# nschloe/flow

Hardware: AMD Instinct MI355X
Metric: ipcs_time_steps_per_sec (higher is better)
Workload: dtype f64

## Files before the change

### flow_amd/_hip.py

```python
import ctypes
import os

import torch

from . import device

_HERE = os.path.dirname(os.path.abspath(__file__))
LIB_PATH = os.path.join(_HERE, 'csrc', 'libflow_hip.so')

REDUCE_WORK = 4096
GMRES_MAX_RESTART = 30
GMRES_PARTIALS = (GMRES_MAX_RESTART + 2) * 1024
GMRES_STATE = 1280
SPMV_ROWS_PER_BLOCK = 256
SPMV_NNZ_PER_BLOCK = 1022
PMG_NNZ_PER_BLOCK = 2044

c_double_p = ctypes.c_void_p
c_int_p = ctypes.c_void_p


class Operator(ctypes.Structure):
    _fields_ = [
        ('kind', ctypes.c_int),
        ('n', ctypes.c_int),
        ('nnz', ctypes.c_int),
        ('nblocks', ctypes.c_int),
        ('rowptr', ctypes.c_void_p),
        ('cols', ctypes.c_void_p),
        ('rowblocks', ctypes.c_void_p),
        ('vals', ctypes.c_void_p * 4),
        ('matfree', ctypes.c_void_p),
        ('rowmask', ctypes.c_void_p),
        ]


class CoarseS(ctypes.Structure):
    _fields_ = [
        ('n', ctypes.c_int),
        ('nc', ctypes.c_int),
        ('agg_ptr', ctypes.c_void_p),
        ('agg_dofs', ctypes.c_void_p),
        ('agg_of', ctypes.c_void_p),
        ('lda', ctypes.c_int),
        ('Ainv', ctypes.c_void_p),
        ]


MG_MAX_LEVELS = 8


class MgS(ctypes.Structure):
    _fields_ = [
        ('nlevels', ctypes.c_int),
        ('Ah', Operator * MG_MAX_LEVELS),
        ('dinv', ctypes.c_void_p * MG_MAX_LEVELS),
        ('Ps', Operator * MG_MAX_LEVELS),
        ('R', Operator * MG_MAX_LEVELS),
        ('r', ctypes.c_void_p * MG_MAX_LEVELS),
        ('x', ctypes.c_void_p * MG_MAX_LEVELS),
        ('t', ctypes.c_void_p * MG_MAX_LEVELS),
        ('nc', ctypes.c_int), ('lda', ctypes.c_int),
        ('Ainv', ctypes.c_void_p),
        ('omega', ctypes.c_double),
        ('C', Operator * MG_MAX_LEVELS),
        ('up_rowblocks', ctypes.c_void_p * MG_MAX_LEVELS),
        ('up_nblocks', ctypes.c_int * MG_MAX_LEVELS),
        ]


class IluPlanS(ctypes.Structure):
    _fields_ = [
        ('n', ctypes.c_int), ('nnz', ctypes.c_int), ('ncolors', ctypes.c_int),
        ('nnz_l', ctypes.c_int), ('nnz_u', ctypes.c_int),
        ('off_l', ctypes.c_int), ('off_u', ctypes.c_int),
        ('off_d', ctypes.c_int), ('lu_size', ctypes.c_int),
        ('max_row', ctypes.c_int), ('nslices', ctypes.c_int),
        ('color_ptr_host', ctypes.c_void_p),
        ('slice_ptr_host', ctypes.c_void_p),
        ('rowptr', ctypes.c_void_p), ('cols', ctypes.c_void_p),
        ('diag', ctypes.c_void_p), ('src_pos', ctypes.c_void_p),
        ('old_of_new', ctypes.c_void_p), ('new_of_old', ctypes.c_void_p),
        ('slice_row', ctypes.c_void_p),
        ('l_slice_off', ctypes.c_void_p), ('l_cols', ctypes.c_void_p),
        ('l_pos', ctypes.c_void_p),
        ('u_slice_off', ctypes.c_void_p), ('u_cols', ctypes.c_void_p),
        ('u_pos', ctypes.c_void_p),
        ]


class IluS(ctypes.Structure):
    _fields_ = [
        ('plan', ctypes.POINTER(IluPlanS)),
        ('nblocks', ctypes.c_int),
        ('lu', ctypes.c_void_p),
        ('packed', ctypes.c_void_p),
        ('single_vector', ctypes.c_int),
        ('cycle', ctypes.c_void_p),
        ]


class TlS(ctypes.Structure):
    _fields_ = [
        ('fine', ctypes.POINTER(IluS)), ('coarse', ctypes.POINTER(IluS)),
        ('fine_op', ctypes.c_void_p), ('coarse_op', ctypes.c_void_p),
        ('pre', ctypes.c_int), ('post', ctypes.c_int),
        ('coarse_sweeps', ctypes.c_int),
        ('ends', ctypes.c_void_p), ('rptr', ctypes.c_void_p),
        ('rsrc', ctypes.c_void_p),
        ('bc_fine', ctypes.c_void_p), ('bc_coarse', ctypes.c_void_p),
        ('rscale', ctypes.c_void_p), ('work', ctypes.c_void_p),
        ]


class PmgLevelS(ctypes.Structure):
    _fields_ = [
        ('n', ctypes.c_int), ('nnz', ctypes.c_int), ('nblocks', ctypes.c_int),
        ('rowptr', ctypes.c_void_p), ('cols', ctypes.c_void_p),
        ('rowblocks', ctypes.c_void_p),
        ('vals', ctypes.c_void_p), ('diag', ctypes.c_void_p),
        ('dinv', ctypes.c_void_p),
        ('lam_min', ctypes.c_double), ('lam_max', ctypes.c_double),
        ('cols16', ctypes.c_void_p), ('cbase', ctypes.c_void_p),
        ('packed', ctypes.c_void_p), ('idrows', ctypes.c_void_p),
        ]


class PmgS(ctypes.Structure):
    _fields_ = [
        ('fine', PmgLevelS), ('coarse', PmgLevelS),
        ('pre', ctypes.c_int), ('post', ctypes.c_int),
        ('coarse_steps', ctypes.c_int),
        ('ends', ctypes.c_void_p),
        ('rptr', ctypes.c_void_p), ('rsrc', ctypes.c_void_p),
        ('bc_fine', ctypes.c_void_p), ('bc_coarse', ctypes.c_void_p),
        ('work', ctypes.c_void_p),
        ('scalar', ctypes.c_int),
        ]


class MassS(ctypes.Structure):
    _fields_ = [
        ('A', ctypes.POINTER(Operator)),
        ('dinv', ctypes.c_void_p),
        ('nblocks16', ctypes.c_int),
        ('rowblocks16', ctypes.c_void_p),
        ('vals16', ctypes.c_void_p),
        ('lam_min', ctypes.c_double), ('lam_max', ctypes.c_double),
        ('steps', ctypes.c_int),
        ('contraction', ctypes.c_double),
        ('work16', ctypes.c_void_p),
        ('packed16', ctypes.c_void_p),
        ('cbase16', ctypes.c_void_p),
        ('work16_rows', ctypes.c_int),
        ]


class MassStripsS(ctypes.Structure):
    _fields_ = [
        ('nlevels', ctypes.c_int),
        ('rowblocks16', ctypes.c_void_p * 16),
        ('nblocks16', ctypes.c_int * 16),
        ('row_lo_last', ctypes.c_int), ('row_hi_last', ctypes.c_int),
        ]


class MeshS(ctypes.Structure):
    _fields_ = [('nc', ctypes.c_int), ('xy', ctypes.c_void_p),
                ('c0', ctypes.c_int), ('c1', ctypes.c_int)]


class SpaceS(ctypes.Structure):
    _fields_ = [
        ('deg', ctypes.c_int),
        ('n', ctypes.c_int),
        ('nnz', ctypes.c_int),
        ('cell_dofs', ctypes.c_void_p),
        ('cptr', ctypes.c_void_p),
        ('csrc', ctypes.c_void_p),
        ('vptr', ctypes.c_void_p),
        ('vsrc', ctypes.c_void_p),
        ('r0', ctypes.c_int), ('r1', ctypes.c_int),
        ('nnz0', ctypes.c_int), ('nnz1', ctypes.c_int),
        ]


class CoefS(ctypes.Structure):
    _fields_ = [
        ('nl', ctypes.c_int),
        ('cell_stride', ctypes.c_int),
        ('values', ctypes.c_void_p),
        ('G', ctypes.c_void_p),
        ]


FORM_MAX_PROGRAM = 64
FORM_REGISTERS = 8
FORM_MAX_CONSTANTS = 32
FORM_MAX_FIELDS = 6
FORM_MAX_EXPRESSIONS = 4
FORM_MAX_POINTS = 256


class FormS(ctypes.Structure):
    _fields_ = [
        ('nprog', ctypes.c_int),
        ('prog', ctypes.c_int * (4 * FORM_MAX_PROGRAM)),
        ('nconst', ctypes.c_int),
        ('consts', ctypes.c_double * FORM_MAX_CONSTANTS),
        ('nfield', ctypes.c_int),
        ('field', ctypes.c_void_p * FORM_MAX_FIELDS),
        ('field_deg', ctypes.c_int * FORM_MAX_FIELDS),
        ('cell_dofs', ctypes.c_void_p * 2),
        ('nexpr', ctypes.c_int),
        ('expr', ctypes.c_void_p * FORM_MAX_EXPRESSIONS),
        ('expr_nl', ctypes.c_int * FORM_MAX_EXPRESSIONS),
        ('expr_table', ctypes.c_int * FORM_MAX_EXPRESSIONS),
        ('nq', ctypes.c_int),
        ('rule', ctypes.c_void_p),
        ('tables', ctypes.c_void_p),
        ('ntables', ctypes.c_int),
        ('nout', ctypes.c_int),
        ]


class PointGridS(ctypes.Structure):
    _fields_ = [
        ('nx', ctypes.c_int), ('ny', ctypes.c_int),
        ('x0', ctypes.c_double), ('y0', ctypes.c_double),
        ('hx_inv', ctypes.c_double), ('hy_inv', ctypes.c_double),
        ('start', ctypes.c_void_p),
        ('cells', ctypes.c_void_p),
        ]


class NsParams(ctypes.Structure):
    _fields_ = [
        ('dt', ctypes.c_double), ('rho', ctypes.c_double),
        ('mu', ctypes.c_double), ('theta_i', ctypes.c_double),
        ('theta_e', ctypes.c_double),
        ]


ALLREDUCE_FN = ctypes.CFUNCTYPE(ctypes.c_int, ctypes.c_void_p, ctypes.c_int)


class PeerS(ctypes.Structure):
    _fields_ = [
        ('flags', ctypes.c_void_p), ('land', ctypes.c_void_p),
        ('land_cap', ctypes.c_int), ('spin_limit', ctypes.c_int),
        ('nb_flags', ctypes.c_void_p * 2), ('nb_land', ctypes.c_void_p * 2),
        ('seq_host', ctypes.POINTER(ctypes.c_ulonglong * 5)),
        ]


PEER_FLAGS = 16


class CommS(ctypes.Structure):
    _fields_ = [
        ('rank', ctypes.c_int), ('world', ctypes.c_int),
        ('buf', ctypes.c_void_p), ('capacity', ctypes.c_int),
        ('allreduce', ALLREDUCE_FN), ('user', ctypes.c_void_p),
        ('peer', ctypes.POINTER(PeerS)),
        ]


class RcclBinding(ctypes.Structure):
    _fields_ = [('comm', ctypes.c_void_p), ('buf', ctypes.c_void_p),
                ('stream', ctypes.c_void_p)]


class RowsS(ctypes.Structure):
    _fields_ = [
        ('n', ctypes.c_int), ('r0', ctypes.c_int), ('r1', ctypes.c_int),
        ('e0', ctypes.c_int), ('e1', ctypes.c_int), ('nhalo', ctypes.c_int),
        ('send_row', ctypes.c_int * 2), ('send_len', ctypes.c_int * 2),
        ('send_slot', ctypes.c_int * 2),
        ('recv_row', ctypes.c_int * 2), ('recv_len', ctypes.c_int * 2),
        ('recv_slot', ctypes.c_int * 2),
        ]


class MgShardS(ctypes.Structure):
    _fields_ = [
        ('mg', ctypes.POINTER(MgS)),
        ('Ah0', Operator), ('Ps0', Operator), ('Rg', Operator),
        ('Cg', Operator),
        ('up_rowblocks0', ctypes.c_void_p), ('up_nblocks0', ctypes.c_int),
        ('z_lo', ctypes.c_int), ('z_hi', ctypes.c_int),
        ]


class MomentumJvp(ctypes.Structure):
    _fields_ = [
        ('mesh', ctypes.POINTER(MeshS)),
        ('W', ctypes.POINTER(SpaceS)),
        ('bfmask', ctypes.c_void_p),
        ('ui', ctypes.c_void_p),
        ('prm', NsParams),
        ('scratch', ctypes.c_void_p),
        ('nbc', ctypes.c_int),
        ('bc_dofs', ctypes.c_void_p),
        ('bc_mask', ctypes.c_void_p),
        ]


_VP = ctypes.c_void_p
_I = ctypes.c_int
_D = ctypes.c_double
_P = ctypes.POINTER
SYMBOLS = {
    'flow_abi_version': [],
    'flow_launch_count': [_P(ctypes.c_ulonglong)],
    'flow_graph_mode': [_I, ctypes.c_longlong],
    'flow_graph_stats': [_P(ctypes.c_ulonglong)],
    'flow_xcd_tile_host': [_I, _I],
    'flow_spmv_tile_nnz': [_I],
    'flow_operator_apply': [_P(Operator), _VP, _VP, _VP],
    'flow_profile_spmv_begin': [_I, _I],
    'flow_profile_spmv_end': [_P(_D), _P(_I)],
    'flow_profile_event_overhead': [_P(_D), _VP],
    'flow_profile_marker': [_I, _VP],
    'flow_profile_stream_copy': [ctypes.c_size_t, _VP, _VP, _VP],
    'flow_profile_stream_read': [ctypes.c_size_t, _VP, _VP, _VP],
    'flow_operator_diag_inv': [_P(Operator), _VP, _VP, _VP],
    'flow_dot_host': [_I, _VP, _VP, _VP, _P(_D), _VP],
    'flow_norm_host': [_I, _VP, _I, _VP, _P(_D), _VP],
    'flow_axpby': [_I, _D, _VP, _D, _VP, _VP],
    'flow_vmul': [_I, _D, _VP, _VP, _VP, _VP],
    'flow_fill': [_I, _D, _VP, _VP],
    'flow_lincomb': [_I, _I, _P(_D), _P(_VP), _VP, _VP],
    'flow_fingerprint': [_I, _P(_VP), _P(_I), _VP, _VP, _VP],
    'flow_read_doubles': [_VP, _I, _P(_D), _VP],
    'flow_extrapolation_weights': [_I, _P(_D), _D, _I, _I, _P(_D)],
    'flow_scale_rows': [_I, _VP, _VP, _VP, _VP],
    'flow_cg_solve': [_P(Operator), _VP, _P(CoarseS), _P(MgS), _VP, _VP, _D, _D,
                      _I, _I, _I, _VP, ctypes.c_size_t, _P(_I), _P(_D), _VP],
    'flow_cg_solve_guarded': [_P(Operator), _VP, _P(CoarseS), _P(MgS), _VP, _VP,
                              _VP, _D, _D, _I, _I, _I, _VP, ctypes.c_size_t,
                              _P(_I), _P(_D), _P(_I), _VP],
    'flow_mg_apply': [_P(MgS), _I, _VP, _VP, _VP],
    'flow_two_level_apply': [_P(CoarseS), _VP, _VP, _VP, _VP, _VP],
    'flow_bicgstab_solve': [_P(Operator), _VP, _P(IluS), _VP, _VP, _D, _D, _I,
                            _I, _I, _VP, ctypes.c_size_t, _P(_I), _P(_D), _VP],
    'flow_gmres_solve': [_P(Operator), _VP, _P(IluS), _P(PmgS), _VP, _VP, _D,
                         _D, _I, _I, _I, _I, _I, _VP, ctypes.c_size_t, _P(_I),
                         _P(_D), _VP],
    'flow_pmg_pack': [_I, _I, _VP, _VP, _VP, _VP, _VP, _VP, _VP, _VP, _VP],
    'flow_pmg_pack1': [_I, _I, _I, _VP, _VP, _VP, _VP, _VP, _VP, _VP, _VP, _VP,
                       _VP, _VP, _VP, _VP],
    'flow_pmg_cols16': [_I, _VP, _VP, _VP, _VP, _VP, _VP, _VP],
    'flow_pmg_lambda_max': [_P(PmgLevelS), _I, _VP, _VP, _VP, _P(_D), _VP],
    'flow_pmg_apply': [_P(PmgS), _VP, _VP, _VP],
    'flow_tl_apply': [_P(TlS), _VP, _VP, _VP],
    'flow_aggregate_host': [_I, _VP, _VP, _VP, ctypes.c_double, _VP, _VP,
                            _P(ctypes.c_int)],
    'flow_peer_alloc': [ctypes.c_int, _P(ctypes.c_void_p), ctypes.c_char_p],
    'flow_peer_open': [ctypes.c_char_p, _P(ctypes.c_void_p)],
    'flow_peer_close': [_VP],
    'flow_peer_free': [_VP],
    'flow_peer_status': [_P(PeerS), _P(ctypes.c_ulonglong), _VP],
    'flow_mass_pack': [_I, _VP, _VP, _VP, _VP, _VP],
    'flow_mass_pack16': [_I, _I, _VP, _VP, _VP, _VP, _VP, _VP, _VP, _VP, _VP],
    'flow_mass_solve': [_P(MassS), _VP, _VP, _D, _D, _I, _I, _VP,
                        ctypes.c_size_t, _P(_I), _P(_D), _VP],
    'flow_mass_solve_increment': [_P(MassS), _VP, _VP, _VP, _VP, _D, _D, _I, _I, _VP,
                                  ctypes.c_size_t, _P(_I), _P(_D), _VP],
    'flow_gather_rows': [_I, _VP, _I, _VP, _I, _VP, _I, _VP],
    'flow_color_greedy_host': [_I, _VP, _VP, _VP, _P(_I)],
    'flow_color_iterate_host': [_I, _VP, _VP, _VP, _P(_I), _I],
    'flow_ilu0_factor': [_P(IluPlanS), _I, _VP, _VP, _VP, _VP],
    'flow_ilu0_pack': [_P(IluS), _VP, _VP],
    'flow_ilu0_solve': [_P(IluS), _VP, _VP, _VP, _VP],
    'flow_rccl_load': [ctypes.c_char_p],
    'flow_rccl_unique_id': [_VP],
    'flow_rccl_comm_create': [_VP, _I, _I, _P(_VP)],
    'flow_rccl_comm_destroy': [_VP],
    'flow_rccl_allreduce': [_VP, _I],
    'flow_shard_halo': [_P(CommS), _P(RowsS), _I, _VP, _I, _VP],
    'flow_shard_reduce_host': [_P(CommS), _P(RowsS), _I, _VP, _VP, _I, _I, _VP,
                               _P(_D), _VP],
    'flow_shard_cg_solve': [_P(CommS), _P(RowsS), _P(Operator), _VP, _VP, _VP,
                            _D, _D, _I, _I, _I, _VP, ctypes.c_size_t, _P(_I),
                            _P(_D), _P(_I), _VP],
    'flow_shard_mgcg_solve': [_P(CommS), _P(RowsS), _P(Operator), _VP,
                              _P(MgShardS), _VP, _VP, _D, _D, _I, _I, _I, _VP,
                              ctypes.c_size_t, _P(_I), _P(_D), _P(_I), _VP],
    'flow_shard_mass_solve': [_P(CommS), _P(RowsS), _P(MassS), _P(MassStripsS),
                              _VP, _VP, _VP, _VP, _D, _D, _I, _I, _VP,
                              ctypes.c_size_t, _P(_I), _P(_D), _VP],
    'flow_shard_gmres_solve': [_P(CommS), _P(RowsS), _P(Operator), _P(IluS),
                               _P(PmgS), _VP, _VP, _D, _D, _I, _I, _I, _I, _I,
                               _VP, ctypes.c_size_t, _P(_I), _P(_D), _VP],
    'flow_assemble_scalar_matrix': [_I, _P(MeshS), _P(SpaceS), _VP, _VP, _VP],
    'flow_assemble_pressure_rhs': [_P(MeshS), _P(SpaceS), _P(SpaceS), _VP, _VP,
                                   _D, _D, _I, _VP, _VP, _VP],
    'flow_assemble_correction_rhs': [_P(MeshS), _P(SpaceS), _P(SpaceS), _VP,
                                     _VP, _VP, _D, _D, _I, _VP, _VP, _VP],
    'flow_assemble_momentum': [_P(MeshS), _P(SpaceS), _P(SpaceS), _VP, _VP, _VP,
                               _VP, _P(CoefS), _P(CoefS), _P(NsParams), _VP,
                               _VP, _VP, ctypes.c_size_t, _VP],
    'flow_momentum_jvp_apply': [_P(MomentumJvp), _VP, _VP, _VP],
    'flow_assemble_source': [_P(MeshS), _P(SpaceS), _I, _P(CoefS), _VP, _VP,
                             _VP],
    'flow_assemble_magnitude': [_P(MeshS), _P(SpaceS), _I, _VP, _VP, _VP, _VP],
    'flow_assemble_div_adjoint': [_P(MeshS), _P(SpaceS), _P(SpaceS), _VP, _VP,
                                  _VP, _VP],
    'flow_bc_identity_rows': [_P(Operator), _VP, _VP, _I, _VP, _VP],
    'flow_bc_residual': [_I, _VP, _VP, _VP, _VP, _VP],
    'flow_bc_set_values': [_I, _VP, _VP, _VP, _VP],
    'flow_bc_symmetric_matrix': [_I, _VP, _VP, _VP, _VP, _VP, _VP],
    'flow_assemble_heat': [_P(MeshS), _P(SpaceS), _P(SpaceS), _VP, _D, _D, _I,
                           _VP, _VP, _VP, _VP, _VP, _VP],
    'flow_assemble_heat_supg_source': [_P(MeshS), _P(SpaceS), _P(SpaceS), _VP,
                                       _D, _D, _P(CoefS), _VP, _VP, _VP, _VP],
    'flow_form_functional': [_P(MeshS), _P(FormS), _VP, _VP, _P(_D), _VP],
    'flow_form_load_vector': [_P(MeshS), _P(SpaceS), _P(FormS), _VP, _VP, _VP],
    'flow_form_facet_functional': [_P(MeshS), _P(FormS), _I, _VP, _VP, _VP, _VP,
                                   _P(_D), _VP],
    'flow_locate_points': [_P(MeshS), _P(PointGridS), _I, _VP, _VP, _VP, _VP],
    'flow_form_points': [_P(MeshS), _P(FormS), _I, _VP, _VP, _VP, _VP],
    }

_LIB = None


class HipError(RuntimeError):
    pass


class NotConverged(RuntimeError):
    '''Krylov / Newton non-convergence.  A RuntimeError, because callers of the
    reference catch exactly that (tests/test_boussinesq.py:254).'''


ABI_VERSION = 30


def load_library():
    global _LIB
    if _LIB is None:
        if not os.path.isfile(LIB_PATH):
            raise HipError(
                'libflow_hip.so not found at %s -- build it with '
                '`python -c "import __graft_entry__ as g; g.build()"` or '
                '`make -C flow_amd/csrc`' % LIB_PATH
                )
        lib = ctypes.CDLL(LIB_PATH)
        lib.flow_last_error.restype = ctypes.c_char_p
        lib.flow_last_error.argtypes = []
        for name, argtypes in SYMBOLS.items():
            fn = getattr(lib, name)
            fn.restype = ctypes.c_int
            fn.argtypes = argtypes
        got = lib.flow_abi_version()
        if got != ABI_VERSION:
            raise HipError(
                '%s is ABI version %d, these bindings are version %d: '
                'rebuild it (`make -C flow_amd/csrc`)'
                % (LIB_PATH, got, ABI_VERSION))
        _LIB = lib
    return _LIB


def launch_count():
    n = ctypes.c_ulonglong(0)
    check(load_library().flow_launch_count(ctypes.byref(n)))
    return int(n.value)


_GRAPHS = {'mode': None}


def graph_mode(mode, auto_rows=-1, sites=0):
    check(load_library().flow_graph_mode(int(mode) | (int(sites) << 4),
                                         int(auto_rows)))
    _GRAPHS['mode'] = int(mode)


def graphs_possible():
    if _GRAPHS['mode'] is not None:
        return _GRAPHS['mode'] != 0
    return os.environ.get('FLOW_AMD_GRAPHS', '0') not in ('', '0')


def graph_stats():
    v = (ctypes.c_ulonglong * 8)()
    check(load_library().flow_graph_stats(v))
    return {'graphs': int(v[0]), 'captures': int(v[1]), 'replays': int(v[2]),
            'nodes': int(v[3]), 'captures_cg': int(v[4]),
            'captures_gmres': int(v[5]), 'captures_mass': int(v[6])}


def spmv_tile_nnz(kind=0):
    return int(load_library().flow_spmv_tile_nnz(int(kind)))


def lib():
    handle = load_library()
    if not device.on_gpu():
        raise HipError(
            'flow_amd needs an AMD GPU (MI355X): the hot path has no CPU '
            'fallback'
            )
    return handle


def check(rc):
    if rc == 0:
        return
    msg = load_library().flow_last_error().decode('utf-8', 'replace')
    if rc == 1:
        raise NotConverged(msg)
    if rc == 2:
        raise ValueError(msg)
    raise HipError(msg)


def _ptr(t, dtype, numel=None, name='operand'):
    if t is None:
        return None
    if not isinstance(t, torch.Tensor):
        raise TypeError('%s: expected a torch tensor' % name)
    if t.dtype != dtype:
        raise TypeError('%s: dtype %s, expected %s' % (name, t.dtype, dtype))
    if not t.is_cuda:
        raise HipError('%s is not in device memory' % name)
    if not t.is_contiguous():
        raise ValueError('%s is not contiguous' % name)
    if numel is not None and t.numel() < numel:
        raise ValueError(
            '%s has %d elements, needs %d' % (name, t.numel(), numel)
            )
    return ctypes.c_void_p(t.data_ptr())


def f64(t, numel=None, name='fp64 operand'):
    return _ptr(t, torch.float64, numel, name)


def f32(t, numel=None, name='fp32 operand'):
    return _ptr(t, torch.float32, numel, name)


def f16(t, numel=None, name='fp16 operand'):
    return _ptr(t, torch.float16, numel, name)


def i32(t, numel=None, name='int32 operand'):
    return _ptr(t, torch.int32, numel, name)


def u8(t, numel=None, name='uint8 operand'):
    return _ptr(t, torch.uint8, numel, name)


def stream():
    return ctypes.c_void_p(device.stream_handle())


def copy(dst, src):
    assert dst.numel() == src.numel()
    if not dst.is_cuda:
        dst.copy_(src)
    elif dst.data_ptr() != src.data_ptr():
        check(lib().flow_axpby(dst.numel(), 1.0, f64(src, name='src'), 0.0,
                               f64(dst, name='dst'), stream()))
    return dst


def fill(t, value=0.0):
    if not t.is_cuda:
        t.fill_(float(value))
    elif t.numel() > 0:
        check(lib().flow_fill(t.numel(), float(value), f64(t), stream()))
    return t


def clone(t):
    out = torch.empty_like(t)
    return copy(out, t)
```

### flow_amd/csrc/assembly_kernels.hip

```cpp
#include <cstdlib>

#include "fem_device.h"

namespace flow {

template <int NP>
__global__ __launch_bounds__(kBlock) void gather_kernel(
    int nout, const int* __restrict__ ptr, const int* __restrict__ src,
    const double* __restrict__ scratch, size_t plane_stride, size_t out_stride,
    double* __restrict__ out, const double* __restrict__ stop,
    const unsigned char* __restrict__ idrow = nullptr, size_t id_stride = 0,
    const double* __restrict__ v = nullptr, size_t v_stride = 0) {
  if (stopped(stop)) return;
  for (int k = blockIdx.x * blockDim.x + threadIdx.x; k < nout;
       k += gridDim.x * blockDim.x) {
    const int a = ptr[k];
    const int b = ptr[k + 1];
    double s[NP];
#pragma unroll
    for (int p = 0; p < NP; ++p) s[p] = 0.0;
    for (int t = a; t < b; t += 4) {
      int idx[4];
#pragma unroll
      for (int j = 0; j < 4; ++j) idx[j] = t + j < b ? src[t + j] : -1;
      double w[NP][4];
#pragma unroll
      for (int p = 0; p < NP; ++p)
#pragma unroll
        for (int j = 0; j < 4; ++j)
          w[p][j] = idx[j] >= 0 ? scratch[p * plane_stride + idx[j]] : 0.0;
#pragma unroll
      for (int p = 0; p < NP; ++p)
#pragma unroll
        for (int j = 0; j < 4; ++j) s[p] += w[p][j];
    }
    if (idrow) {
#pragma unroll
      for (int p = 0; p < NP; ++p)
        if (idrow[p * id_stride + k]) s[p] = v[p * v_stride + k];
    }
#pragma unroll
    for (int p = 0; p < NP; ++p) out[static_cast<size_t>(p) * out_stride + k] = s[p];
  }
}

int gather(int nout, int nplanes, const int* ptr, const int* src,
           const double* scratch, size_t plane_stride, double* out,
           hipStream_t st, size_t out_stride, int r0, int r1, const double* stop,
           const unsigned char* idrow, const double* v, size_t v_stride) {
  const size_t os = out_stride ? out_stride : static_cast<size_t>(nout);
  const size_t ids = static_cast<size_t>(nout);
  if (r1 > 0) {
    ptr += r0;
    out += r0;
    if (idrow) idrow += r0;
    if (v) v += r0;
    nout = r1 - r0;
  }
  const dim3 grid(grid_for(nout, kBlock, 1 << 20));
  FLOW_REQUIRE(nplanes == 1 || nplanes == 2, "gather: 1 or 2 planes");
  if (nplanes == 1)
    hipLaunchKernelGGL(gather_kernel<1>, grid, dim3(kBlock), 0, st, nout, ptr,
                       src, scratch, plane_stride, os, out, stop, idrow, ids, v,
                       v_stride);
  else
    hipLaunchKernelGGL(gather_kernel<2>, grid, dim3(kBlock), 0, st, nout, ptr,
                       src, scratch, plane_stride, os, out, stop, idrow, ids, v,
                       v_stride);
  FLOW_CHECK_LAUNCH();
  return FLOW_OK;
}

template <int NL>
__device__ __forceinline__ void load_local(const double* __restrict__ u, int n,
                                           const int* __restrict__ cd, int nc,
                                           int c, int ,
                                           double U[2][NL]) {
#pragma unroll
  for (int i = 0; i < NL; ++i) {
    const int d = cd[i * nc + c];
    U[0][i] = u[d];
    U[1][i] = u[static_cast<size_t>(n) + d];
  }
}

template <int DEG>
__global__ __launch_bounds__(kBlock) void scalar_matrix_kernel(
    int kind, int nc, const double* __restrict__ xy,
    double* __restrict__ scratch) {
  constexpr int NL = Elem<DEG>::NL;
  constexpr int NQ = Elem<2>::NQ;
  const int c = blockIdx.x * blockDim.x + threadIdx.x;
  if (c >= nc) return;
  const Geom g = load_geom(xy, nc, c);
  double Ke[NL][NL];
#pragma unroll
  for (int i = 0; i < NL; ++i)
#pragma unroll
    for (int j = 0; j < NL; ++j) Ke[i][j] = 0.0;
  if (kind == 2) {
#pragma unroll
    for (int i = 0; i < 3; ++i) Ke[i][i] = g.adet / 6.0;
  } else {
#pragma unroll
    for (int q = 0; q < NQ; ++q) {
      const double L[3] = {kQ7L[q][0], kQ7L[q][1], kQ7L[q][2]};
      const double w = 0.5 * kQ7W[q] * g.adet;
      double phi[NL], dphi[NL][3], gphi[NL][2];
      basis<DEG>(L, phi, dphi);
      phys_grad<NL>(g, dphi, gphi);
#pragma unroll
      for (int i = 0; i < NL; ++i)
#pragma unroll
        for (int j = 0; j < NL; ++j)
          Ke[i][j] += (kind == 0)
                          ? w * (gphi[i][0] * gphi[j][0] + gphi[i][1] * gphi[j][1])
                          : w * phi[i] * phi[j];
    }
  }
#pragma unroll
  for (int i = 0; i < NL; ++i)
#pragma unroll
    for (int j = 0; j < NL; ++j)
      scratch[static_cast<size_t>(i * NL + j) * nc + c] = Ke[i][j];
}

template <int DEG>
__global__ __launch_bounds__(kBlock) void pressure_rhs_kernel(
    int nc, int cb, int ce, const double* __restrict__ xy, const int* __restrict__ cdu, int nu,
    const int* __restrict__ cdp, const double* __restrict__ u,
    const double* __restrict__ p0, double alpha_rho_dt, double mu,
    int rotational, double* __restrict__ scratch) {
  constexpr int NL = Elem<DEG>::NL;
  const int c = cb + xcd_tile(blockIdx.x, gridDim.x) * blockDim.x + threadIdx.x;
  if (c >= ce) return;
  const Geom g = load_geom(xy, nc, c);
  double U[2][NL];
  load_local<NL>(u, nu, cdu, nc, c, 2, U);
  double d[3];
  div_at_vertices<DEG>(g, U, d);
  const double area = 0.5 * g.adet;
  const double dsum = d[0] + d[1] + d[2];
  double gp[2] = {0.0, 0.0};
#pragma unroll
  for (int k = 0; k < 3; ++k) {
    double coef = p0[cdp[k * nc + c]];
    if (rotational) coef -= mu * d[k];
    gp[0] += coef * g.gl[k][0];
    gp[1] += coef * g.gl[k][1];
  }
#pragma unroll
  for (int i = 0; i < 3; ++i) {
    const double b = -alpha_rho_dt * (area / 12.0) * (dsum + d[i]) +
                     area * (gp[0] * g.gl[i][0] + gp[1] * g.gl[i][1]);
    scratch[static_cast<size_t>(i) * nc + c] = b;
  }
}

template <int DEG>
__global__ __launch_bounds__(kBlock) void correction_rhs_kernel(
    int nc, int cb, int ce, const double* __restrict__ xy, const int* __restrict__ cdu, int nu,
    const int* __restrict__ cdp, const double* __restrict__ u,
    const double* __restrict__ p1, const double* __restrict__ p0, double dt_rho,
    double mu, int rotational, double* __restrict__ scratch) {
  constexpr int NL = Elem<DEG>::NL;
  constexpr int NQ = Elem<2>::NQ;
  const int c = cb + xcd_tile(blockIdx.x, gridDim.x) * blockDim.x + threadIdx.x;
  if (c >= ce) return;
  const Geom g = load_geom(xy, nc, c);
  double U[2][NL];
  load_local<NL>(u, nu, cdu, nc, c, 2, U);
  double d[3] = {0.0, 0.0, 0.0};
  if (rotational & 1) div_at_vertices<DEG>(g, U, d);
  const double mass = (rotational & 2) ? 0.0 : 1.0;
  double gphi_f[2] = {0.0, 0.0};
#pragma unroll
  for (int k = 0; k < 3; ++k) {
    const int dof = cdp[k * nc + c];
    const double coef = p1[dof] - p0[dof] + mu * d[k];
    gphi_f[0] += coef * g.gl[k][0];
    gphi_f[1] += coef * g.gl[k][1];
  }
  double acc[2][NL];
#pragma unroll
  for (int a = 0; a < 2; ++a)
#pragma unroll
    for (int i = 0; i < NL; ++i) acc[a][i] = 0.0;
#pragma unroll
  for (int q = 0; q < NQ; ++q) {
    const double L[3] = {kQ7L[q][0], kQ7L[q][1], kQ7L[q][2]};
    const double w = 0.5 * kQ7W[q] * g.adet;
    double phi[NL], dphi[NL][3];
    basis<DEG>(L, phi, dphi);
#pragma unroll
    for (int a = 0; a < 2; ++a) {
      double uq = 0.0;
#pragma unroll
      for (int j = 0; j < NL; ++j) uq += U[a][j] * phi[j];
      const double val = w * (mass * uq - dt_rho * gphi_f[a]);
#pragma unroll
      for (int i = 0; i < NL; ++i) acc[a][i] += val * phi[i];
    }
  }
#pragma unroll
  for (int a = 0; a < 2; ++a)
#pragma unroll
    for (int i = 0; i < NL; ++i)
      scratch[static_cast<size_t>(a * NL + i) * nc + c] = acc[a][i];
}

template <int NL>
__device__ __forceinline__ void add_source(const flow_coef& f, int nc, int c,
                                           int dim, double scale,
                                           double acc[][NL]) {
  const size_t nce = f.cell_stride ? static_cast<size_t>(nc) : 1;
  const size_t cc = f.cell_stride ? static_cast<size_t>(c) : 0;
  for (int a = 0; a < dim; ++a) {
    for (int l = 0; l < f.nl; ++l) {
      const double F = scale * f.values[(static_cast<size_t>(a) * f.nl + l) * nce + cc];
#pragma unroll
      for (int i = 0; i < NL; ++i) acc[a][i] += F * f.G[l * NL + i];
    }
  }
}

template <int DEG>
__global__ __launch_bounds__(kBlock) void source_kernel(
    int nc, const double* __restrict__ xy, int dim, flow_coef f,
    double* __restrict__ scratch) {
  constexpr int NL = Elem<DEG>::NL;
  const int c = blockIdx.x * blockDim.x + threadIdx.x;
  if (c >= nc) return;
  const Geom g = load_geom(xy, nc, c);
  double acc[2][NL];
#pragma unroll
  for (int a = 0; a < 2; ++a)
#pragma unroll
    for (int i = 0; i < NL; ++i) acc[a][i] = 0.0;
  add_source<NL>(f, nc, c, dim, g.adet, acc);
  for (int a = 0; a < dim; ++a)
#pragma unroll
    for (int i = 0; i < NL; ++i)
      scratch[static_cast<size_t>(a * NL + i) * nc + c] = acc[a][i];
}

template <int NL>
__device__ __forceinline__ void add_rhs_weak_point(
    double w, double rho, double mu, const double U[2][NL], const double P[3],
    const double L[3], const double phi[NL], const double gphi[NL][2],
    double acc[2][NL]) {
  double uq[2] = {0.0, 0.0};
  double gu[2][2] = {{0.0, 0.0}, {0.0, 0.0}};
#pragma unroll
  for (int j = 0; j < NL; ++j) {
#pragma unroll
    for (int a = 0; a < 2; ++a) {
      uq[a] += U[a][j] * phi[j];
      gu[a][0] += U[a][j] * gphi[j][0];
      gu[a][1] += U[a][j] * gphi[j][1];
    }
  }
  const double pq = P[0] * L[0] + P[1] * L[1] + P[2] * L[2];
  const double conv[2] = {gu[0][0] * uq[0] + gu[0][1] * uq[1],
                          gu[1][0] * uq[0] + gu[1][1] * uq[1]};
#pragma unroll
  for (int i = 0; i < NL; ++i) {
    const double ugp = uq[0] * gphi[i][0] + uq[1] * gphi[i][1];
#pragma unroll
    for (int a = 0; a < 2; ++a) {
      double r = -0.5 * rho * (conv[a] * phi[i] - ugp * uq[a]);
      r -= mu * ((gu[a][0] + gu[0][a]) * gphi[i][0] +
                 (gu[a][1] + gu[1][a]) * gphi[i][1]);
      r += pq * gphi[i][a];
      acc[a][i] += w * r;
    }
  }
}

template <int DEG>
__device__ __forceinline__ void add_rhs_weak_facets(
    int mask, double scale, double mu, const Geom& g,
    const double U[2][Elem<DEG>::NL], const double P[3],
    double acc[2][Elem<DEG>::NL]) {
  constexpr int NL = Elem<DEG>::NL;
  for (int lf = 0; lf < 3; ++lf) {
    if (!((mask >> lf) & 1)) continue;
    const int v0 = facet_v0(lf), v1 = facet_v1(lf);
    const double nL[2] = {-g.gl[lf][0] * g.adet, -g.gl[lf][1] * g.adet};
    for (int gq = 0; gq < 2; ++gq) {
      const double s = gq == 0 ? FLOW_G2A : FLOW_G2B;
      double L[3] = {0.0, 0.0, 0.0};
      L[v0] = 1.0 - s;
      L[v1] = s;
      double phi[NL], dphi[NL][3], gphi[NL][2];
      basis<DEG>(L, phi, dphi);
      phys_grad<NL>(g, dphi, gphi);
      double gu[2][2] = {{0.0, 0.0}, {0.0, 0.0}};
#pragma unroll
      for (int j = 0; j < NL; ++j)
#pragma unroll
        for (int a = 0; a < 2; ++a) {
          gu[a][0] += U[a][j] * gphi[j][0];
          gu[a][1] += U[a][j] * gphi[j][1];
        }
      const double pq = P[0] * L[0] + P[1] * L[1] + P[2] * L[2];
      const double w = 0.5 * scale;
#pragma unroll
      for (int a = 0; a < 2; ++a) {
        const double t = -pq * nL[a] + mu * (gu[0][a] * nL[0] + gu[1][a] * nL[1]);
#pragma unroll
        for (int i = 0; i < NL; ++i) acc[a][i] += w * t * phi[i];
      }
    }
  }
}

template <int DEG>
__global__ __launch_bounds__(kBlock) void momentum_residual_kernel(
    int nc, int cb, int ce, const double* __restrict__ xy, const int* __restrict__ cdu, int nu,
    const int* __restrict__ cdp, const int* __restrict__ bfmask,
    const double* __restrict__ ui, const double* __restrict__ u0,
    const double* __restrict__ p0, flow_coef f0, flow_coef f1,
    flow_ns_params prm, double* __restrict__ scratch) {
  constexpr int NL = Elem<DEG>::NL;
  constexpr int NQ = Elem<DEG>::NQ;
  const int c = cb + xcd_tile(blockIdx.x, gridDim.x) * blockDim.x + threadIdx.x;
  if (c >= ce) return;
  const Geom g = load_geom(xy, nc, c);
  double Ui[2][NL], U0[2][NL], P[3];
  load_local<NL>(ui, nu, cdu, nc, c, 2, Ui);
  load_local<NL>(u0, nu, cdu, nc, c, 2, U0);
#pragma unroll
  for (int k = 0; k < 3; ++k) P[k] = p0[cdp[k * nc + c]];
  const int mask = bfmask[c];
  const double ci = -prm.dt / prm.rho * prm.theta_i;
  const double cexp = -prm.dt / prm.rho * prm.theta_e;
  double acc[2][NL];
#pragma unroll
  for (int a = 0; a < 2; ++a)
#pragma unroll
    for (int i = 0; i < NL; ++i) acc[a][i] = 0.0;

#pragma unroll
  for (int q = 0; q < NQ; ++q) {
    const double L[3] = {qpoint<DEG>(q, 0), qpoint<DEG>(q, 1), qpoint<DEG>(q, 2)};
    const double w = 0.5 * qweight<DEG>(q) * g.adet;
    double phi[NL], dphi[NL][3], gphi[NL][2];
    basis<DEG>(L, phi, dphi);
    phys_grad<NL>(g, dphi, gphi);
#pragma unroll
    for (int a = 0; a < 2; ++a) {
      double du = 0.0;
#pragma unroll
      for (int j = 0; j < NL; ++j) du += (Ui[a][j] - U0[a][j]) * phi[j];
#pragma unroll
      for (int i = 0; i < NL; ++i) acc[a][i] += w * du * phi[i];
    }
    if (ci != 0.0)
      add_rhs_weak_point<NL>(w * ci, prm.rho, prm.mu, Ui, P, L, phi, gphi, acc);
    if (cexp != 0.0)
      add_rhs_weak_point<NL>(w * cexp, prm.rho, prm.mu, U0, P, L, phi, gphi, acc);
  }
  if (mask) {
    if (ci != 0.0) add_rhs_weak_facets<DEG>(mask, ci, prm.mu, g, Ui, P, acc);
    if (cexp != 0.0) add_rhs_weak_facets<DEG>(mask, cexp, prm.mu, g, U0, P, acc);
  }
  if (ci != 0.0) add_source<NL>(f1, nc, c, 2, ci * g.adet, acc);
  if (cexp != 0.0) add_source<NL>(f0, nc, c, 2, cexp * g.adet, acc);
#pragma unroll
  for (int a = 0; a < 2; ++a)
#pragma unroll
    for (int i = 0; i < NL; ++i)
      scratch[static_cast<size_t>(a * NL + i) * nc + c] = acc[a][i];
}

template <int DEG>
__global__ __launch_bounds__(kBlock) void momentum_jvp_kernel(
    int nc, int cb, int ce, const double* __restrict__ xy,
    const int* __restrict__ cdu, int nu, int nv,
    const int* __restrict__ bfmask, const double* __restrict__ ui,
    const double* __restrict__ v, flow_ns_params prm,
    const double* __restrict__ prm_dev,
    double* __restrict__ scratch, const double* __restrict__ stop) {
  constexpr int NL = Elem<DEG>::NL;
  constexpr int NQ = Elem<DEG>::NQ;
  if (stopped(stop)) return;
  const int c = cb + xcd_tile(blockIdx.x, gridDim.x) * blockDim.x + threadIdx.x;
  if (c >= ce) return;
  const Geom g = load_geom(xy, nc, c);
  double U[2][NL], V[2][NL];
  load_local<NL>(ui, nu, cdu, nc, c, 2, U);
  load_local<NL>(v, nv, cdu, nc, c, 2, V);
  const int mask = bfmask[c];
  const double ci = prm_dev ? load_scalar(prm_dev)
                            : -prm.dt / prm.rho * prm.theta_i;
  const double hr = prm_dev ? load_scalar(prm_dev + 1) : 0.5 * prm.rho;
  const double mu = prm_dev ? load_scalar(prm_dev + 2) : prm.mu;
  double acc[2][NL];
#pragma unroll
  for (int a = 0; a < 2; ++a)
#pragma unroll
    for (int i = 0; i < NL; ++i) acc[a][i] = 0.0;

#pragma unroll
  for (int q = 0; q < NQ; ++q) {
    const double L[3] = {qpoint<DEG>(q, 0), qpoint<DEG>(q, 1), qpoint<DEG>(q, 2)};
    const double w = 0.5 * qweight<DEG>(q) * g.adet;
    double uq[2], vq[2], gu[2][2], gv[2][2];
#pragma unroll
    for (int a = 0; a < 2; ++a) {
      uq[a] = eval_at<DEG>(U[a], L);
      vq[a] = eval_at<DEG>(V[a], L);
      double gur[3], gvr[3];
      ref_gradient<DEG>(U[a], L, gur);
      ref_gradient<DEG>(V[a], L, gvr);
#pragma unroll
      for (int d = 0; d < 2; ++d) {
        gu[a][d] = gur[0] * g.gl[0][d] + gur[1] * g.gl[1][d] + gur[2] * g.gl[2][d];
        gv[a][d] = gvr[0] * g.gl[0][d] + gvr[1] * g.gl[1][d] + gvr[2] * g.gl[2][d];
      }
    }
#pragma unroll
    for (int a = 0; a < 2; ++a) {
      const double dconv = gv[a][0] * uq[0] + gv[a][1] * uq[1] +
                           gu[a][0] * vq[0] + gu[a][1] * vq[1];
      const double s0 = w * (vq[a] - ci * hr * dconv);
      double S1[2];
#pragma unroll
      for (int d = 0; d < 2; ++d)
        S1[d] = w * ci * (hr * (vq[d] * uq[a] + uq[d] * vq[a]) -
                          mu * (gv[a][d] + gv[d][a]));
      double T[3];
#pragma unroll
      for (int k = 0; k < 3; ++k) T[k] = g.gl[k][0] * S1[0] + g.gl[k][1] * S1[1];
      test_accumulate<DEG>(L, s0, T, acc[a]);
    }
  }
  if (mask && ci != 0.0) {
    const double P0[3] = {0.0, 0.0, 0.0};
    add_rhs_weak_facets<DEG>(mask, ci, mu, g, V, P0, acc);
  }
#pragma unroll
  for (int a = 0; a < 2; ++a)
#pragma unroll
    for (int i = 0; i < NL; ++i)
      scratch[static_cast<size_t>(a * NL + i) * nc + c] = acc[a][i];
}

template <int DEG>
__global__ __launch_bounds__(kBlock) void momentum_jvp_pair_kernel(
    int nc, int cb, int ce, const double* __restrict__ xy,
    const int* __restrict__ cdu, int nu, int nv,
    const int* __restrict__ bfmask, const double* __restrict__ ui,
    const double* __restrict__ v, flow_ns_params prm,
    const double* __restrict__ prm_dev,
    double* __restrict__ scratch, const double* __restrict__ stop) {
  constexpr int NL = Elem<DEG>::NL;
  constexpr int NQ = Elem<DEG>::NQ;
  if (stopped(stop)) return;
  const int t = xcd_tile(blockIdx.x, gridDim.x) * blockDim.x + threadIdx.x;
  const int c = cb + (t >> 1);
  const int a = t & 1;
  if (c >= ce) return;
  const Geom g = load_geom(xy, nc, c);
  double U[NL], V[NL];
#pragma unroll
  for (int i = 0; i < NL; ++i) {
    const int d = cdu[i * nc + c];
    U[i] = ui[static_cast<size_t>(a) * nu + d];
    V[i] = v[static_cast<size_t>(a) * nv + d];
  }
  const int mask = bfmask[c];
  const double ci = prm_dev ? load_scalar(prm_dev)
                            : -prm.dt / prm.rho * prm.theta_i;
  const double hr = prm_dev ? load_scalar(prm_dev + 1) : 0.5 * prm.rho;
  const double mu = prm_dev ? load_scalar(prm_dev + 2) : prm.mu;
  double acc[NL];
#pragma unroll
  for (int i = 0; i < NL; ++i) acc[i] = 0.0;

#pragma unroll
  for (int q = 0; q < NQ; ++q) {
    const double L[3] = {qpoint<DEG>(q, 0), qpoint<DEG>(q, 1), qpoint<DEG>(q, 2)};
    const double w = 0.5 * qweight<DEG>(q) * g.adet;
    const double uq = eval_at<DEG>(U, L);
    const double vq = eval_at<DEG>(V, L);
    double gur[3], gvr[3], gu[2], gv[2];
    ref_gradient<DEG>(U, L, gur);
    ref_gradient<DEG>(V, L, gvr);
#pragma unroll
    for (int d = 0; d < 2; ++d) {
      gu[d] = gur[0] * g.gl[0][d] + gur[1] * g.gl[1][d] + gur[2] * g.gl[2][d];
      gv[d] = gvr[0] * g.gl[0][d] + gvr[1] * g.gl[1][d] + gvr[2] * g.gl[2][d];
    }
    const double uo = __shfl_xor(uq, 1, 64);
    const double vo = __shfl_xor(vq, 1, 64);
    const double cross = __shfl_xor(a == 0 ? gv[1] : gv[0], 1, 64);
    const double u0 = a == 0 ? uq : uo, u1 = a == 0 ? uo : uq;
    const double v0 = a == 0 ? vq : vo, v1 = a == 0 ? vo : vq;
    const double dconv = gv[0] * u0 + gv[1] * u1 + gu[0] * v0 + gu[1] * v1;
    const double s0 = w * (vq - ci * hr * dconv);
    const double t0 = a == 0 ? gv[0] : cross;
    const double t1 = a == 0 ? cross : gv[1];
    double S1[2];
    S1[0] = w * ci * (hr * (v0 * uq + u0 * vq) - mu * (gv[0] + t0));
    S1[1] = w * ci * (hr * (v1 * uq + u1 * vq) - mu * (gv[1] + t1));
    double T[3];
#pragma unroll
    for (int k = 0; k < 3; ++k) T[k] = g.gl[k][0] * S1[0] + g.gl[k][1] * S1[1];
    test_accumulate<DEG>(L, s0, T, acc);
  }
  if (mask && ci != 0.0) {
    for (int lf = 0; lf < 3; ++lf) {
      if (!((mask >> lf) & 1)) continue;
      const int f0 = facet_v0(lf), f1 = facet_v1(lf);
      const double nL[2] = {-g.gl[lf][0] * g.adet, -g.gl[lf][1] * g.adet};
      for (int gq = 0; gq < 2; ++gq) {
        const double sg = gq == 0 ? FLOW_G2A : FLOW_G2B;
        double L[3] = {0.0, 0.0, 0.0};
        L[f0] = 1.0 - sg;
        L[f1] = sg;
        double gvr[3], gv[2];
        ref_gradient<DEG>(V, L, gvr);
#pragma unroll
        for (int d = 0; d < 2; ++d)
          gv[d] = gvr[0] * g.gl[0][d] + gvr[1] * g.gl[1][d] + gvr[2] * g.gl[2][d];
        const double cross = __shfl_xor(a == 0 ? gv[1] : gv[0], 1, 64);
        const double tn = a == 0 ? gv[0] * nL[0] + cross * nL[1]
                                 : cross * nL[0] + gv[1] * nL[1];
        const double wt = 0.5 * ci * mu * tn;
        double phi[NL], dphi[NL][3];
        basis<DEG>(L, phi, dphi);
#pragma unroll
        for (int i = 0; i < NL; ++i) acc[i] += wt * phi[i];
      }
    }
  }
#pragma unroll
  for (int i = 0; i < NL; ++i)
    scratch[static_cast<size_t>(a * NL + i) * nc + c] = acc[i];
}

__global__ void bc_copy_kernel(int nbc, const int* __restrict__ dofs, int n,
                               int r0, int r1, const double* __restrict__ v,
                               int vs, double* __restrict__ out, int os,
                               const double* __restrict__ stop) {
  if (stopped(stop)) return;
  const int k = blockIdx.x * blockDim.x + threadIdx.x;
  if (k >= nbc) return;
  const int d = dofs[k];
  const int a = d / n;
  const int row = d - a * n;
  if (row >= r0 && row < r1)
    out[static_cast<size_t>(a) * os + row] = v[static_cast<size_t>(a) * vs + row];
}

template <int DEG>
struct BasisTab {
  double phi[Elem<DEG>::NQ][Elem<DEG>::NL];
  double dphi[Elem<DEG>::NQ][Elem<DEG>::NL][3];
};

template <int DEG>
__global__ __launch_bounds__(kBlock) void momentum_jacobian_kernel(
    int nc, int cb, int ce, const double* __restrict__ xy, const int* __restrict__ cdu, int nu,
    const int* __restrict__ bfmask, const double* __restrict__ ui,
    flow_ns_params prm, double* __restrict__ scratch) {
  constexpr int NL = Elem<DEG>::NL;
  constexpr int NQ = Elem<DEG>::NQ;
  constexpr int NP = NL * NL;
  __shared__ double s_uq[NQ][2][64];
  __shared__ double s_gu[NQ][4][64];
  __shared__ BasisTab<DEG> tab;

  const int lane = threadIdx.x & 63;
  const int grp = threadIdx.x >> 6;
  const int c = cb + blockIdx.x * 64 + lane;
  const bool active = c < ce;
  const int cc = active ? c : ce - 1;

  for (int t = threadIdx.x; t < NQ * NL; t += kBlock) {
    const int q = t / NL, i = t % NL;
    const double L[3] = {qpoint<DEG>(q, 0), qpoint<DEG>(q, 1), qpoint<DEG>(q, 2)};
    double phi[NL], dphi[NL][3];
    basis<DEG>(L, phi, dphi);
    tab.phi[q][i] = phi[i];
    tab.dphi[q][i][0] = dphi[i][0];
    tab.dphi[q][i][1] = dphi[i][1];
    tab.dphi[q][i][2] = dphi[i][2];
  }

  const Geom g = load_geom(xy, nc, cc);
  const int mask = bfmask[cc];
  {
    double U[2][NL];
    load_local<NL>(ui, nu, cdu, nc, cc, 2, U);
    for (int q = grp; q < NQ; q += 4) {
      const double L[3] = {qpoint<DEG>(q, 0), qpoint<DEG>(q, 1),
                           qpoint<DEG>(q, 2)};
      double phi[NL], dphi[NL][3], gphi[NL][2];
      basis<DEG>(L, phi, dphi);
      phys_grad<NL>(g, dphi, gphi);
      double uq[2] = {0.0, 0.0}, gu[4] = {0.0, 0.0, 0.0, 0.0};
#pragma unroll
      for (int j = 0; j < NL; ++j) {
        uq[0] += U[0][j] * phi[j];
        uq[1] += U[1][j] * phi[j];
        gu[0] += U[0][j] * gphi[j][0];
        gu[1] += U[0][j] * gphi[j][1];
        gu[2] += U[1][j] * gphi[j][0];
        gu[3] += U[1][j] * gphi[j][1];
      }
      s_uq[q][0][lane] = uq[0];
      s_uq[q][1][lane] = uq[1];
#pragma unroll
      for (int k = 0; k < 4; ++k) s_gu[q][k][lane] = gu[k];
    }
  }
  __syncthreads();

  const double c1 = -prm.dt / prm.rho * prm.theta_i;
  const double hr = 0.5 * prm.rho;
  const double mu = prm.mu;

  for (int pr = grp; pr < NP; pr += 4) {
    const int i = pr / NL, j = pr % NL;
    double B[2][2] = {{0.0, 0.0}, {0.0, 0.0}};
#pragma unroll
    for (int q = 0; q < NQ; ++q) {
      const double w = 0.5 * qweight<DEG>(q) * g.adet;
      const double pi = tab.phi[q][i], pj = tab.phi[q][j];
      double gi[2], gj[2];
#pragma unroll
      for (int d = 0; d < 2; ++d) {
        gi[d] = tab.dphi[q][i][0] * g.gl[0][d] + tab.dphi[q][i][1] * g.gl[1][d] +
                tab.dphi[q][i][2] * g.gl[2][d];
        gj[d] = tab.dphi[q][j][0] * g.gl[0][d] + tab.dphi[q][j][1] * g.gl[1][d] +
                tab.dphi[q][j][2] * g.gl[2][d];
      }
      const double u0 = s_uq[q][0][lane], u1 = s_uq[q][1][lane];
      const double gu[2][2] = {{s_gu[q][0][lane], s_gu[q][1][lane]},
                               {s_gu[q][2][lane], s_gu[q][3][lane]}};
      const double uq[2] = {u0, u1};
      const double ugj = u0 * gj[0] + u1 * gj[1];
      const double ugi = u0 * gi[0] + u1 * gi[1];
      const double kij = gi[0] * gj[0] + gi[1] * gj[1];
      const double diag =
          pi * pj + c1 * (-hr * (ugj * pi - ugi * pj) - mu * kij);
#pragma unroll
      for (int a = 0; a < 2; ++a)
#pragma unroll
        for (int cb = 0; cb < 2; ++cb) {
          double v = c1 * (-hr * (pj * pi * gu[a][cb] - pj * gi[cb] * uq[a]) -
                           mu * gj[a] * gi[cb]);
          if (a == cb) v += diag;
          B[a][cb] += w * v;
        }
    }
    if (mask) {
      for (int lf = 0; lf < 3; ++lf) {
        if (!((mask >> lf) & 1)) continue;
        const int v0 = facet_v0(lf), v1 = facet_v1(lf);
        const double nL[2] = {-g.gl[lf][0] * g.adet, -g.gl[lf][1] * g.adet};
        for (int gq = 0; gq < 2; ++gq) {
          const double s = gq == 0 ? FLOW_G2A : FLOW_G2B;
          double L[3] = {0.0, 0.0, 0.0};
          L[v0] = 1.0 - s;
          L[v1] = s;
          double phi[NL], dphi[NL][3], gphi[NL][2];
          basis<DEG>(L, phi, dphi);
          phys_grad<NL>(g, dphi, gphi);
          double pi = 0.0, gj0 = 0.0, gj1 = 0.0;
#pragma unroll
          for (int t = 0; t < NL; ++t) {
            if (t == i) pi = phi[t];
            if (t == j) {
              gj0 = gphi[t][0];
              gj1 = gphi[t][1];
            }
          }
          const double w = 0.5 * c1 * mu * pi;
          B[0][0] += w * gj0 * nL[0];
          B[0][1] += w * gj0 * nL[1];
          B[1][0] += w * gj1 * nL[0];
          B[1][1] += w * gj1 * nL[1];
        }
      }
    }
    if (active) {
      double2* out = reinterpret_cast<double2*>(
          scratch + (static_cast<size_t>(c) * NP + pr) * 4);
      out[0] = make_double2(B[0][0], B[0][1]);
      out[1] = make_double2(B[1][0], B[1][1]);
    }
  }
}

__global__ void gather_blocks_kernel(int k0, int nnz, int nc, int np,
                                     const int* __restrict__ ptr,
                                     const int* __restrict__ src,
                                     const double* __restrict__ scratch,
                                     size_t out_stride,
                                     double* __restrict__ out) {
  for (int k = k0 + blockIdx.x * blockDim.x + threadIdx.x; k < nnz;
       k += gridDim.x * blockDim.x) {
    const int a = ptr[k];
    const int b = ptr[k + 1];
    double s0 = 0.0, s1 = 0.0, s2 = 0.0, s3 = 0.0;
    for (int t = a; t < b; ++t) {
      const int s = src[t];
      const int ij = s / nc;
      const int cell = s - ij * nc;
      const double2* blk = reinterpret_cast<const double2*>(
          scratch + (static_cast<size_t>(cell) * np + ij) * 4);
      const double2 v0 = blk[0], v1 = blk[1];
      s0 += v0.x;
      s1 += v0.y;
      s2 += v1.x;
      s3 += v1.y;
    }
    out[k] = s0;
    out[out_stride + k] = s1;
    out[2 * out_stride + k] = s2;
    out[3 * out_stride + k] = s3;
  }
}

__global__ void bc_identity_rows_kernel(int kind, int n, size_t nnz,
                                        const int* __restrict__ rowptr,
                                        const int* __restrict__ diag_idx,
                                        int nbc, const int* __restrict__ dofs,
                                        double* __restrict__ vals) {
  for (int t = blockIdx.x * blockDim.x + threadIdx.x; t < nbc;
       t += gridDim.x * blockDim.x) {
    const int d = dofs[t];
    const int a = d / n;
    const int i = d - a * n;
    const int k0 = rowptr[i], k1 = rowptr[i + 1];
    if (kind == 2) {
      double* p0 = vals + static_cast<size_t>(2 * a) * nnz;
      double* p1 = vals + static_cast<size_t>(2 * a + 1) * nnz;
      for (int k = k0; k < k1; ++k) {
        p0[k] = 0.0;
        p1[k] = 0.0;
      }
      vals[static_cast<size_t>(3 * a) * nnz + diag_idx[i]] = 1.0;
    } else {
      double* p = vals + static_cast<size_t>(a) * nnz;
      for (int k = k0; k < k1; ++k) p[k] = 0.0;
      p[diag_idx[i]] = 1.0;
    }
  }
}

__global__ void bc_residual_kernel(int nbc, const int* __restrict__ dofs,
                                   const double* __restrict__ g,
                                   const double* __restrict__ u,
                                   double* __restrict__ F) {
  for (int t = blockIdx.x * blockDim.x + threadIdx.x; t < nbc;
       t += gridDim.x * blockDim.x) {
    const int d = dofs[t];
    F[d] = u ? u[d] - g[t] : g[t];
  }
}

__global__ void bc_symmetric_kernel(int n, const int* __restrict__ rowptr,
                                    const int* __restrict__ cols,
                                    const double* __restrict__ vin,
                                    const unsigned char* __restrict__ isbc,
                                    double* __restrict__ vout) {
  for (int r = blockIdx.x * blockDim.x + threadIdx.x; r < n;
       r += gridDim.x * blockDim.x) {
    const bool rb = isbc[r] != 0;
    for (int k = rowptr[r]; k < rowptr[r + 1]; ++k) {
      const int c = cols[k];
      vout[k] = (rb || isbc[c]) ? (r == c ? 1.0 : 0.0) : vin[k];
    }
  }
}

__device__ __forceinline__ double supg_tau(const double px[3], const double py[3],
                                           double area, double bx, double by,
                                           double eps, int p, int* status) {
  const double nb = sqrt(bx * bx + by * by);
  if (nb < 1.0e-10) return 0.0;
  double sum = 0.0;
#pragma unroll
  for (int i = 0; i < 3; ++i)
#pragma unroll
    for (int j = i + 1; j < 3; ++j) {
      const double e0 = px[i] - px[j];
      const double e1 = py[i] - py[j];
      sum += fabs(e1 * bx - e0 * by);
    }
  const double h = 4.0 * nb * area / sum;
  const double Pe = 0.5 * nb * h / (p * eps);
  const double xi = Pe > 1.0e-5
                        ? (1.0 / tanh(Pe) - 1.0 / Pe) / Pe
                        : 1.0 / 3.0 - Pe * Pe / 45.0 +
                              2.0 / 945.0 * Pe * Pe * Pe * Pe;
  const double tau = h * h / 4.0 / eps / p * xi;
  if (tau > 1.0e3) *status = 1;
  return tau;
}

template <int DEGQ, int DEGW, bool SUPG>
__global__ __launch_bounds__(kBlock) void heat_kernel(
    int nc, int cb, int ce, const double* __restrict__ xy,
    const int* __restrict__ cdw, int nw,
    const double* __restrict__ conv, double kappa, double rho_cp,
    double* __restrict__ scratch, double* __restrict__ tau_out,
    int* __restrict__ status) {
  constexpr int NL = Elem<DEGQ>::NL;
  constexpr int NW = Elem<DEGW>::NL;
  constexpr int NQ = SUPG ? 16 : 7;
  const int c = cb + blockIdx.x * blockDim.x + threadIdx.x;
  if (c >= ce) return;
  const Geom g = load_geom(xy, nc, c);
  double Cv[2][NW];
  load_local<NW>(conv, nw, cdw, nc, c, 2, Cv);
  double tau_v[3] = {0.0, 0.0, 0.0};
  double lap[NL];
#pragma unroll
  for (int i = 0; i < NL; ++i) lap[i] = 0.0;
  if constexpr (SUPG) {
    const double px[3] = {xy[0 * nc + c], xy[1 * nc + c], xy[2 * nc + c]};
    const double py[3] = {xy[3 * nc + c], xy[4 * nc + c], xy[5 * nc + c]};
#pragma unroll
    for (int m = 0; m < 3; ++m)
      tau_v[m] = supg_tau(px, py, 0.5 * g.adet, Cv[0][m], Cv[1][m], kappa, DEGQ,
                          status);
    if (tau_out) {
#pragma unroll
      for (int m = 0; m < 3; ++m) tau_out[static_cast<size_t>(m) * nc + c] = tau_v[m];
    }
    if constexpr (DEGQ == 2) {
#pragma unroll
      for (int i = 0; i < 3; ++i)
        lap[i] = 4.0 * (g.gl[i][0] * g.gl[i][0] + g.gl[i][1] * g.gl[i][1]);
#pragma unroll
      for (int e = 0; e < 3; ++e) {
        const int j = facet_v0(e), k = facet_v1(e);
        lap[3 + e] = 8.0 * (g.gl[j][0] * g.gl[k][0] + g.gl[j][1] * g.gl[k][1]);
      }
    }
  }
  const size_t plane = static_cast<size_t>(NL * NL) * nc;
  for (int i = 0; i < NL; ++i) {
    double Ka[NL], Ma[NL];
#pragma unroll
    for (int j = 0; j < NL; ++j) Ka[j] = Ma[j] = 0.0;
    for (int q = 0; q < NQ; ++q) {
      const double L[3] = {SUPG ? kQ16L[q][0] : kQ7L[q][0],
                           SUPG ? kQ16L[q][1] : kQ7L[q][1],
                           SUPG ? kQ16L[q][2] : kQ7L[q][2]};
      const double w = 0.5 * (SUPG ? kQ16W[q] : kQ7W[q]) * g.adet;
      double phi[NL], dphi[NL][3], gphi[NL][2];
      basis<DEGQ>(L, phi, dphi);
      phys_grad<NL>(g, dphi, gphi);
      double wphi[NW], wd[NW][3];
      basis<DEGW>(L, wphi, wd);
      double b[2] = {0.0, 0.0};
#pragma unroll
      for (int t = 0; t < NW; ++t) {
        b[0] += Cv[0][t] * wphi[t];
        b[1] += Cv[1][t] * wphi[t];
      }
      double pi = 0.0, gi0 = 0.0, gi1 = 0.0;
#pragma unroll
      for (int t = 0; t < NL; ++t)
        if (t == i) {
          pi = phi[t];
          gi0 = gphi[t][0];
          gi1 = gphi[t][1];
        }
      const double tq = tau_v[0] * L[0] + tau_v[1] * L[1] + tau_v[2] * L[2];
      const double cgi = b[0] * gi0 + b[1] * gi1;
#pragma unroll
      for (int j = 0; j < NL; ++j) {
        const double cgj = b[0] * gphi[j][0] + b[1] * gphi[j][1];
        double k = -kappa / rho_cp * (gphi[j][0] * gi0 + gphi[j][1] * gi1) -
                   cgj * pi;
        if constexpr (SUPG) {
          k += (kappa / rho_cp * lap[j] - cgj) * tq * cgi;
          Ma[j] += w * phi[j] * tq * cgi;
        }
        Ka[j] += w * k;
      }
    }
#pragma unroll
    for (int j = 0; j < NL; ++j) {
      const size_t idx = static_cast<size_t>(i * NL + j) * nc + c;
      scratch[idx] = Ka[j];
      if constexpr (SUPG) scratch[plane + idx] = Ma[j];
    }
  }
}

template <int DEGQ, int DEGW>
__global__ __launch_bounds__(kBlock) void heat_supg_source_kernel(
    int nc, int cb, int ce, const double* __restrict__ xy,
    const int* __restrict__ cdw, int nw,
    const double* __restrict__ conv, double kappa, double rho_cp, flow_coef f,
    double* __restrict__ scratch, int* __restrict__ status) {
  constexpr int NL = Elem<DEGQ>::NL;
  constexpr int NW = Elem<DEGW>::NL;
  const int c = cb + blockIdx.x * blockDim.x + threadIdx.x;
  if (c >= ce) return;
  const Geom g = load_geom(xy, nc, c);
  double Cv[2][NW];
  load_local<NW>(conv, nw, cdw, nc, c, 2, Cv);
  const double px[3] = {xy[0 * nc + c], xy[1 * nc + c], xy[2 * nc + c]};
  const double py[3] = {xy[3 * nc + c], xy[4 * nc + c], xy[5 * nc + c]};
  double tau_v[3];
#pragma unroll
  for (int m = 0; m < 3; ++m)
    tau_v[m] = supg_tau(px, py, 0.5 * g.adet, Cv[0][m], Cv[1][m], kappa, DEGQ,
                        status);
  const size_t nce = f.cell_stride ? static_cast<size_t>(nc) : 1;
  const size_t cc = f.cell_stride ? static_cast<size_t>(c) : 0;
  double Sv[6] = {0.0, 0.0, 0.0, 0.0, 0.0, 0.0};
  for (int l = 0; l < f.nl; ++l) Sv[l] = f.values[static_cast<size_t>(l) * nce + cc];
  double acc[NL];
#pragma unroll
  for (int i = 0; i < NL; ++i) acc[i] = 0.0;
  for (int q = 0; q < 16; ++q) {
    const double L[3] = {kQ16L[q][0], kQ16L[q][1], kQ16L[q][2]};
    const double w = 0.5 * kQ16W[q] * g.adet;
    double phi[NL], dphi[NL][3], gphi[NL][2];
    basis<DEGQ>(L, phi, dphi);
    phys_grad<NL>(g, dphi, gphi);
    double wphi[NW], wd[NW][3];
    basis<DEGW>(L, wphi, wd);
    double b[2] = {0.0, 0.0};
#pragma unroll
    for (int t = 0; t < NW; ++t) {
      b[0] += Cv[0][t] * wphi[t];
      b[1] += Cv[1][t] * wphi[t];
    }
    double sq;
    if (f.nl == 1) {
      sq = Sv[0];
    } else if (f.nl == 3) {
      sq = Sv[0] * L[0] + Sv[1] * L[1] + Sv[2] * L[2];
    } else {
      double p2[6], d2[6][3];
      basis<2>(L, p2, d2);
      sq = 0.0;
#pragma unroll
      for (int l = 0; l < 6; ++l) sq += Sv[l] * p2[l];
    }
    const double tq = tau_v[0] * L[0] + tau_v[1] * L[1] + tau_v[2] * L[2];
    const double fac = w * sq / rho_cp * tq;
#pragma unroll
    for (int i = 0; i < NL; ++i)
      acc[i] += fac * (b[0] * gphi[i][0] + b[1] * gphi[i][1]);
  }
#pragma unroll
  for (int i = 0; i < NL; ++i) scratch[static_cast<size_t>(i) * nc + c] = acc[i];
}

template <int DEG>
__global__ __launch_bounds__(kBlock) void div_adjoint_kernel(
    int nc, const double* __restrict__ xy, const int* __restrict__ cdp,
    const double* __restrict__ p, double* __restrict__ scratch) {
  constexpr int NL = Elem<DEG>::NL;
  constexpr int NQ = 7;
  const int c = blockIdx.x * blockDim.x + threadIdx.x;
  if (c >= nc) return;
  const Geom g = load_geom(xy, nc, c);
  double P[3];
#pragma unroll
  for (int k = 0; k < 3; ++k) P[k] = p[cdp[k * nc + c]];
  double acc[2][NL];
#pragma unroll
  for (int a = 0; a < 2; ++a)
#pragma unroll
    for (int i = 0; i < NL; ++i) acc[a][i] = 0.0;
#pragma unroll
  for (int q = 0; q < NQ; ++q) {
    const double L[3] = {kQ7L[q][0], kQ7L[q][1], kQ7L[q][2]};
    const double w = 0.5 * kQ7W[q] * g.adet;
    double phi[NL], dphi[NL][3], gphi[NL][2];
    basis<DEG>(L, phi, dphi);
    phys_grad<NL>(g, dphi, gphi);
    const double pq = P[0] * L[0] + P[1] * L[1] + P[2] * L[2];
#pragma unroll
    for (int i = 0; i < NL; ++i) {
      acc[0][i] -= w * pq * gphi[i][0];
      acc[1][i] -= w * pq * gphi[i][1];
    }
  }
#pragma unroll
  for (int a = 0; a < 2; ++a)
#pragma unroll
    for (int i = 0; i < NL; ++i)
      scratch[static_cast<size_t>(a * NL + i) * nc + c] = acc[a][i];
}

template <int DEG>
__global__ __launch_bounds__(kBlock) void magnitude_kernel(
    int nc, int cb, int ce, const double* __restrict__ xy, const int* __restrict__ cdu, int nu,
    const double* __restrict__ u, int mode, double* __restrict__ scratch) {
  constexpr int NL = Elem<DEG>::NL;
  constexpr int NQ = 7;
  const int c = cb + xcd_tile(blockIdx.x, gridDim.x) * blockDim.x + threadIdx.x;
  if (c >= ce) return;
  const Geom g = load_geom(xy, nc, c);
  double U[2][NL];
  load_local<NL>(u, nu, cdu, nc, c, 2, U);
  double acc[NL];
#pragma unroll
  for (int i = 0; i < NL; ++i) acc[i] = 0.0;
#pragma unroll
  for (int q = 0; q < NQ; ++q) {
    const double L[3] = {kQ7L[q][0], kQ7L[q][1], kQ7L[q][2]};
    const double w = 0.5 * kQ7W[q] * g.adet;
    double phi[NL], dphi[NL][3];
    basis<DEG>(L, phi, dphi);
    double ux = 0.0, uy = 0.0;
#pragma unroll
    for (int j = 0; j < NL; ++j) {
      ux += U[0][j] * phi[j];
      uy += U[1][j] * phi[j];
    }
    const double m = mode == 0 ? sqrt(ux * ux + uy * uy) : fabs(ux) + fabs(uy);
#pragma unroll
    for (int i = 0; i < NL; ++i) acc[i] += w * m * phi[i];
  }
#pragma unroll
  for (int i = 0; i < NL; ++i) scratch[static_cast<size_t>(i) * nc + c] = acc[i];
}

static int check_mesh_space(const flow_mesh* mesh, const flow_space* V) {
  FLOW_REQUIRE(mesh && mesh->nc > 0 && mesh->xy, "mesh");
  FLOW_REQUIRE(mesh->c1 == 0 ||
                   (0 <= mesh->c0 && mesh->c0 < mesh->c1 && mesh->c1 <= mesh->nc),
               "mesh cell range");
  FLOW_REQUIRE(V && (V->deg == 1 || V->deg == 2) && V->n > 0 && V->cell_dofs,
               "space");
  FLOW_REQUIRE(V->r1 == 0 || (0 <= V->r0 && V->r0 < V->r1 && V->r1 <= V->n),
               "space row range");
  return FLOW_OK;
}

struct CellRange {
  int cb, ce;
  explicit CellRange(const flow_mesh* m)
      : cb(m->c1 > 0 ? m->c0 : 0), ce(m->c1 > 0 ? m->c1 : m->nc) {}
  int count() const { return ce - cb; }
};

}

using namespace flow;

#define FLOW_DISPATCH_DEG(deg, KERNEL, grid, st, ...)                          \
  do {                                                                         \
    if ((deg) == 1)                                                            \
      hipLaunchKernelGGL(KERNEL<1>, grid, dim3(kBlock), 0, st, __VA_ARGS__);   \
    else                                                                       \
      hipLaunchKernelGGL(KERNEL<2>, grid, dim3(kBlock), 0, st, __VA_ARGS__);   \
    FLOW_CHECK_LAUNCH();                                                       \
  } while (0)

static inline dim3 cell_grid(int nc) { return dim3((nc + kBlock - 1) / kBlock); }


extern "C" int flow_assemble_scalar_matrix(int kind, const flow_mesh* mesh,
                                           const flow_space* V, double* scratch,
                                           double* vals, void* stream) {
  int rc = check_mesh_space(mesh, V);
  if (rc) return rc;
  FLOW_REQUIRE(kind >= 0 && kind <= 2, "matrix kind");
  FLOW_REQUIRE(scratch && vals && V->cptr && V->csrc && V->nnz > 0, "matrix maps");
  hipStream_t st = as_stream(stream);
  FLOW_DISPATCH_DEG(V->deg, scalar_matrix_kernel, cell_grid(mesh->nc), st, kind,
                    mesh->nc, mesh->xy, scratch);
  return gather(V->nnz, 1, V->cptr, V->csrc, scratch, 0, vals, st);
}

extern "C" int flow_assemble_pressure_rhs(const flow_mesh* mesh,
                                          const flow_space* W,
                                          const flow_space* P, const double* u,
                                          const double* p0, double alpha_rho_dt,
                                          double mu, int rotational,
                                          double* scratch, double* b,
                                          void* stream) {
  int rc = check_mesh_space(mesh, W);
  if (rc) return rc;
  if ((rc = check_mesh_space(mesh, P))) return rc;
  FLOW_REQUIRE(P->deg == 1 && P->vptr && P->vsrc, "pressure space must be P1");
  FLOW_REQUIRE(u && p0 && scratch && b, "pointers");
  hipStream_t st = as_stream(stream);
  const CellRange cr(mesh);
  FLOW_DISPATCH_DEG(W->deg, pressure_rhs_kernel, cell_grid(cr.count()), st,
                    mesh->nc, cr.cb, cr.ce, mesh->xy, W->cell_dofs, W->n,
                    P->cell_dofs, u, p0, alpha_rho_dt, mu, rotational, scratch);
  return gather(P->n, 1, P->vptr, P->vsrc, scratch, 0, b, st, 0, P->r0, P->r1);
}

extern "C" int flow_assemble_correction_rhs(
    const flow_mesh* mesh, const flow_space* W, const flow_space* P,
    const double* u, const double* p1, const double* p0, double dt_rho,
    double mu, int rotational, double* scratch, double* b, void* stream) {
  int rc = check_mesh_space(mesh, W);
  if (rc) return rc;
  if ((rc = check_mesh_space(mesh, P))) return rc;
  FLOW_REQUIRE(P->deg == 1 && W->vptr && W->vsrc, "spaces");
  FLOW_REQUIRE(u && p1 && p0 && scratch && b, "pointers");
  hipStream_t st = as_stream(stream);
  const CellRange cr(mesh);
  FLOW_DISPATCH_DEG(W->deg, correction_rhs_kernel, cell_grid(cr.count()), st,
                    mesh->nc, cr.cb, cr.ce, mesh->xy, W->cell_dofs, W->n,
                    P->cell_dofs, u, p1, p0, dt_rho, mu, rotational, scratch);
  const int nl = W->deg == 1 ? 3 : 6;
  return gather(W->n, 2, W->vptr, W->vsrc, scratch,
                static_cast<size_t>(nl) * mesh->nc, b, st, 0, W->r0, W->r1);
}

static int check_coef(const flow_coef* f) {
  FLOW_REQUIRE(f && f->nl >= 1 && f->nl <= 21 && f->values && f->G, "coefficient");
  FLOW_REQUIRE(f->cell_stride == 0 || f->cell_stride == 1, "coefficient stride");
  return FLOW_OK;
}

extern "C" int flow_assemble_source(const flow_mesh* mesh, const flow_space* V,
                                    int dim, const flow_coef* f, double* scratch,
                                    double* b, void* stream) {
  int rc = check_mesh_space(mesh, V);
  if (rc) return rc;
  if ((rc = check_coef(f))) return rc;
  FLOW_REQUIRE(dim == 1 || dim == 2, "dim");
  FLOW_REQUIRE(scratch && b && V->vptr && V->vsrc, "pointers");
  hipStream_t st = as_stream(stream);
  FLOW_DISPATCH_DEG(V->deg, source_kernel, cell_grid(mesh->nc), st, mesh->nc,
                    mesh->xy, dim, *f, scratch);
  const int nl = V->deg == 1 ? 3 : 6;
  return gather(V->n, dim, V->vptr, V->vsrc, scratch,
                static_cast<size_t>(nl) * mesh->nc, b, st);
}

extern "C" int flow_assemble_momentum(
    const flow_mesh* mesh, const flow_space* W, const flow_space* P,
    const int* bfmask, const double* ui, const double* u0, const double* p0,
    const flow_coef* f0, const flow_coef* f1, const flow_ns_params* prm,
    double* scratch, double* F, double* Jvals, size_t j_plane_stride,
    void* stream) {
  int rc = check_mesh_space(mesh, W);
  if (rc) return rc;
  if ((rc = check_mesh_space(mesh, P))) return rc;
  if ((rc = check_coef(f0))) return rc;
  if ((rc = check_coef(f1))) return rc;
  FLOW_REQUIRE(P->deg == 1, "pressure space must be P1");
  FLOW_REQUIRE(bfmask && ui && u0 && p0 && prm && scratch, "pointers");
  FLOW_REQUIRE(prm->dt > 0.0 && prm->rho > 0.0 && prm->mu > 0.0, "parameters");
  hipStream_t st = as_stream(stream);
  const int nl = W->deg == 1 ? 3 : 6;
  const CellRange cr(mesh);
  if (F) {
    FLOW_REQUIRE(W->vptr && W->vsrc, "vector map");
    FLOW_DISPATCH_DEG(W->deg, momentum_residual_kernel, cell_grid(cr.count()),
                      st, mesh->nc, cr.cb, cr.ce, mesh->xy, W->cell_dofs, W->n,
                      P->cell_dofs, bfmask, ui, u0, p0, *f0, *f1, *prm, scratch);
    if ((rc = gather(W->n, 2, W->vptr, W->vsrc, scratch,
                     static_cast<size_t>(nl) * mesh->nc, F, st, 0, W->r0,
                     W->r1)))
      return rc;
  }
  if (Jvals) {
    FLOW_REQUIRE(W->cptr && W->csrc && W->nnz > 0, "matrix map");
    FLOW_REQUIRE(j_plane_stride >= (size_t)W->nnz, "Jacobian plane stride");
    FLOW_DISPATCH_DEG(W->deg, momentum_jacobian_kernel,
                      dim3((cr.count() + 63) / 64), st, mesh->nc, cr.cb, cr.ce,
                      mesh->xy, W->cell_dofs, W->n, bfmask, ui, *prm, scratch);
    int k0 = 0, k1 = W->nnz;
    if (W->r1 > 0) {
      FLOW_REQUIRE(W->nnz0 >= 0 && W->nnz0 < W->nnz1 && W->nnz1 <= W->nnz,
                   "space nonzero range");
      k0 = W->nnz0;
      k1 = W->nnz1;
    }
    hipLaunchKernelGGL(gather_blocks_kernel,
                       dim3(grid_for(k1 - k0, kBlock, 1 << 20)), dim3(kBlock), 0,
                       st, k0, k1, mesh->nc, nl * nl, W->cptr, W->csrc, scratch,
                       j_plane_stride, Jvals);
    FLOW_CHECK_LAUNCH();
  }
  return FLOW_OK;
}

int flow::momentum_jvp_check(const flow_momentum_jvp* J) {
  FLOW_REQUIRE(J != nullptr, "matrix-free Jacobian is NULL");
  int rc = check_mesh_space(J->mesh, J->W);
  if (rc) return rc;
  FLOW_REQUIRE(J->W->vptr && J->W->vsrc, "vector map");
  FLOW_REQUIRE(J->bfmask && J->ui && J->scratch, "matrix-free Jacobian pointers");
  FLOW_REQUIRE(J->prm.dt > 0.0 && J->prm.rho > 0.0 && J->prm.mu > 0.0,
               "parameters");
  FLOW_REQUIRE(J->nbc >= 0 && (J->nbc == 0 || J->bc_dofs), "Dirichlet dofs");
  return FLOW_OK;
}

__global__ void jvp_params_kernel(flow_ns_params prm, double* __restrict__ dst) {
  if (threadIdx.x == 0) {
    store_scalar(dst, -prm.dt / prm.rho * prm.theta_i);
    store_scalar(dst + 1, 0.5 * prm.rho);
    store_scalar(dst + 2, prm.mu);
  }
}

int flow::momentum_jvp_params(const flow_momentum_jvp* J, double* dst,
                              hipStream_t st) {
  hipLaunchKernelGGL(jvp_params_kernel, dim3(1), dim3(64), 0, st, J->prm, dst);
  FLOW_CHECK_LAUNCH();
  return FLOW_OK;
}

int flow::momentum_jvp_apply(const flow_momentum_jvp* J, const double* v,
                             double* out, hipStream_t st, int v_stride,
                             int out_stride, const double* stop,
                             const double* prm_dev) {
  const flow_mesh* mesh = J->mesh;
  const flow_space* W = J->W;
  const int nl = W->deg == 1 ? 3 : 6;
  const int vs = v_stride ? v_stride : W->n;
  const int os = out_stride ? out_stride : W->n;
  const CellRange cr(mesh);
  int rc;
  static const bool pair = [] {
    const char* e = getenv("FLOW_AMD_JVP_PAIR");
    return e && e[0] == '1';
  }();
  if (W->deg == 2 && pair) {
    hipLaunchKernelGGL(momentum_jvp_pair_kernel<2>, cell_grid(2 * cr.count()),
                       dim3(kBlock), 0, st, mesh->nc, cr.cb, cr.ce, mesh->xy,
                       W->cell_dofs, W->n, vs, J->bfmask, J->ui, v, J->prm,
                       prm_dev, J->scratch, stop);
    FLOW_CHECK_LAUNCH();
  } else {
    FLOW_DISPATCH_DEG(W->deg, momentum_jvp_kernel, cell_grid(cr.count()), st,
                      mesh->nc, cr.cb, cr.ce, mesh->xy, W->cell_dofs, W->n, vs,
                      J->bfmask, J->ui, v, J->prm, prm_dev, J->scratch, stop);
  }
  if ((rc = gather(W->n, 2, W->vptr, W->vsrc, J->scratch,
                   static_cast<size_t>(nl) * mesh->nc, out, st, os, W->r0,
                   W->r1, stop, J->nbc > 0 ? J->bc_mask : nullptr, v, vs)))
    return rc;
  if (J->nbc > 0 && !J->bc_mask) {
    const int r0 = W->r1 > 0 ? W->r0 : 0, r1 = W->r1 > 0 ? W->r1 : W->n;
    hipLaunchKernelGGL(bc_copy_kernel, dim3(grid_for(J->nbc)), dim3(kBlock), 0,
                       st, J->nbc, J->bc_dofs, W->n, r0, r1, v, vs, out, os, stop);
    FLOW_CHECK_LAUNCH();
  }
  return FLOW_OK;
}

extern "C" int flow_momentum_jvp_apply(const flow_momentum_jvp* J,
                                       const double* v, double* out,
                                       void* stream) {
  int rc = momentum_jvp_check(J);
  if (rc) return rc;
  FLOW_REQUIRE(v && out && v != out, "jvp vectors");
  return momentum_jvp_apply(J, v, out, as_stream(stream), 0, 0, nullptr);
}

extern "C" int flow_assemble_magnitude(const flow_mesh* mesh, const flow_space* W,
                                       int mode, const double* u,
                                       double* scratch, double* b,
                                       void* stream) {
  int rc = check_mesh_space(mesh, W);
  if (rc) return rc;
  FLOW_REQUIRE(mode == 0 || mode == 1, "mode");
  FLOW_REQUIRE(u && scratch && b && W->vptr && W->vsrc, "pointers");
  hipStream_t st = as_stream(stream);
  const CellRange cr(mesh);
  FLOW_DISPATCH_DEG(W->deg, magnitude_kernel, cell_grid(cr.count()), st, mesh->nc,
                    cr.cb, cr.ce, mesh->xy, W->cell_dofs, W->n, u, mode, scratch);
  return gather(W->n, 1, W->vptr, W->vsrc, scratch, 0, b, st, 0, W->r0, W->r1);
}

extern "C" int flow_assemble_div_adjoint(const flow_mesh* mesh,
                                         const flow_space* W, const flow_space* P,
                                         const double* p, double* scratch,
                                         double* out, void* stream) {
  int rc = check_mesh_space(mesh, W);
  if (rc) return rc;
  if ((rc = check_mesh_space(mesh, P))) return rc;
  FLOW_REQUIRE(P->deg == 1, "pressure space must be P1");
  FLOW_REQUIRE(p && scratch && out && W->vptr && W->vsrc, "pointers");
  hipStream_t st = as_stream(stream);
  FLOW_DISPATCH_DEG(W->deg, div_adjoint_kernel, cell_grid(mesh->nc), st, mesh->nc,
                    mesh->xy, P->cell_dofs, p, scratch);
  const int nl = W->deg == 1 ? 3 : 6;
  return gather(W->n, 2, W->vptr, W->vsrc, scratch,
                static_cast<size_t>(nl) * mesh->nc, out, st);
}

extern "C" int flow_bc_identity_rows(const flow_operator* A, double* vals_planes,
                                     const int* diag_idx, int nbc,
                                     const int* dofs, void* stream) {
  FLOW_REQUIRE(A && A->n > 0 && A->nnz > 0 && A->rowptr, "operator");
  FLOW_REQUIRE(A->kind >= 0 && A->kind <= 2, "operator kind");
  FLOW_REQUIRE(vals_planes && diag_idx && nbc >= 0, "pointers");
  if (nbc == 0) return FLOW_OK;
  FLOW_REQUIRE(dofs != nullptr, "dofs");
  FLOW_REQUIRE(vals_planes == A->vals[0], "vals_planes must be A->vals[0]");
  const long long stride =
      A->kind == 0 ? A->nnz : static_cast<long long>(A->vals[1] - A->vals[0]);
  FLOW_REQUIRE(stride >= A->nnz, "plane stride");
  if (A->kind == 2)
    FLOW_REQUIRE(A->vals[2] - A->vals[0] == 2 * stride &&
                     A->vals[3] - A->vals[0] == 3 * stride,
                 "equally spaced planes");
  hipLaunchKernelGGL(bc_identity_rows_kernel, dim3(grid_for(nbc)), dim3(kBlock),
                     0, as_stream(stream), A->kind, A->n,
                     static_cast<size_t>(stride), A->rowptr, diag_idx, nbc, dofs,
                     vals_planes);
  FLOW_CHECK_LAUNCH();
  return FLOW_OK;
}

extern "C" int flow_bc_residual(int nbc, const int* dofs, const double* g,
                                const double* u, double* F, void* stream) {
  FLOW_REQUIRE(nbc >= 0, "nbc");
  if (nbc == 0) return FLOW_OK;
  FLOW_REQUIRE(dofs && g && u && F, "pointers");
  hipLaunchKernelGGL(bc_residual_kernel, dim3(grid_for(nbc)), dim3(kBlock), 0,
                     as_stream(stream), nbc, dofs, g, u, F);
  FLOW_CHECK_LAUNCH();
  return FLOW_OK;
}

extern "C" int flow_bc_set_values(int nbc, const int* dofs, const double* g,
                                  double* x, void* stream) {
  FLOW_REQUIRE(nbc >= 0, "nbc");
  if (nbc == 0) return FLOW_OK;
  FLOW_REQUIRE(dofs && g && x, "pointers");
  hipLaunchKernelGGL(bc_residual_kernel, dim3(grid_for(nbc)), dim3(kBlock), 0,
                     as_stream(stream), nbc, dofs, g,
                     static_cast<const double*>(nullptr), x);
  FLOW_CHECK_LAUNCH();
  return FLOW_OK;
}

extern "C" int flow_bc_symmetric_matrix(int n, const int* rowptr,
                                        const int* cols, const double* vals_in,
                                        const unsigned char* isbc,
                                        double* vals_out, void* stream) {
  FLOW_REQUIRE(n > 0 && rowptr && cols && vals_in && isbc && vals_out, "pointers");
  hipLaunchKernelGGL(bc_symmetric_kernel, dim3(grid_for(n)), dim3(kBlock), 0,
                     as_stream(stream), n, rowptr, cols, vals_in, isbc, vals_out);
  FLOW_CHECK_LAUNCH();
  return FLOW_OK;
}

extern "C" int flow_assemble_heat(const flow_mesh* mesh, const flow_space* Q,
                                  const flow_space* W, const double* conv,
                                  double kappa, double rho_cp, int supg,
                                  double* scratch, double* Avals,
                                  double* Msupg_vals, double* tau_out,
                                  int* status_dev, void* stream) {
  int rc = check_mesh_space(mesh, Q);
  if (rc) return rc;
  if ((rc = check_mesh_space(mesh, W))) return rc;
  FLOW_REQUIRE(conv && scratch && Avals && status_dev, "pointers");
  FLOW_REQUIRE(Q->cptr && Q->csrc && Q->nnz > 0, "matrix map");
  FLOW_REQUIRE(!supg || Msupg_vals, "Msupg_vals required with supg");
  FLOW_REQUIRE(kappa > 0.0 && rho_cp > 0.0, "coefficients");
  hipStream_t st = as_stream(stream);
  const CellRange cr(mesh);
  const dim3 grid = cell_grid(cr.count());
#define FLOW_HEAT(DQ, DW)                                                      \
  do {                                                                         \
    if (supg)                                                                  \
      hipLaunchKernelGGL((heat_kernel<DQ, DW, true>), grid, dim3(kBlock), 0, st, \
                         mesh->nc, cr.cb, cr.ce, mesh->xy, W->cell_dofs, W->n, \
                         conv, kappa, rho_cp, scratch, tau_out, status_dev);   \
    else                                                                       \
      hipLaunchKernelGGL((heat_kernel<DQ, DW, false>), grid, dim3(kBlock), 0,  \
                         st, mesh->nc, cr.cb, cr.ce, mesh->xy, W->cell_dofs,   \
                         W->n, conv, kappa, rho_cp, scratch, tau_out,          \
                         status_dev);                                          \
  } while (0)
  if (Q->deg == 1 && W->deg == 1) FLOW_HEAT(1, 1);
  else if (Q->deg == 1 && W->deg == 2) FLOW_HEAT(1, 2);
  else if (Q->deg == 2 && W->deg == 1) FLOW_HEAT(2, 1);
  else FLOW_HEAT(2, 2);
#undef FLOW_HEAT
  FLOW_CHECK_LAUNCH();
  const int nl = Q->deg == 1 ? 3 : 6;
  const size_t plane = static_cast<size_t>(nl) * nl * mesh->nc;
  int k0 = 0, k1 = 0;
  if (Q->r1 > 0) {
    FLOW_REQUIRE(Q->nnz0 >= 0 && Q->nnz0 < Q->nnz1 && Q->nnz1 <= Q->nnz,
                 "space nonzero range");
    k0 = Q->nnz0;
    k1 = Q->nnz1;
  }
  if ((rc = gather(Q->nnz, 1, Q->cptr, Q->csrc, scratch, 0, Avals, st, 0, k0, k1)))
    return rc;
  if (supg)
    return gather(Q->nnz, 1, Q->cptr, Q->csrc, scratch + plane, 0, Msupg_vals, st,
                  0, k0, k1);
  return FLOW_OK;
}

extern "C" int flow_assemble_heat_supg_source(
    const flow_mesh* mesh, const flow_space* Q, const flow_space* W,
    const double* conv, double kappa, double rho_cp, const flow_coef* source,
    double* scratch, double* b, int* status_dev, void* stream) {
  int rc = check_mesh_space(mesh, Q);
  if (rc) return rc;
  if ((rc = check_mesh_space(mesh, W))) return rc;
  FLOW_REQUIRE(source && source->values &&
                   (source->nl == 1 || source->nl == 3 || source->nl == 6),
               "SUPG source: a P0, P1 or P2 interpolant per cell");
  FLOW_REQUIRE(source->cell_stride == 0 || source->cell_stride == 1,
               "coefficient stride");
  FLOW_REQUIRE(conv && scratch && b && status_dev && Q->vptr && Q->vsrc,
               "pointers");
  FLOW_REQUIRE(kappa > 0.0 && rho_cp > 0.0, "coefficients");
  hipStream_t st = as_stream(stream);
  const CellRange cr(mesh);
  const dim3 grid = cell_grid(cr.count());
#define FLOW_HEAT(DQ, DW)                                                        \
  hipLaunchKernelGGL((heat_supg_source_kernel<DQ, DW>), grid, dim3(kBlock), 0,   \
                     st, mesh->nc, cr.cb, cr.ce, mesh->xy, W->cell_dofs, W->n,   \
                     conv, kappa, rho_cp, *source, scratch, status_dev)
  if (Q->deg == 1 && W->deg == 1) FLOW_HEAT(1, 1);
  else if (Q->deg == 1 && W->deg == 2) FLOW_HEAT(1, 2);
  else if (Q->deg == 2 && W->deg == 1) FLOW_HEAT(2, 1);
  else FLOW_HEAT(2, 2);
#undef FLOW_HEAT
  FLOW_CHECK_LAUNCH();
  return gather(Q->n, 1, Q->vptr, Q->vsrc, scratch, 0, b, st, 0, Q->r0, Q->r1);
}
```

### flow_amd/csrc/common.h

```cpp
#pragma once
#include <hip/hip_runtime.h>

#include <algorithm>
#include <cstdarg>
#include <cstdio>
#include <functional>
#include <vector>

#include "../../include/flow_hip.h"

namespace flow {
extern unsigned long long g_launches;
}
#undef hipLaunchKernelGGL
#define hipLaunchKernelGGL(kernelName, numBlocks, numThreads, memPerBlock,        \
                           streamId, ...)                                       \
  do {                                                                          \
    ++flow::g_launches;                                                         \
    (kernelName)<<<(numBlocks), (numThreads), (memPerBlock), (streamId)>>>(     \
        __VA_ARGS__);                                                           \
  } while (0)

namespace flow {

void set_error(const char* fmt, ...);

inline hipStream_t as_stream(void* s) { return static_cast<hipStream_t>(s); }

int ilu_apply(const flow_ilu* ilu, const double* in, double* out, double* work,
              hipStream_t st, const double* stop = nullptr);
int ilu_check(const flow_ilu* ilu, int op_size);

int pmg_apply(const flow_pmg* M, const double* r, double* z, hipStream_t st,
              const double* stop = nullptr);
int pmg_check(const flow_pmg* M, int op_size);
int tl_apply(const flow_tl* T, const double* r, double* z, hipStream_t st,
             const double* stop = nullptr);
int tl_check(const flow_tl* T, int op_size);
int operator_apply(const flow_operator* A, const double* x, double* y,
                   hipStream_t st, const double* stop = nullptr);
int operator_size(const flow_operator* A);
int sum_partials_host(double* work, int nparts, double* host, hipStream_t st);
int check_operator(const flow_operator* A);
int fill(int n, double value, double* y, hipStream_t st);
struct NoEarly {
  __device__ __forceinline__ void operator()(int, bool) const {}
};

enum Slot {
  kGamma = 0, kAlpha, kBeta, kRes2, kB2, kRho, kOmega, kRhoNew, kTmp,
  kBreak, kTarget2, kDone, kConvIt, kIter, kNumSlots = 16
};
int read_state(const double* S, double* host, hipStream_t st);
int check_comm(const flow_comm* c, long long need);
int check_rows(const flow_rows* R);
int exchange(const flow_comm* c, int count);
int exchange_halo(const flow_comm* C, const flow_rows* R, int ncomp, int sum_count,
                  int hoff, hipStream_t st);

int gather(int nout, int nplanes, const int* ptr, const int* src,
           const double* scratch, size_t plane_stride, double* out,
           hipStream_t st, size_t out_stride = 0, int r0 = 0, int r1 = 0,
           const double* stop = nullptr, const unsigned char* idrow = nullptr,
           const double* v = nullptr, size_t v_stride = 0);
int momentum_jvp_check(const flow_momentum_jvp* J);
int momentum_jvp_apply(const flow_momentum_jvp* J, const double* v, double* out,
                       hipStream_t st, int v_stride = 0, int out_stride = 0,
                       const double* stop = nullptr,
                       const double* prm_dev = nullptr);
int momentum_jvp_params(const flow_momentum_jvp* J, double* dst, hipStream_t st);

constexpr long long kReplayAutoRows = 1500000;
struct KeyHash {
  unsigned long long h = 1469598103934665603ull;
  void bytes(const void* p, size_t n) {
    const unsigned char* c = static_cast<const unsigned char*>(p);
    for (size_t i = 0; i < n; ++i) h = (h ^ c[i]) * 1099511628211ull;
  }
  template <class T> KeyHash& pod(const T& v) {
    bytes(&v, sizeof(T));
    return *this;
  }
  template <class T> KeyHash& obj(const T* p) {
    const unsigned char tag = p ? 1 : 0;
    bytes(&tag, 1);
    if (p) bytes(p, sizeof(T));
    return *this;
  }
};
enum ReplaySite { kReplayCg = 1, kReplayGmres = 2, kReplayMass = 4 };
bool replay_wanted(long long rows, int site);
int replay_prepare(unsigned long long key, int site, hipStream_t st,
                   const std::function<int()>& body, hipGraphExec_t* exec,
                   int* nodes);
int replay_launch(hipGraphExec_t exec, int nodes, hipStream_t st);
void key_operator(KeyHash& k, const flow_operator* A, bool skip_prm = false);

#define FLOW_CHECK_HIP(expr)                                                 \
  do {                                                                       \
    hipError_t err_ = (expr);                                                \
    if (err_ != hipSuccess) {                                                \
      flow::set_error("%s failed: %s (%s:%d)", #expr, hipGetErrorString(err_), \
                      __FILE__, __LINE__);                                   \
      return FLOW_HIP_ERROR;                                                 \
    }                                                                        \
  } while (0)

#define FLOW_REQUIRE(cond, msg)                                  \
  do {                                                           \
    if (!(cond)) {                                               \
      flow::set_error("invalid argument: %s (%s)", msg, #cond);  \
      return FLOW_INVALID;                                       \
    }                                                            \
  } while (0)

#define FLOW_CHECK_LAUNCH() FLOW_CHECK_HIP(hipGetLastError())

constexpr int kBlock = 256;
constexpr int kRedBlocks = 1024;
constexpr int kMaxGrid = 2048;

inline int grid_for(long long n, int per_block = kBlock, int cap = kMaxGrid) {
  long long g = (n + per_block - 1) / per_block;
  if (g < 1) g = 1;
  if (g > cap) g = cap;
  return static_cast<int>(g);
}

__device__ __forceinline__ double load_scalar(const double* p) {
  return __hip_atomic_load(const_cast<double*>(p), __ATOMIC_RELAXED,
                           __HIP_MEMORY_SCOPE_SYSTEM);
}
__device__ __forceinline__ void store_scalar(double* p, double v) {
  __hip_atomic_store(p, v, __ATOMIC_RELAXED, __HIP_MEMORY_SCOPE_SYSTEM);
}

__device__ __forceinline__ bool stopped(const double* stop) {
  return stop != nullptr && load_scalar(stop) != 0.0;
}

constexpr int kXcdRun = 64;
__host__ __device__ __forceinline__ int xcd_tile(int b, int nwg) {
  constexpr int kGroup = 8 * kXcdRun;
  const int full = (nwg / kGroup) * kGroup;
  if (b < full) {
    const int g = b / kGroup, i = b - g * kGroup;
    return g * kGroup + (i & 7) * kXcdRun + (i >> 3);
  }
  const int nt = nwg - full, i = b - full;
  const int q = nt >> 3, r = nt & 7, xcd = i & 7;
  return full + (xcd < r ? xcd * (q + 1) : r * (q + 1) + (xcd - r) * q) +
         (i >> 3);
}

__device__ inline double block_sum(double v) {
  __shared__ double wave_part[4];
#pragma unroll
  for (int off = 32; off > 0; off >>= 1) v += __shfl_down(v, off, 64);
  const int lane = threadIdx.x & 63;
  const int wave = threadIdx.x >> 6;
  __syncthreads();
  if (lane == 0) wave_part[wave] = v;
  __syncthreads();
  if (threadIdx.x == 0) v = wave_part[0] + wave_part[1] + wave_part[2] + wave_part[3];
  return v;
}

__device__ inline double block_sum_once(double v) {
  __shared__ double wave_part_once[4];
#pragma unroll
  for (int off = 32; off > 0; off >>= 1) v += __shfl_down(v, off, 64);
  if ((threadIdx.x & 63) == 0) wave_part_once[threadIdx.x >> 6] = v;
  __syncthreads();
  if (threadIdx.x == 0)
    v = wave_part_once[0] + wave_part_once[1] + wave_part_once[2] +
        wave_part_once[3];
  return v;
}

__device__ inline double block_max(double v) {
  __shared__ double wave_part_m[4];
#pragma unroll
  for (int off = 32; off > 0; off >>= 1) v = fmax(v, __shfl_down(v, off, 64));
  const int lane = threadIdx.x & 63;
  const int wave = threadIdx.x >> 6;
  __syncthreads();
  if (lane == 0) wave_part_m[wave] = v;
  __syncthreads();
  if (threadIdx.x == 0)
    v = fmax(fmax(wave_part_m[0], wave_part_m[1]), fmax(wave_part_m[2], wave_part_m[3]));
  return v;
}

}
```

### flow_amd/csrc/la_kernels.hip

```cpp
#include <cstring>

#include "common.h"
#include "csr_stream.h"

namespace flow {

thread_local char g_error[512] = "";

void set_error(const char* fmt, ...) {
  va_list ap;
  va_start(ap, fmt);
  vsnprintf(g_error, sizeof(g_error), fmt, ap);
  va_end(ap);
}

static_assert(3 * kRedBlocks + kNumSlots <= FLOW_REDUCE_WORK, "work size");


template <bool DOT>
__global__ __launch_bounds__(kBlock) void spmv_stream_kernel(
    int n, const int* __restrict__ rowptr, const int* __restrict__ cols,
    const double* __restrict__ vals0, const double* __restrict__ vals1,
    const int* __restrict__ rowblocks, const double* __restrict__ x,
    double* __restrict__ y, double* __restrict__ dpart,
    const double* __restrict__ stop) {
  __shared__ double prod[kTile];
  if (stopped(stop)) return;
  const double* __restrict__ vals = blockIdx.y == 0 ? vals0 : vals1;
  x += static_cast<size_t>(blockIdx.y) * n;
  y += static_cast<size_t>(blockIdx.y) * n;
  int r, r1;
  double xi = 0.0;
  auto early = [&](int row, bool has) {
    if (DOT && has) xi = x[row];
  };
  const double s =
      stream_tile_row_sum(rowptr, cols, vals, rowblocks, x, prod, r, r1, early);
  double t = 0.0;
  if (r < r1) {
    y[r] = s;
    if (DOT) t = s * xi;
  }
  if (DOT) {
    t = block_sum_once(t);
    if (threadIdx.x == 0) dpart[blockIdx.y * gridDim.x + blockIdx.x] = t;
  }
}

template <int UP, bool DOTS>
__global__ __launch_bounds__(kBlock) void mg_level_kernel(
    const int* __restrict__ rowptr, const int* __restrict__ cols,
    const double* __restrict__ vals, const int* __restrict__ rowblocks,
    const double* __restrict__ x, const double* __restrict__ c,
    const double* __restrict__ t, const double* __restrict__ dinv, double omega,
    double* __restrict__ y, double* __restrict__ gpart,
    double* __restrict__ rpart, const double* __restrict__ stop) {
  __shared__ double prod[kTile];
  if (stopped(stop)) return;
  int r, r1;
  const double s =
      stream_tile_row_sum(rowptr, cols, vals, rowblocks, x, prod, r, r1);
  double g = 0.0, rr = 0.0;
  if (r < r1) {
    const double ci = c[r];
    if (UP) {
      const double yi = s + omega * dinv[r] * (ci + t[r]);
      y[r] = yi;
      if (DOTS) {
        g = ci * yi;
        rr = yi * yi;
      }
    } else {
      y[r] = ci - s;
    }
  }
  if (DOTS) {
    g = block_sum(g);
    rr = block_sum(rr);
    if (threadIdx.x == 0) {
      gpart[blockIdx.x] = g;
      rpart[blockIdx.x] = rr;
    }
  }
}

template <bool DOTS>
__global__ __launch_bounds__(kBlock) void mg_up2_kernel(
    const int* __restrict__ rowblocks, const int* __restrict__ p_rowptr,
    const int* __restrict__ p_cols, const double* __restrict__ p_vals,
    const int* __restrict__ a_rowptr, const int* __restrict__ a_cols,
    const double* __restrict__ a_vals, const double* __restrict__ xc,
    const double* __restrict__ c, const double* __restrict__ dinv, double omega,
    double* __restrict__ y, double* __restrict__ gpart,
    double* __restrict__ rpart, const double* __restrict__ stop,
    int own_lo = 0, int own_hi = 0x7fffffff) {
  __shared__ double prod_p[kTile];
  __shared__ double prod_a[kTile];
  if (stopped(stop)) return;
  const int tile = xcd_tile(blockIdx.x, gridDim.x);
  const int r0 = rowblocks[tile];
  const int r1 = rowblocks[tile + 1];
  const int r = r0 + threadIdx.x;
  double ci = 0.0, di = 0.0;
  if (r < r1) {
    ci = c[r];
    di = dinv[r];
  }
  const double sp = stream_rows_sum(r0, r1, p_rowptr, p_cols, p_vals, xc, prod_p);
  const double sa = stream_rows_sum(r0, r1, a_rowptr, a_cols, a_vals, c, prod_a);
  double g = 0.0, rr = 0.0;
  if (r < r1) {
    const double yi = sp + omega * di * (2.0 * ci - sa);
    y[r] = yi;
    if (DOTS && r >= own_lo && r < own_hi) {
      g = ci * yi;
      rr = yi * yi;
    }
  }
  if (DOTS) {
    g = block_sum(g);
    rr = block_sum(rr);
    if (threadIdx.x == 0) {
      gpart[blockIdx.x] = g;
      rpart[blockIdx.x] = rr;
    }
  }
}

template <bool DOT>
__global__ __launch_bounds__(kBlock) void spmv_stream_block2_kernel(
    int n, const int* __restrict__ rowptr, const int* __restrict__ cols,
    const double* __restrict__ vxx, const double* __restrict__ vxy,
    const double* __restrict__ vyx, const double* __restrict__ vyy,
    const int* __restrict__ rowblocks, const double* __restrict__ x,
    double* __restrict__ y, double* __restrict__ dpart,
    const double* __restrict__ stop) {
  __shared__ double prod0[kTile2];
  __shared__ double prod1[kTile2];
  if (stopped(stop)) return;
  const int tile = xcd_tile(blockIdx.x, gridDim.x);
  const int r0 = rowblocks[tile];
  const int r1 = rowblocks[tile + 1];
  const int k0 = rowptr[r0];
  const int k1 = rowptr[r1];
  const int ka = k0 & ~1;
  const int r = r0 + threadIdx.x;
  int a = 0, b = 0;
  if (r < r1) {
    a = rowptr[r] - ka;
    b = rowptr[r + 1] - ka;
  }
  const int npair = (k1 - ka + 1) >> 1;
  const int2* __restrict__ c2p = reinterpret_cast<const int2*>(cols + ka);
  const double2* __restrict__ pxx = reinterpret_cast<const double2*>(vxx + ka);
  const double2* __restrict__ pxy = reinterpret_cast<const double2*>(vxy + ka);
  const double2* __restrict__ pyx = reinterpret_cast<const double2*>(vyx + ka);
  const double2* __restrict__ pyy = reinterpret_cast<const double2*>(vyy + ka);
#pragma unroll
  for (int j = 0; j < kPairs2; ++j) {
    const int p = threadIdx.x + j * kBlock;
    if (p < npair) {
      const int2 c = c2p[p];
      const double2 axx = pxx[p], axy = pxy[p], ayx = pyx[p], ayy = pyy[p];
      const int cx = 2 * p >= k0 - ka ? c.x : cols[k0];
      const int cy = 2 * p + 1 < k1 - ka ? c.y : cols[k0];
      const double u0 = x[cx], u1 = x[n + cx];
      const double w0 = x[cy], w1 = x[n + cy];
      prod0[2 * p] = axx.x * u0 + axy.x * u1;
      prod1[2 * p] = ayx.x * u0 + ayy.x * u1;
      prod0[2 * p + 1] = axx.y * w0 + axy.y * w1;
      prod1[2 * p + 1] = ayx.y * w0 + ayy.y * w1;
    }
  }
  __syncthreads();
  double t = 0.0;
  if (r < r1) {
    double s0 = 0.0, s1 = 0.0;
    for (int k = a; k < b; ++k) {
      s0 += prod0[k];
      s1 += prod1[k];
    }
    y[r] = s0;
    y[n + r] = s1;
    if (DOT) t = s0 * x[r] + s1 * x[n + r];
  }
  if (DOT) {
    t = block_sum_once(t);
    if (threadIdx.x == 0) dpart[blockIdx.x] = t;
  }
}

template <bool DOT>
__global__ __launch_bounds__(kBlock) void spmv_stream_pair_kernel(
    int n, const int* __restrict__ rowptr, const int* __restrict__ cols,
    const double* __restrict__ vals, const int* __restrict__ rowblocks,
    const unsigned char* __restrict__ mask, const double* __restrict__ x,
    double* __restrict__ y, int xs, double* __restrict__ dpart,
    const double* __restrict__ stop) {
  __shared__ double2 prod[kTile2];
  if (stopped(stop)) return;
  int r, r1;
  const double2 s =
      stream_tile_pair_row_sum(rowptr, cols, vals, rowblocks, x, xs, prod, r, r1);
  double s0 = s.x, s1 = s.y;
  double t = 0.0;
  if (r < r1) {
    const double x0 = x[r], x1 = x[xs + r];
    if (!mask[r]) s0 = x0;
    if (!mask[n + r]) s1 = x1;
    y[r] = s0;
    y[xs + r] = s1;
    if (DOT) t = s0 * x0 + s1 * x1;
  }
  if (DOT) {
    t = block_sum_once(t);
    if (threadIdx.x == 0) dpart[blockIdx.x] = t;
  }
}

int check_operator(const flow_operator* A) {
  FLOW_REQUIRE(A != nullptr, "operator is NULL");
  FLOW_REQUIRE(A->kind >= 0 && A->kind <= 4, "operator kind");
  if (A->kind == 3) {
    const flow_momentum_jvp* J =
        static_cast<const flow_momentum_jvp*>(A->matfree);
    int rc = momentum_jvp_check(J);
    if (rc) return rc;
    FLOW_REQUIRE(A->n == J->W->n, "matrix-free operator size");
    return FLOW_OK;
  }
  FLOW_REQUIRE(A->n > 0 && A->nnz > 0 && A->nblocks > 0, "operator sizes");
  FLOW_REQUIRE(A->rowptr && A->cols && A->rowblocks, "operator pattern");
  const int planes = (A->kind == 0 || A->kind == 4) ? 1 : (A->kind == 1 ? 2 : 4);
  FLOW_REQUIRE(A->kind != 4 || A->rowmask != nullptr, "operator row mask");
  for (int p = 0; p < planes; ++p) {
    FLOW_REQUIRE(A->vals[p] != nullptr, "operator value plane");
    FLOW_REQUIRE((reinterpret_cast<size_t>(A->vals[p]) & 15) == 0,
                 "value planes must be 16-byte aligned");
  }
  FLOW_REQUIRE((reinterpret_cast<size_t>(A->cols) & 7) == 0,
               "cols must be 8-byte aligned");
  return FLOW_OK;
}

static inline int op_size(const flow_operator* A) {
  return A->kind == 0 ? A->n : 2 * A->n;
}

static inline int dot_parts(const flow_operator* A) {
  return A->kind == 1 ? 2 * A->nblocks : A->nblocks;
}

struct SpmvProfile {
  int rows = 0, cap = 0, used = 0;
  hipEvent_t* ev = nullptr;
};
static SpmvProfile g_spmv_profile;

void key_operator(KeyHash& k, const flow_operator* A, bool skip_prm) {
  k.obj(A);
  if (A && A->kind == 3 && A->matfree) {
    flow_momentum_jvp J = *static_cast<const flow_momentum_jvp*>(A->matfree);
    if (skip_prm) J.prm = flow_ns_params{0.0, 0.0, 0.0, 0.0, 0.0};
    k.obj(&J).obj(J.mesh).obj(J.W);
  }
}

static int apply(const flow_operator* A, const double* x, double* y,
                 hipStream_t st, double* dpart = nullptr,
                 const double* stop = nullptr, int vec_stride = 0,
                 int out_stride = 0, const double* jvp_prm = nullptr) {
  if (A->kind == 3) {
    FLOW_REQUIRE(dpart == nullptr, "matrix-free operators carry no fused dot");
    return momentum_jvp_apply(static_cast<const flow_momentum_jvp*>(A->matfree),
                              x, y, st, vec_stride, out_stride, stop, jvp_prm);
  }
  const int xs = vec_stride ? vec_stride : A->n;
  const dim3 grid(A->nblocks, A->kind == 1 ? 2 : 1);
  const double* v1 = A->kind == 1 ? A->vals[1] : A->vals[0];
  if (A->kind == 4) {
    if (dpart)
      hipLaunchKernelGGL(spmv_stream_pair_kernel<true>, grid, dim3(kBlock), 0, st,
                         A->n, A->rowptr, A->cols, A->vals[0], A->rowblocks,
                         A->rowmask, x, y, xs, dpart, stop);
    else
      hipLaunchKernelGGL(spmv_stream_pair_kernel<false>, grid, dim3(kBlock), 0,
                         st, A->n, A->rowptr, A->cols, A->vals[0], A->rowblocks,
                         A->rowmask, x, y, xs, dpart, stop);
  } else if (A->kind == 2) {
    if (dpart)
      hipLaunchKernelGGL(spmv_stream_block2_kernel<true>, grid, dim3(kBlock), 0,
                         st, A->n, A->rowptr, A->cols, A->vals[0], A->vals[1],
                         A->vals[2], A->vals[3], A->rowblocks, x, y, dpart,
                         stop);
    else
      hipLaunchKernelGGL(spmv_stream_block2_kernel<false>, grid, dim3(kBlock), 0,
                         st, A->n, A->rowptr, A->cols, A->vals[0], A->vals[1],
                         A->vals[2], A->vals[3], A->rowblocks, x, y, dpart,
                         stop);
  } else if (dpart) {
    SpmvProfile& pf = g_spmv_profile;
    const bool timed = pf.used < pf.cap && A->kind == 0 && A->n == pf.rows;
    if (timed) FLOW_CHECK_HIP(hipEventRecord(pf.ev[2 * pf.used], st));
    hipLaunchKernelGGL(spmv_stream_kernel<true>, grid, dim3(kBlock), 0, st, A->n,
                       A->rowptr, A->cols, A->vals[0], v1, A->rowblocks, x, y,
                       dpart, stop);
    if (timed) FLOW_CHECK_HIP(hipEventRecord(pf.ev[2 * pf.used++ + 1], st));
  } else {
    hipLaunchKernelGGL(spmv_stream_kernel<false>, grid, dim3(kBlock), 0, st,
                       A->n, A->rowptr, A->cols, A->vals[0], v1, A->rowblocks, x,
                       y, dpart, stop);
  }
  FLOW_CHECK_LAUNCH();
  return FLOW_OK;
}

int operator_apply(const flow_operator* A, const double* x, double* y,
                   hipStream_t st, const double* stop) {
  return apply(A, x, y, st, nullptr, stop);
}
int operator_size(const flow_operator* A) { return op_size(A); }

__global__ void diag_inv_kernel(int n, int planes_kind,
                                const int* __restrict__ diag_idx,
                                const double* __restrict__ v0,
                                const double* __restrict__ v1,
                                const unsigned char* __restrict__ mask,
                                double* __restrict__ dinv) {
  for (int i = blockIdx.x * blockDim.x + threadIdx.x; i < n;
       i += gridDim.x * blockDim.x) {
    const int k = diag_idx[i];
    dinv[i] = (mask && !mask[i]) ? 1.0 : 1.0 / v0[k];
    if (planes_kind > 0)
      dinv[n + i] = (mask && !mask[n + i]) ? 1.0 : 1.0 / v1[k];
  }
}

__global__ __launch_bounds__(kBlock) void dot3_kernel(
    int n, int nd, const double* __restrict__ a0, const double* __restrict__ b0,
    const double* __restrict__ a1, const double* __restrict__ b1,
    const double* __restrict__ a2, const double* __restrict__ b2,
    double* __restrict__ partial) {
  double s0 = 0.0, s1 = 0.0, s2 = 0.0;
  for (int i = blockIdx.x * blockDim.x + threadIdx.x; i < n;
       i += gridDim.x * blockDim.x) {
    s0 += a0[i] * b0[i];
    if (nd > 1) s1 += a1[i] * b1[i];
    if (nd > 2) s2 += a2[i] * b2[i];
  }
  s0 = block_sum(s0);
  if (nd > 1) s1 = block_sum(s1);
  if (nd > 2) s2 = block_sum(s2);
  if (threadIdx.x == 0) {
    partial[blockIdx.x] = s0;
    if (nd > 1) partial[kRedBlocks + blockIdx.x] = s1;
    if (nd > 2) partial[2 * kRedBlocks + blockIdx.x] = s2;
  }
}

__global__ __launch_bounds__(kBlock) void absmax_kernel(
    int n, const double* __restrict__ x, double* __restrict__ partial) {
  double m = 0.0;
  for (int i = blockIdx.x * blockDim.x + threadIdx.x; i < n;
       i += gridDim.x * blockDim.x)
    m = fmax(m, fabs(x[i]));
  m = block_max(m);
  if (threadIdx.x == 0) partial[blockIdx.x] = m;
}

__global__ __launch_bounds__(kBlock) void finish_kernel(
    int nparts, int nd, int is_max, const double* __restrict__ partial,
    double* __restrict__ out) {
  for (int j = 0; j < nd; ++j) {
    double v = 0.0;
    for (int i = threadIdx.x; i < nparts; i += kBlock) {
      const double p = load_scalar(partial + j * kRedBlocks + i);
      v = is_max ? fmax(v, p) : v + p;
    }
    v = is_max ? block_max(v) : block_sum(v);
    if (threadIdx.x == 0) store_scalar(out + j, v);
  }
}

__global__ void axpby_kernel(int n, double a, const double* __restrict__ x,
                             double b, double* __restrict__ y) {
  for (int i = blockIdx.x * blockDim.x + threadIdx.x; i < n;
       i += gridDim.x * blockDim.x)
    y[i] = (b == 0.0) ? a * x[i] : a * x[i] + b * y[i];
}

__global__ void fill_kernel(int n, double value, double* __restrict__ y) {
  for (int i = blockIdx.x * blockDim.x + threadIdx.x; i < n;
       i += gridDim.x * blockDim.x)
    y[i] = value;
}

int fill(int n, double value, double* y, hipStream_t st) {
  hipLaunchKernelGGL(fill_kernel, dim3(grid_for(n)), dim3(kBlock), 0, st, n,
                     value, y);
  FLOW_CHECK_LAUNCH();
  return FLOW_OK;
}

__global__ void vmul_kernel(int n, double a, const double* x, const double* y,
                            double* out, const double* stop = nullptr) {
  if (stopped(stop)) return;
  for (int i = blockIdx.x * blockDim.x + threadIdx.x; i < n;
       i += gridDim.x * blockDim.x)
    out[i] = a * x[i] * y[i];
}

__global__ void residual_kernel(int n, const double* __restrict__ b,
                                const double* __restrict__ q,
                                const double* __restrict__ dinv,
                                double* __restrict__ r, double* __restrict__ z) {
  for (int i = blockIdx.x * blockDim.x + threadIdx.x; i < n;
       i += gridDim.x * blockDim.x) {
    const double ri = b[i] - q[i];
    r[i] = ri;
    if (z) z[i] = dinv ? dinv[i] * ri : ri;
  }
}

constexpr int kScalarBlock = 1024;
__global__ __launch_bounds__(kScalarBlock) void cg_scalar_kernel(
    int nparts, int ndelta, int first, const double* __restrict__ gpart,
    const double* __restrict__ rpart, const double* __restrict__ dpart,
    double rtol2, double atol2, double* __restrict__ S) {
  __shared__ double wsum[3][kScalarBlock / 64];
  if (stopped(S + kDone)) return;
  double g = 0.0, rr = 0.0;
  for (int i = threadIdx.x; i < nparts; i += kScalarBlock) {
    g += load_scalar(gpart + i);
    rr += load_scalar(rpart + i);
  }
  double d0 = 0.0, d1 = 0.0, d2 = 0.0, d3 = 0.0;
  int i = threadIdx.x;
  for (; i + 3 * kScalarBlock < ndelta; i += 4 * kScalarBlock) {
    d0 += load_scalar(dpart + i);
    d1 += load_scalar(dpart + i + kScalarBlock);
    d2 += load_scalar(dpart + i + 2 * kScalarBlock);
    d3 += load_scalar(dpart + i + 3 * kScalarBlock);
  }
  for (; i < ndelta; i += kScalarBlock) d0 += load_scalar(dpart + i);
  double d = (d0 + d1) + (d2 + d3);
#pragma unroll
  for (int off = 32; off > 0; off >>= 1) {
    g += __shfl_down(g, off, 64);
    d += __shfl_down(d, off, 64);
    rr += __shfl_down(rr, off, 64);
  }
  if ((threadIdx.x & 63) == 0) {
    wsum[0][threadIdx.x >> 6] = g;
    wsum[1][threadIdx.x >> 6] = d;
    wsum[2][threadIdx.x >> 6] = rr;
  }
  __syncthreads();
  if (threadIdx.x == 0) {
    g = d = rr = 0.0;
    for (int w = 0; w < kScalarBlock / 64; ++w) {
      g += wsum[0][w];
      d += wsum[1][w];
      rr += wsum[2][w];
    }
  }
  if (threadIdx.x == 0) {
    double alpha, beta;
    if (first) {
      beta = 0.0;
      alpha = (d != 0.0) ? g / d : 0.0;
      const double b2 = load_scalar(S + kB2);
      store_scalar(S + kTarget2, fmax(rtol2 * b2, atol2));
      store_scalar(S + kIter, 0.0);
      if (first == 2 && rr > b2) {
        store_scalar(S + kConvIt, 0.0);
        store_scalar(S + kRes2, rr);
        store_scalar(S + kDone, 5.0);
        return;
      }
    } else {
      const double g_old = load_scalar(S + kGamma);
      const double a_old = load_scalar(S + kAlpha);
      beta = (g_old != 0.0) ? g / g_old : 0.0;
      const double den = (a_old != 0.0) ? d - beta * g / a_old : 0.0;
      alpha = (den != 0.0) ? g / den : 0.0;
    }
    const double k = load_scalar(S + kIter);
    const bool nan = !(rr == rr);
    if (nan || rr <= load_scalar(S + kTarget2)) {
      store_scalar(S + kConvIt, k);
      store_scalar(S + kDone, nan ? 2.0 : 1.0);
      alpha = beta = 0.0;
    }
    store_scalar(S + kIter, k + 1.0);
    store_scalar(S + kGamma, g);
    store_scalar(S + kAlpha, alpha);
    store_scalar(S + kBeta, beta);
    store_scalar(S + kRes2, rr);
  }
}

template <bool DOTS>
__global__ __launch_bounds__(kBlock) void cg_update_kernel(
    int n, const double* __restrict__ S, const double* __restrict__ dinv,
    const double* __restrict__ w, double* __restrict__ z, double* __restrict__ p,
    double* __restrict__ s, double* __restrict__ x, double* __restrict__ r,
    int want_z, double* __restrict__ partial,
    const double* __restrict__ own) {
  if (stopped(S + kDone)) return;
  const double alpha = load_scalar(S + kAlpha);
  const double beta = load_scalar(S + kBeta);
  double g = 0.0, rr = 0.0;
  for (int i = blockIdx.x * blockDim.x + threadIdx.x; i < n;
       i += gridDim.x * blockDim.x) {
    const double pi = z[i] + beta * p[i];
    const double si = w[i] + beta * s[i];
    p[i] = pi;
    s[i] = si;
    x[i] += alpha * pi;
    const double ri = r[i] - alpha * si;
    r[i] = ri;
    if (want_z) {
      const double zi = dinv ? dinv[i] * ri : ri;
      z[i] = zi;
      if (DOTS && (!own || own[i] != 0.0)) {
        g += ri * zi;
        rr += zi * zi;
      }
    }
  }
  if (DOTS) {
    g = block_sum(g);
    rr = block_sum(rr);
    if (threadIdx.x == 0) {
      partial[blockIdx.x] = g;
      partial[2 * kRedBlocks + blockIdx.x] = rr;
    }
  }
}

__global__ __launch_bounds__(kBlock) void coarse_restrict_kernel(
    int nc, const int* __restrict__ agg_ptr, const int* __restrict__ agg_dofs,
    const double* __restrict__ r, int r0, int r1, double* __restrict__ rc,
    const double* __restrict__ stop) {
  if (stopped(stop)) return;
  const int lane = threadIdx.x & 63;
  for (int a = blockIdx.x * 4 + (threadIdx.x >> 6); a < nc; a += gridDim.x * 4) {
    double sum = 0.0;
    for (int k = agg_ptr[a] + lane; k < agg_ptr[a + 1]; k += 64) {
      const int d = agg_dofs[k];
      if (d >= r0 && d < r1) sum += r[d];
    }
#pragma unroll
    for (int off = 32; off > 0; off >>= 1) sum += __shfl_down(sum, off, 64);
    if (lane == 0) rc[a] = sum;
  }
}

__global__ __launch_bounds__(kBlock) void coarse_gemv_kernel(
    int nc, int lda, const float* __restrict__ Ainv,
    const double* __restrict__ rc, double* __restrict__ zc,
    const double* __restrict__ stop) {
  if (stopped(stop)) return;
  const int lane = threadIdx.x & 63;
  const int nq = lda >> 2;
  for (int row = blockIdx.x * 4 + (threadIdx.x >> 6); row < nc;
       row += gridDim.x * 4) {
// ... 2987 lines not shown
```

### flow_amd/fem/ops.py

```python
import ctypes

import numpy
import torch

from . import reference
from .function import (
    Function, Expression, Constant, as_cell_coefficient, cell_lattice_points,
    )
from .space import mesh_geometry_dev
from .. import _hip
from .. import device


def mesh_struct(mesh):
    if 'mesh_struct' not in mesh._cache:
        xy = mesh_geometry_dev(mesh)
        s = _hip.MeshS(mesh.num_cells(), _hip.f64(xy, 6 * mesh.num_cells(), 'xy'))
        mesh._cache['mesh_struct'] = (s, xy)
    return mesh._cache['mesh_struct'][0]


def space_struct(layout):
    if 'struct' not in layout._dev:
        nc = layout.mesh.num_cells()
        cd = layout.dev('cell_dofs')
        s = _hip.SpaceS(
            layout.degree, layout.N, layout.nnz,
            _hip.i32(cd, layout.nloc * nc, 'cell_dofs'),
            _hip.i32(layout.dev('cptr'), layout.nnz + 1, 'cptr'),
            _hip.i32(layout.dev('csrc'), layout.nloc**2 * nc, 'csrc'),
            _hip.i32(layout.dev('vptr'), layout.N + 1, 'vptr'),
            _hip.i32(layout.dev('vsrc'), layout.nloc * nc, 'vsrc'),
            )
        layout._dev['struct'] = s
    return layout._dev['struct']


_G_CACHE = {}


def coef_struct(coef, mesh, test_degree):
    key = (coef.k, test_degree, str(device.get()))
    if key not in _G_CACHE:
        _G_CACHE[key] = device.to_device(
            reference.source_matrix(coef.k, test_degree)
            )
    G = _G_CACHE[key]
    nce = mesh.num_cells() if coef.cell_stride else 1
    s = _hip.CoefS(
        coef.nl, coef.cell_stride,
        _hip.f64(coef.values, coef.dim * coef.nl * nce, 'coefficient values'),
        _hip.f64(G, coef.nl * reference.nloc(test_degree), 'G'),
        )
    return s, (coef.values, G)


def scratch(mesh, ndoubles):
    buf = mesh._cache.get('scratch')
    if buf is None or buf.numel() < ndoubles:
        mesh._cache['scratch'] = None
        buf = device.empty(ndoubles)
        mesh._cache['scratch'] = buf
    if device._POISON:
        _hip.fill(buf, float('nan'))
    return buf


_WORK = {}


def work(ndoubles):
    key = str(device.get())
    buf = _WORK.get(key)
    if buf is None or buf.numel() < ndoubles:
        _WORK[key] = None
        buf = device.empty(ndoubles)
        _WORK[key] = buf
    return buf


def plane_stride(layout):
    return layout.nnz + (layout.nnz & 1)


def value_plane(layout):
    return device.zeros(plane_stride(layout))


class Matrix(object):
    NPLANES = {0: 1, 1: 2, 2: 4, 4: 1}

    def __init__(self, layout, kind, vals=None, rowmask=None):
        self.layout = layout
        self.kind = kind
        assert (rowmask is not None) == (kind == 4)
        if rowmask is not None:
            assert rowmask.dtype == torch.uint8 and \
                rowmask.numel() == 2 * layout.N
        self.rowmask = rowmask
        self.nplanes = self.NPLANES[kind]
        nnz = layout.nnz
        self.stride = plane_stride(layout)
        if vals is None:
            vals = device.zeros(self.nplanes * self.stride)
        elif vals.numel() == self.nplanes * nnz and self.stride != nnz:
            packed = device.zeros(self.nplanes * self.stride)
            for p in range(self.nplanes):
                packed[p * self.stride:p * self.stride + nnz] = \
                    vals[p * nnz:(p + 1) * nnz]
            vals = packed
        assert vals.numel() == self.nplanes * self.stride
        assert vals.data_ptr() % 16 == 0
        self.vals = vals
        self._op = None
        return

    @property
    def size(self):
        return self.layout.N * (1 if self.kind == 0 else 2)

    def plane(self, p):
        return self.vals[p * self.stride:p * self.stride + self.layout.nnz]

    def operator(self):
        if self._op is None:
            lay = self.layout
            op = _hip.Operator()
            op.kind = self.kind
            op.n = lay.N
            op.nnz = lay.nnz
            rb = lay.dev('rowblocks2' if self.kind in (2, 4) else 'rowblocks')
            op.nblocks = rb.numel() - 1
            op.rowptr = _hip.i32(lay.dev('rowptr'), lay.N + 1, 'rowptr')
            op.cols = _hip.i32(lay.dev('cols'), lay.nnz, 'cols')
            op.rowblocks = _hip.i32(rb, None, 'rowblocks')
            base = _hip.f64(self.vals, self.nplanes * self.stride, 'vals').value
            for p in range(self.nplanes):
                op.vals[p] = base + 8 * p * self.stride
            if self.rowmask is not None:
                op.rowmask = _hip.u8(self.rowmask, 2 * lay.N, 'rowmask').value
            self._op = op
        return self._op

    def apply(self, x, y):
        lib = _hip.lib()
        assert x.data_ptr() != y.data_ptr()
        _hip.check(lib.flow_operator_apply(
            ctypes.byref(self.operator()), _hip.f64(x, self.size, 'x'),
            _hip.f64(y, self.size, 'y'), _hip.stream()
            ))
        return y

    def diag_inv(self):
        lib = _hip.lib()
        out = device.empty(self.size)
        _hip.check(lib.flow_operator_diag_inv(
            ctypes.byref(self.operator()),
            _hip.i32(self.layout.dev('diag_idx'), self.layout.N, 'diag_idx'),
            _hip.f64(out), _hip.stream()
            ))
        return out

    def to_scipy(self):
        import scipy.sparse as sp
        lay = self.layout
        rp = lay.pattern('rowptr')
        cols = lay.pattern('cols')
        v = device.to_host(self.vals).numpy()
        nnz = lay.nnz
        st = self.stride
        P = [sp.csr_matrix((v[p * st:p * st + nnz], cols, rp),
                           shape=(lay.N, lay.N)) for p in range(self.nplanes)]
        if self.kind == 0:
            return P[0]
        if self.kind == 4:
            m = device.to_host(self.rowmask).numpy().astype(float)
            blocks = [
                sp.diags(m[c * lay.N:(c + 1) * lay.N]).dot(P[0])
                + sp.diags(1.0 - m[c * lay.N:(c + 1) * lay.N])
                for c in range(2)
                ]
            return sp.block_diag(blocks, format='csr')
        if self.kind == 1:
            return sp.block_diag(P, format='csr')
        return sp.bmat([[P[0], P[1]], [P[2], P[3]]], format='csr')


class MomentumJacobian(object):
    kind = 3

    def __init__(self, W, bfmask, ui, prm, bc_dofs, mesh_s=None, space_s=None):
        mesh = W.mesh()
        self.layout = W.layout
        self.size = W.size()
        n2 = self.size
        nc = mesh.num_cells()
        if mesh_s is None:
            mesh_s = mesh_struct(mesh)
        if space_s is None:
            space_s = space_struct(W.layout)
        self._keep = (bfmask, ui, bc_dofs,
                      device.empty(2 * W.layout.nloc * nc), mesh_s, space_s)
        self.struct = _hip.MomentumJvp(
            ctypes.pointer(mesh_s),
            ctypes.pointer(space_s),
            _hip.i32(bfmask, nc, 'bfmask'), _hip.f64(ui, n2, 'ui'), prm,
            _hip.f64(self._keep[3]), int(bc_dofs.numel()),
            _hip.i32(bc_dofs) if bc_dofs.numel() else None,
            self._bc_mask(bc_dofs),
            )
        op = _hip.Operator()
        op.kind = 3
        op.n = W.layout.N
        op.matfree = ctypes.cast(ctypes.pointer(self.struct), ctypes.c_void_p)
        self._op = op

    def operator(self):
        return self._op

    def _bc_mask(self, bc_dofs):
        if not bc_dofs.numel():
            return None
        held = getattr(self, '_mask', None)
        stamp = (bc_dofs.data_ptr(), bc_dofs.numel(), bc_dofs._version)
        if held is None or held[0] is not bc_dofs or held[2] != stamp:
            mask = torch.zeros(self.size, dtype=torch.uint8,
                               device=bc_dofs.device)
            mask[bc_dofs.long()] = 1
            device.synchronize()
            self._mask = held = (bc_dofs, mask, stamp)
        return _hip.u8(held[1], self.size, 'bc_mask')

    def rebind(self, bfmask, ui, prm, bc_dofs):
        nc = self.layout.mesh.num_cells()
        self._keep = (bfmask, ui, bc_dofs) + self._keep[3:]
        s = self.struct
        s.bfmask = _hip.i32(bfmask, nc, 'bfmask')
        s.ui = _hip.f64(ui, self.size, 'ui')
        s.prm = prm
        s.nbc = int(bc_dofs.numel())
        s.bc_dofs = _hip.i32(bc_dofs) if bc_dofs.numel() else None
        s.bc_mask = self._bc_mask(bc_dofs)
        return self

    @classmethod
    def cached(cls, W, bfmask, ui, prm, bc_dofs, mesh_s=None, space_s=None):
        key = ('jvp_operator', id(mesh_s), id(space_s))
        held = W.layout._dev.get(key)
        if held is None:
            held = cls(W, bfmask, ui, prm, bc_dofs, mesh_s, space_s)
            W.layout._dev[key] = held
            return held
        return held.rebind(bfmask, ui, prm, bc_dofs)

    def apply(self, x, y):
        lib = _hip.lib()
        assert x.data_ptr() != y.data_ptr()
        _hip.check(lib.flow_momentum_jvp_apply(
            ctypes.byref(self.struct), _hip.f64(x, self.size, 'x'),
            _hip.f64(y, self.size, 'y'), _hip.stream()
            ))
        return y


STIFFNESS, MASS, LUMPED_MASS = 0, 1, 2


def assemble_scalar_matrix(layout, kind):
    key = ('matrix', kind)
    if key not in layout._dev:
        lib = _hip.lib()
        mesh = layout.mesh
        A = Matrix(layout, 0)
        buf = scratch(mesh, layout.nloc**2 * mesh.num_cells())
        _hip.check(lib.flow_assemble_scalar_matrix(
            kind, ctypes.byref(mesh_struct(mesh)),
            ctypes.byref(space_struct(layout)), _hip.f64(buf),
            _hip.f64(A.vals), _hip.stream()
            ))
        layout._dev[key] = A
    return layout._dev[key]


def assemble_mass(V):
    return assemble_scalar_matrix(V.layout, MASS)


def assemble_stiffness(V):
    return assemble_scalar_matrix(V.layout, STIFFNESS)


def symmetric_bc_matrix(A, isbc):
    lib = _hip.lib()
    lay = A.layout
    out = Matrix(lay, 0)
    _hip.check(lib.flow_bc_symmetric_matrix(
        lay.N, _hip.i32(lay.dev('rowptr')), _hip.i32(lay.dev('cols')),
        _hip.f64(A.vals, lay.nnz), _hip.u8(isbc, lay.N, 'isbc'),
        _hip.f64(out.vals, lay.nnz), _hip.stream()
        ))
    return out


class CoarseSpace(object):

    def __init__(self, A, isbc=None, singular=False, target_nc=4096):
        import scipy.sparse as sp
        lay = A.layout
        n = lay.N
        assert A.kind == 0
        isbc = numpy.zeros(n, dtype=bool) if isbc is None else \
            numpy.asarray(isbc, dtype=bool)
        x = lay.dof_coords
        h = numpy.sqrt(2.0 * lay.mesh.cell_areas().mean())
        nfree = int(n - isbc.sum())
        s = max(2.0, numpy.sqrt(max(nfree, 1) / float(target_nc)))
        while True:
            ix = numpy.floor((x[:, 0] - x[:, 0].min()) / (s * h) + 1e-9)
            iy = numpy.floor((x[:, 1] - x[:, 1].min()) / (s * h) + 1e-9)
            key = (ix * 2000003 + iy).astype(numpy.int64)
            key[isbc] = -1
            ukey, agg = numpy.unique(key, return_inverse=True)
            if len(ukey) and ukey[0] == -1:
                agg = agg - 1
                nc = len(ukey) - 1
            else:
                nc = len(ukey)
            if nc <= 1.25 * target_nc or s > 1.0e6:
                break
            s *= 1.1
        assert nc >= 1
        self.s = s
        self.nc = nc
        self.n = n
        free = numpy.nonzero(agg >= 0)[0]
        Pm = sp.csr_matrix(
            (numpy.ones(len(free)), (free, agg[free])), shape=(n, nc)
            )
# ... 529 lines not shown
```

### include/flow_hip.h

```cpp
#ifndef FLOW_HIP_H
#define FLOW_HIP_H

#include <stddef.h>

#ifdef __cplusplus
extern "C" {
#endif

#define FLOW_OK 0
#define FLOW_NOT_CONVERGED 1
#define FLOW_INVALID 2
#define FLOW_HIP_ERROR 3

#define FLOW_SPMV_ROWS_PER_BLOCK 256
#define FLOW_SPMV_NNZ_PER_BLOCK 1022
int flow_spmv_tile_nnz(int kind);

const char* flow_last_error(void);
int flow_abi_version(void);
int flow_launch_count(unsigned long long* count_host);
int flow_graph_mode(int mode, long long auto_rows);
int flow_graph_stats(unsigned long long* stats_host);
int flow_xcd_tile_host(int block, int nblocks);

// ... 120 lines not shown
int flow_ilu0_factor(const flow_ilu_plan* plan, int nblocks,
                     const double* avals0, const double* avals1, double* lu,
                     void* stream);
int flow_ilu0_pack(const flow_ilu* ilu, float* packed, void* stream);
int flow_ilu0_solve(const flow_ilu* ilu, const double* r, double* z,
                    double* work, void* stream);

#define FLOW_PMG_NNZ_PER_BLOCK 2044
typedef struct {
  int n, nnz, nblocks;
  const int* rowptr;
  const int* cols;
  const int* rowblocks;
  const void* vals;
  const float* diag;
  const float* dinv;
  double lam_min, lam_max;
  const void* cols16;
  const int* cbase;
  const void* packed;
  const unsigned char* idrows;
} flow_pmg_level;
typedef struct {
  flow_pmg_level fine, coarse;
  int pre, post, coarse_steps;
  const int* ends;
  const int* rptr;
  const int* rsrc;
  const unsigned char* bc_fine;
  const unsigned char* bc_coarse;
  float* work;
  int scalar;
} flow_pmg;
int flow_pmg_pack(int n, int nnz, const int* rowptr, const int* diag_idx,
                  const double* a00, const double* a11,
                  const unsigned char* keep, void* vals, float* diag,
                  float* dinv, void* stream);
int flow_pmg_pack1(int n, int nnz, int nblocks, const int* rowblocks,
                   const int* rowptr, const int* cols, const int* diag_idx,
                   const double* a00, const double* a11,
                   const unsigned char* keep, const int* cbase,
                   unsigned char* idrows, void* packed, float* diag,
                   float* dinv, void* stream);
int flow_pmg_cols16(int nblocks, const int* rowblocks, const int* rowptr,
                    const int* cols, int* cbase, void* cols16,
                    int* overflow_dev, void* stream);
int flow_pmg_lambda_max(const flow_pmg_level* level, int iterations, float* work,
                        double* dwork, float* start, double* result_host,
                        void* stream);
int flow_pmg_apply(const flow_pmg* pmg, const double* r, double* z, void* stream);

int flow_aggregate_host(int n, const int* rowptr, const int* cols,
                        const double* vals, double theta,
                        const unsigned char* free_rows, int* agg,
                        int* naggregates);

typedef struct {
  const flow_ilu* fine;
  const flow_ilu* coarse;
  const flow_operator* fine_op;
  const flow_operator* coarse_op;
  int pre, post;
  int coarse_sweeps;
  const int* ends;
  const int* rptr;
  const int* rsrc;
  const unsigned char* bc_fine;
  const unsigned char* bc_coarse;
  const double* rscale;
  double* work;
} flow_tl;
int flow_tl_apply(const flow_tl* tl, const double* r, double* z, void* stream);

typedef struct {
  const flow_operator* A;
  const double* dinv;
  int nblocks16;
  const int* rowblocks16;
  const void* vals16;
  double lam_min, lam_max;
  int steps;
  double contraction;
  float* work16;
  const void* packed16;
  const int* cbase16;
  int work16_rows;
} flow_mass;
int flow_mass_pack(int n, const int* rowptr, const int* diag_idx,
                   const double* vals, void* vals16, void* stream);
int flow_mass_pack16(int n, int nblocks16, const int* rowblocks16,
                     const int* rowptr, const int* cols, const int* diag_idx,
                     const double* vals, int* cbase16, void* packed16,
                     int* overflow_dev, void* stream);
int flow_mass_solve(const flow_mass* M, const double* b, double* x, double rtol,
                    double atol, int maxit, int first_check, double* work,
                    size_t work_len, int* iters_host, double* resid_host,
                    void* stream);

int flow_mass_solve_increment(const flow_mass* M, const double* g,
                              const double* xbase, const double* delta0,
                              double* x, double rtol,
                              double atol, int maxit, int first_check,
                              double* work, size_t work_len, int* iters_host,
                              double* resid_host, void* stream);

int flow_cg_solve(const flow_operator* A, const double* dinv,
                  const flow_coarse* coarse, const flow_mg* mg,
                  const double* b, double* x,
                  double rtol, double atol, int maxit, int check_every,
                  int first_check, double* work, size_t work_len,
                  int* iters_host, double* resid_host, void* stream);
int flow_cg_solve_guarded(const flow_operator* A, const double* dinv,
                          const flow_coarse* coarse, const flow_mg* mg,
                          const double* b, double* x, const double* x_fallback,
                          double rtol, double atol, int maxit, int check_every,
                          int first_check, double* work, size_t work_len,
                          int* iters_host, double* resid_host,
                          int* starts_dropped_host, void* stream);
int flow_bicgstab_solve(const flow_operator* A, const double* dinv,
                        const flow_ilu* ilu, const double* b, double* x,
                        double rtol, double atol, int maxit, int check_every,
                        int first_check, double* work, size_t work_len,
                        int* iters_host, double* resid_host, void* stream);
#define FLOW_GMRES_MAX_RESTART 30
#define FLOW_GMRES_PARTIALS ((FLOW_GMRES_MAX_RESTART + 2) * 1024)
#define FLOW_GMRES_STATE 1280
int flow_gmres_solve(const flow_operator* A, const double* dinv,
                     const flow_ilu* ilu, const flow_pmg* pmg, const double* b,
                     double* x,
                     double rtol, double atol, int maxit, int restart,
                     int x_is_zero, int expected_its, int verify, double* work,
                     size_t work_len, int* iters_host, double* resid_host,
                     void* stream);

typedef int (*flow_allreduce_fn)(void* user, int count);
#define FLOW_PEER_FLAGS 16
typedef struct {
  unsigned long long* flags;
  double* land;
  int land_cap;
  int spin_limit;
  unsigned long long* nb_flags[2];
  double* nb_land[2];
  unsigned long long* seq_host;
} flow_peer;
typedef struct {
  int rank, world;
  double* buf;
  int capacity;
  flow_allreduce_fn allreduce;
  void* user;
  const flow_peer* peer;
} flow_comm;
int flow_peer_alloc(int land_cap, void** base_out, char* handle_out);
int flow_peer_open(const char* handle, void** base_out);
int flow_peer_close(void* mapped_base);
int flow_peer_free(void* base);
int flow_peer_status(const flow_peer* peer, unsigned long long* error_host,
                     void* stream);

#define FLOW_RCCL_ID_BYTES 128
typedef struct {
  void* comm;
  double* buf;
  void* stream;
} flow_rccl_binding;
int flow_rccl_load(const char* librccl_path);
int flow_rccl_unique_id(char* id_host);
int flow_rccl_comm_create(const char* id_host, int rank, int world,
                          void** comm_out);
int flow_rccl_comm_destroy(void* comm);
int flow_rccl_allreduce(void* user, int count);

typedef struct {
  int n;
  int r0, r1;
  int e0, e1;
  int nhalo;
  int send_row[2], send_len[2], send_slot[2];
  int recv_row[2], recv_len[2], recv_slot[2];
} flow_rows;

int flow_shard_halo(const flow_comm* comm, const flow_rows* rows, int ncomp,
                    double* x, int stride, void* stream);
int flow_shard_reduce_host(const flow_comm* comm, const flow_rows* rows,
                           int ncomp, const double* x, const double* y,
                           int stride, int kind, double* work,
                           double* result_host, void* stream);

int flow_shard_cg_solve(const flow_comm* comm, const flow_rows* rows,
                        const flow_operator* A, const double* dinv,
                        const double* b, double* x, double rtol, double atol,
                        int maxit, int check_every, int first_check,
                        double* work, size_t work_len, int* iters_host,
                        double* resid_host, int* start_rejected_host,
                        void* stream);

typedef struct {
  const flow_mg* mg;
  flow_operator Ah0, Ps0, Rg;
  flow_operator Cg;
  const int* up_rowblocks0;
  int up_nblocks0;
  int z_lo, z_hi;
} flow_mg_shard;
int flow_shard_mgcg_solve(const flow_comm* comm, const flow_rows* rows,
                          const flow_operator* A, const double* dinv,
                          const flow_mg_shard* mgs, const double* b, double* x,
                          double rtol, double atol, int maxit, int check_every,
                          int first_check, double* work, size_t work_len,
                          int* iters_host, double* resid_host,
                          int* start_rejected_host, void* stream);

typedef struct {
  int nlevels;
  const int* rowblocks16[16];
  int nblocks16[16];
  int row_lo_last, row_hi_last;
} flow_mass_strips;
int flow_shard_mass_solve(const flow_comm* comm, const flow_rows* rows,
                          const flow_mass* M, const flow_mass_strips* levels,
                          const double* b, const double* xbase,
                          const double* delta0, double* x, double rtol,
                          double atol, int maxit, int first_check, double* work,
                          size_t work_len, int* iters_host, double* resid_host,
                          void* stream);

int flow_shard_gmres_solve(const flow_comm* comm, const flow_rows* rows,
                           const flow_operator* A, const flow_ilu* ilu,
                           const flow_pmg* pmg, const double* b, double* x,
                           double rtol, double atol,
                           int maxit, int restart, int x_is_zero,
                           int expected_its, int verify, double* work,
                           size_t work_len, int* iters_host, double* resid_host,
                           void* stream);

typedef struct {
  int nc;
  const double* xy;
  int c0, c1;
} flow_mesh;

typedef struct {
  int deg;
  int n;
  int nnz;
  const int* cell_dofs;
  const int* cptr;
  const int* csrc;
  const int* vptr;
  const int* vsrc;
  int r0, r1;
  int nnz0, nnz1;
} flow_space;

typedef struct {
  int nl;
  int cell_stride;
  const double* values;
  const double* G;
} flow_coef;

int flow_assemble_scalar_matrix(int kind, const flow_mesh* mesh,
                                const flow_space* V, double* scratch,
                                double* vals, void* stream);

int flow_assemble_pressure_rhs(const flow_mesh* mesh, const flow_space* W,
                               const flow_space* P, const double* u,
                               const double* p0, double alpha_rho_dt, double mu,
                               int rotational, double* scratch, double* b,
                               void* stream);

int flow_assemble_correction_rhs(const flow_mesh* mesh, const flow_space* W,
                                 const flow_space* P, const double* u,
                                 const double* p1, const double* p0,
                                 double dt_rho, double mu, int rotational,
                                 double* scratch, double* b, void* stream);

typedef struct {
  double dt, rho, mu, theta_i, theta_e;
} flow_ns_params;
int flow_assemble_momentum(const flow_mesh* mesh, const flow_space* W,
                           const flow_space* P, const int* bfmask,
                           const double* ui, const double* u0,
                           const double* p0, const flow_coef* f0,
                           const flow_coef* f1, const flow_ns_params* prm,
                           double* scratch, double* F, double* Jvals,
                           size_t j_plane_stride, void* stream);

typedef struct {
  const flow_mesh* mesh;
  const flow_space* W;
  const int* bfmask;
  const double* ui;
  flow_ns_params prm;
  double* scratch;
  int nbc;
  const int* bc_dofs;
  const unsigned char* bc_mask;
} flow_momentum_jvp;
int flow_momentum_jvp_apply(const flow_momentum_jvp* J, const double* v,
                            double* out, void* stream);

int flow_assemble_source(const flow_mesh* mesh, const flow_space* V, int dim,
                         const flow_coef* f, double* scratch, double* b,
                         void* stream);

int flow_assemble_div_adjoint(const flow_mesh* mesh, const flow_space* W,
                              const flow_space* P, const double* p,
                              double* scratch, double* out, void* stream);

int flow_assemble_magnitude(const flow_mesh* mesh, const flow_space* W, int mode,
                            const double* u, double* scratch, double* b,
                            void* stream);

#define FLOW_FORM_MAX_PROGRAM 64
#define FLOW_FORM_REGISTERS 8
#define FLOW_FORM_MAX_CONSTANTS 32
#define FLOW_FORM_MAX_FIELDS 6
#define FLOW_FORM_MAX_EXPRESSIONS 4
#define FLOW_FORM_MAX_POINTS 256
#define FLOW_FORM_OP_CONST 0
#define FLOW_FORM_OP_COORD 1
#define FLOW_FORM_OP_FIELD 2
#define FLOW_FORM_OP_EXPR 3
#define FLOW_FORM_OP_MOV 4
#define FLOW_FORM_OP_ADD 5
#define FLOW_FORM_OP_SUB 6
#define FLOW_FORM_OP_MUL 7
#define FLOW_FORM_OP_DIV 8
#define FLOW_FORM_OP_POW 9
#define FLOW_FORM_OP_NEG 10
#define FLOW_FORM_OP_ABS 11
#define FLOW_FORM_OP_SQRT 12
#define FLOW_FORM_OP_EXP 13
#define FLOW_FORM_OP_LN 14
#define FLOW_FORM_OP_SIN 15
#define FLOW_FORM_OP_COS 16
#define FLOW_FORM_OP_OUT 17
#define FLOW_FORM_OP_NORMAL 18
typedef struct {
  int nprog;
  int prog[4 * FLOW_FORM_MAX_PROGRAM];
  int nconst;
  double consts[FLOW_FORM_MAX_CONSTANTS];
  int nfield;
  const double* field[FLOW_FORM_MAX_FIELDS];
  int field_deg[FLOW_FORM_MAX_FIELDS];
  const int* cell_dofs[2];
  int nexpr;
  const double* expr[FLOW_FORM_MAX_EXPRESSIONS];
  int expr_nl[FLOW_FORM_MAX_EXPRESSIONS];
  int expr_table[FLOW_FORM_MAX_EXPRESSIONS];
  int nq;
  const double* rule;
  const double* tables;
  int ntables;
  int nout;
} flow_form;

int flow_form_functional(const flow_mesh* mesh, const flow_form* form,
                         double* scratch, double* work, double* result_host,
                         void* stream);

int flow_form_facet_functional(const flow_mesh* mesh, const flow_form* form,
                               int nfacets, const int* facet_cell,
                               const int* facet_local, double* scratch,
                               double* work, double* result_host, void* stream);

int flow_form_load_vector(const flow_mesh* mesh, const flow_space* V,
                          const flow_form* form, double* scratch, double* b,
                          void* stream);

typedef struct {
  int nx, ny;
  double x0, y0;
  double hx_inv, hy_inv;
  const int* start;
  const int* cells;
} flow_point_grid;

int flow_locate_points(const flow_mesh* mesh, const flow_point_grid* grid, int n,
                       const double* xy, int* cell, double* bary, void* stream);

int flow_form_points(const flow_mesh* mesh, const flow_form* form, int n,
                     const int* cell, const double* bary, double* out,
                     void* stream);

int flow_bc_identity_rows(const flow_operator* A, double* vals_planes,
                          const int* diag_idx, int nbc, const int* dofs,
                          void* stream);
int flow_bc_residual(int nbc, const int* dofs, const double* g, const double* u,
                     double* F, void* stream);
int flow_bc_set_values(int nbc, const int* dofs, const double* g, double* x,
                       void* stream);
int flow_bc_symmetric_matrix(int n, const int* rowptr, const int* cols,
                             const double* vals_in, const unsigned char* isbc,
                             double* vals_out, void* stream);

int flow_assemble_heat(const flow_mesh* mesh, const flow_space* Q,
                       const flow_space* W, const double* conv, double kappa,
                       double rho_cp, int supg, double* scratch, double* Avals,
                       double* Msupg_vals, double* tau_out, int* status_dev,
                       void* stream);

int flow_assemble_heat_supg_source(const flow_mesh* mesh, const flow_space* Q,
                                   const flow_space* W, const double* conv,
                                   double kappa, double rho_cp,
                                   const flow_coef* source, double* scratch,
                                   double* b, int* status_dev, void* stream);

#ifdef __cplusplus
}
#endif
#endif
```

Before: 126.4.

## Fuse P2 cell assembly with tile-local LDS scatter via spatial cell tiles

Partitions the mesh cells into spatial tiles of 256 cells and builds a plan that classifies dofs as tile-interior or boundary. Per-cell assembly bodies are factored into device functions so that a tiled kernel can compute cell contributions into shared memory and sum interior dofs locally, instead of writing every cell's contributions to a global scratch array and gathering them in a separate kernel. Boundary dofs still go through a slot-based global path. This aims to cut the global scratch round-trip and a launch, at the cost of host-side plan construction, extra device arrays and LDS pressure.

```diff
diff --git a/flow_amd/_hip.py b/flow_amd/_hip.py
--- a/flow_amd/_hip.py
+++ b/flow_amd/_hip.py
@@ -182,6 +182,19 @@
         ('vsrc', ctypes.c_void_p),
         ('r0', ctypes.c_int), ('r1', ctypes.c_int),
         ('nnz0', ctypes.c_int), ('nnz1', ctypes.c_int),
+        ]
+
+
+class TilePlanS(ctypes.Structure):
+    _fields_ = [
+        ('nc', ctypes.c_int), ('n', ctypes.c_int), ('ntiles', ctypes.c_int),
+        ('nbnd', ctypes.c_int), ('nbsrc', ctypes.c_int),
+        ('tile_ptr', ctypes.c_void_p), ('tile_cells', ctypes.c_void_p),
+        ('int_ptr', ctypes.c_void_p), ('int_dof', ctypes.c_void_p),
+        ('int_rows', ctypes.c_void_p),
+        ('bt_ptr', ctypes.c_void_p), ('bt_slot', ctypes.c_void_p),
+        ('bnd_dof', ctypes.c_void_p), ('bnd_ptr', ctypes.c_void_p),
+        ('bnd_src', ctypes.c_void_p),
         ]
 
 
@@ -402,6 +415,8 @@
                                _VP, _P(CoefS), _P(CoefS), _P(NsParams), _VP,
                                _VP, _VP, ctypes.c_size_t, _VP],
     'flow_momentum_jvp_apply': [_P(MomentumJvp), _VP, _VP, _VP],
+    'flow_space_set_tiles': [_P(SpaceS), _P(TilePlanS)],
+    'flow_space_tiled': [_P(MeshS), _P(SpaceS)],
     'flow_assemble_source': [_P(MeshS), _P(SpaceS), _I, _P(CoefS), _VP, _VP,
                              _VP],
     'flow_assemble_magnitude': [_P(MeshS), _P(SpaceS), _I, _VP, _VP, _VP, _VP],
diff --git a/flow_amd/csrc/assembly_kernels.hip b/flow_amd/csrc/assembly_kernels.hip
--- a/flow_amd/csrc/assembly_kernels.hip
+++ b/flow_amd/csrc/assembly_kernels.hip
@@ -1,8 +1,34 @@
 #include <cstdlib>
+#include <mutex>
+#include <vector>
 
 #include "fem_device.h"
 
 namespace flow {
+
+template <int NP>
+__device__ __forceinline__ void gather_sum(int a, int b,
+                                           const int* __restrict__ src,
+                                           const double* __restrict__ scratch,
+                                           size_t plane_stride, double s[NP]) {
+#pragma unroll
+  for (int p = 0; p < NP; ++p) s[p] = 0.0;
+  for (int t = a; t < b; t += 4) {
+    int idx[4];
+#pragma unroll
+    for (int j = 0; j < 4; ++j) idx[j] = t + j < b ? src[t + j] : -1;
+    double w[NP][4];
+#pragma unroll
+    for (int p = 0; p < NP; ++p)
+#pragma unroll
+      for (int j = 0; j < 4; ++j)
+        w[p][j] = idx[j] >= 0 ? scratch[p * plane_stride + idx[j]] : 0.0;
+#pragma unroll
+    for (int p = 0; p < NP; ++p)
+#pragma unroll
+      for (int j = 0; j < 4; ++j) s[p] += w[p][j];
+  }
+}
 
 template <int NP>
 __global__ __launch_bounds__(kBlock) void gather_kernel(
@@ -14,26 +40,8 @@
   if (stopped(stop)) return;
   for (int k = blockIdx.x * blockDim.x + threadIdx.x; k < nout;
        k += gridDim.x * blockDim.x) {
-    const int a = ptr[k];
-    const int b = ptr[k + 1];
     double s[NP];
-#pragma unroll
-    for (int p = 0; p < NP; ++p) s[p] = 0.0;
-    for (int t = a; t < b; t += 4) {
-      int idx[4];
-#pragma unroll
-      for (int j = 0; j < 4; ++j) idx[j] = t + j < b ? src[t + j] : -1;
-      double w[NP][4];
-#pragma unroll
-      for (int p = 0; p < NP; ++p)
-#pragma unroll
-        for (int j = 0; j < 4; ++j)
-          w[p][j] = idx[j] >= 0 ? scratch[p * plane_stride + idx[j]] : 0.0;
-#pragma unroll
-      for (int p = 0; p < NP; ++p)
-#pragma unroll
-        for (int j = 0; j < 4; ++j) s[p] += w[p][j];
-    }
+    gather_sum<NP>(ptr[k], ptr[k + 1], src, scratch, plane_stride, s);
     if (idrow) {
 #pragma unroll
       for (int p = 0; p < NP; ++p)
@@ -158,15 +166,13 @@
 }
 
 template <int DEG>
-__global__ __launch_bounds__(kBlock) void correction_rhs_kernel(
-    int nc, int cb, int ce, const double* __restrict__ xy, const int* __restrict__ cdu, int nu,
-    const int* __restrict__ cdp, const double* __restrict__ u,
+__device__ __forceinline__ void correction_rhs_cell(
+    int nc, int c, const double* __restrict__ xy, const int* __restrict__ cdu,
+    int nu, const int* __restrict__ cdp, const double* __restrict__ u,
     const double* __restrict__ p1, const double* __restrict__ p0, double dt_rho,
-    double mu, int rotational, double* __restrict__ scratch) {
+    double mu, int rotational, double acc[2][Elem<DEG>::NL]) {
   constexpr int NL = Elem<DEG>::NL;
   constexpr int NQ = Elem<2>::NQ;
-  const int c = cb + xcd_tile(blockIdx.x, gridDim.x) * blockDim.x + threadIdx.x;
-  if (c >= ce) return;
   const Geom g = load_geom(xy, nc, c);
   double U[2][NL];
   load_local<NL>(u, nu, cdu, nc, c, 2, U);
@@ -181,7 +187,6 @@
     gphi_f[0] += coef * g.gl[k][0];
     gphi_f[1] += coef * g.gl[k][1];
   }
-  double acc[2][NL];
 #pragma unroll
   for (int a = 0; a < 2; ++a)
 #pragma unroll
@@ -202,6 +207,20 @@
       for (int i = 0; i < NL; ++i) acc[a][i] += val * phi[i];
     }
   }
+}
+
+template <int DEG>
+__global__ __launch_bounds__(kBlock) void correction_rhs_kernel(
+    int nc, int cb, int ce, const double* __restrict__ xy, const int* __restrict__ cdu, int nu,
+    const int* __restrict__ cdp, const double* __restrict__ u,
+    const double* __restrict__ p1, const double* __restrict__ p0, double dt_rho,
+    double mu, int rotational, double* __restrict__ scratch) {
+  constexpr int NL = Elem<DEG>::NL;
+  const int c = cb + xcd_tile(blockIdx.x, gridDim.x) * blockDim.x + threadIdx.x;
+  if (c >= ce) return;
+  double acc[2][NL];
+  correction_rhs_cell<DEG>(nc, c, xy, cdu, nu, cdp, u, p1, p0, dt_rho, mu,
+                           rotational, acc);
 #pragma unroll
   for (int a = 0; a < 2; ++a)
 #pragma unroll
@@ -316,6 +335,57 @@
 }
 
 template <int DEG>
+__device__ __forceinline__ void momentum_residual_cell(
+    int nc, int c, const double* __restrict__ xy, const int* __restrict__ cdu,
+    int nu, const int* __restrict__ cdp, const int* __restrict__ bfmask,
+    const double* __restrict__ ui, const double* __restrict__ u0,
+    const double* __restrict__ p0, const flow_coef& f0, const flow_coef& f1,
+    const flow_ns_params& prm, double acc[2][Elem<DEG>::NL]) {
+  constexpr int NL = Elem<DEG>::NL;
+  constexpr int NQ = Elem<DEG>::NQ;
+  const Geom g = load_geom(xy, nc, c);
+  double Ui[2][NL], U0[2][NL], P[3];
+  load_local<NL>(ui, nu, cdu, nc, c, 2, Ui);
+  load_local<NL>(u0, nu, cdu, nc, c, 2, U0);
+#pragma unroll
+  for (int k = 0; k < 3; ++k) P[k] = p0[cdp[k * nc + c]];
+  const int mask = bfmask[c];
+  const double ci = -prm.dt / prm.rho * prm.theta_i;
+  const double cexp = -prm.dt / prm.rho * prm.theta_e;
+#pragma unroll
+  for (int a = 0; a < 2; ++a)
+#pragma unroll
+    for (int i = 0; i < NL; ++i) acc[a][i] = 0.0;
+
+#pragma unroll
+  for (int q = 0; q < NQ; ++q) {
+    const double L[3] = {qpoint<DEG>(q, 0), qpoint<DEG>(q, 1), qpoint<DEG>(q, 2)};
+    const double w = 0.5 * qweight<DEG>(q) * g.adet;
+    double phi[NL], dphi[NL][3], gphi[NL][2];
+    basis<DEG>(L, phi, dphi);
+    phys_grad<NL>(g, dphi, gphi);
+#pragma unroll
+    for (int a = 0; a < 2; ++a) {
+      double du = 0.0;
+#pragma unroll
+      for (int j = 0; j < NL; ++j) du += (Ui[a][j] - U0[a][j]) * phi[j];
+#pragma unroll
+      for (int i = 0; i < NL; ++i) acc[a][i] += w * du * phi[i];
+    }
+    if (ci != 0.0)
+      add_rhs_weak_point<NL>(w * ci, prm.rho, prm.mu, Ui, P, L, phi, gphi, acc);
+    if (cexp != 0.0)
+      add_rhs_weak_point<NL>(w * cexp, prm.rho, prm.mu, U0, P, L, phi, gphi, acc);
+  }
+  if (mask) {
+    if (ci != 0.0) add_rhs_weak_facets<DEG>(mask, ci, prm.mu, g, Ui, P, acc);
+    if (cexp != 0.0) add_rhs_weak_facets<DEG>(mask, cexp, prm.mu, g, U0, P, acc);
+  }
+  if (ci != 0.0) add_source<NL>(f1, nc, c, 2, ci * g.adet, acc);
+  if (cexp != 0.0) add_source<NL>(f0, nc, c, 2, cexp * g.adet, acc);
+}
+
+template <int DEG>
 __global__ __launch_bounds__(kBlock) void momentum_residual_kernel(
     int nc, int cb, int ce, const double* __restrict__ xy, const int* __restrict__ cdu, int nu,
     const int* __restrict__ cdp, const int* __restrict__ bfmask,
@@ -323,19 +393,31 @@
     const double* __restrict__ p0, flow_coef f0, flow_coef f1,
     flow_ns_params prm, double* __restrict__ scratch) {
   constexpr int NL = Elem<DEG>::NL;
-  constexpr int NQ = Elem<DEG>::NQ;
   const int c = cb + xcd_tile(blockIdx.x, gridDim.x) * blockDim.x + threadIdx.x;
   if (c >= ce) return;
+  double acc[2][NL];
+  momentum_residual_cell<DEG>(nc, c, xy, cdu, nu, cdp, bfmask, ui, u0, p0, f0,
+                              f1, prm, acc);
+#pragma unroll
+  for (int a = 0; a < 2; ++a)
+#pragma unroll
+    for (int i = 0; i < NL; ++i)
+      scratch[static_cast<size_t>(a * NL + i) * nc + c] = acc[a][i];
+}
+
+template <int DEG>
+__device__ __forceinline__ void momentum_jvp_cell(
+    int nc, int c, const double* __restrict__ xy, const int* __restrict__ cdu,
+    int nu, int nv, const int* __restrict__ bfmask,
+    const double* __restrict__ ui, const double* __restrict__ v, double ci,
+    double hr, double mu, double acc[2][Elem<DEG>::NL]) {
+  constexpr int NL = Elem<DEG>::NL;
+  constexpr int NQ = Elem<DEG>::NQ;
   const Geom g = load_geom(xy, nc, c);
-  double Ui[2][NL], U0[2][NL], P[3];
-  load_local<NL>(ui, nu, cdu, nc, c, 2, Ui);
-  load_local<NL>(u0, nu, cdu, nc, c, 2, U0);
-#pragma unroll
-  for (int k = 0; k < 3; ++k) P[k] = p0[cdp[k * nc + c]];
+  double U[2][NL], V[2][NL];
+  load_local<NL>(ui, nu, cdu, nc, c, 2, U);
+  load_local<NL>(v, nv, cdu, nc, c, 2, V);
   const int mask = bfmask[c];
-  const double ci = -prm.dt / prm.rho * prm.theta_i;
-  const double cexp = -prm.dt / prm.rho * prm.theta_e;
-  double acc[2][NL];
 #pragma unroll
   for (int a = 0; a < 2; ++a)
 #pragma unroll
@@ -345,33 +427,48 @@
   for (int q = 0; q < NQ; ++q) {
     const double L[3] = {qpoint<DEG>(q, 0), qpoint<DEG>(q, 1), qpoint<DEG>(q, 2)};
     const double w = 0.5 * qweight<DEG>(q) * g.adet;
-    double phi[NL], dphi[NL][3], gphi[NL][2];
-    basis<DEG>(L, phi, dphi);
-    phys_grad<NL>(g, dphi, gphi);
+    double uq[2], vq[2], gu[2][2], gv[2][2];
 #pragma unroll
     for (int a = 0; a < 2; ++a) {
-      double du = 0.0;
-#pragma unroll
-      for (int j = 0; j < NL; ++j) du += (Ui[a][j] - U0[a][j]) * phi[j];
-#pragma unroll
-      for (int i = 0; i < NL; ++i) acc[a][i] += w * du * phi[i];
-    }
-    if (ci != 0.0)
-      add_rhs_weak_point<NL>(w * ci, prm.rho, prm.mu, Ui, P, L, phi, gphi, acc);
-    if (cexp != 0.0)
-      add_rhs_weak_point<NL>(w * cexp, prm.rho, prm.mu, U0, P, L, phi, gphi, acc);
-  }
-  if (mask) {
-    if (ci != 0.0) add_rhs_weak_facets<DEG>(mask, ci, prm.mu, g, Ui, P, acc);
-    if (cexp != 0.0) add_rhs_weak_facets<DEG>(mask, cexp, prm.mu, g, U0, P, acc);
-  }
-  if (ci != 0.0) add_source<NL>(f1, nc, c, 2, ci * g.adet, acc);
-  if (cexp != 0.0) add_source<NL>(f0, nc, c, 2, cexp * g.adet, acc);
-#pragma unroll
-  for (int a = 0; a < 2; ++a)
-#pragma unroll
-    for (int i = 0; i < NL; ++i)
-      scratch[static_cast<size_t>(a * NL + i) * nc + c] = acc[a][i];
+      uq[a] = eval_at<DEG>(U[a], L);
+      vq[a] = eval_at<DEG>(V[a], L);
+      double gur[3], gvr[3];
+      ref_gradient<DEG>(U[a], L, gur);
+      ref_gradient<DEG>(V[a], L, gvr);
+#pragma unroll
+      for (int d = 0; d < 2; ++d) {
+        gu[a][d] = gur[0] * g.gl[0][d] + gur[1] * g.gl[1][d] + gur[2] * g.gl[2][d];
+        gv[a][d] = gvr[0] * g.gl[0][d] + gvr[1] * g.gl[1][d] + gvr[2] * g.gl[2][d];
+      }
+    }
+#pragma unroll
+    for (int a = 0; a < 2; ++a) {
+      const double dconv = gv[a][0] * uq[0] + gv[a][1] * uq[1] +
+                           gu[a][0] * vq[0] + gu[a][1] * vq[1];
+      const double s0 = w * (vq[a] - ci * hr * dconv);
+      double S1[2];
+#pragma unroll
+      for (int d = 0; d < 2; ++d)
+        S1[d] = w * ci * (hr * (vq[d] * uq[a] + uq[d] * vq[a]) -
+                          mu * (gv[a][d] + gv[d][a]));
+      double T[3];
+#pragma unroll
+      for (int k = 0; k < 3; ++k) T[k] = g.gl[k][0] * S1[0] + g.gl[k][1] * S1[1];
+      test_accumulate<DEG>(L, s0, T, acc[a]);
+    }
+  }
+  if (mask && ci != 0.0) {
+    const double P0[3] = {0.0, 0.0, 0.0};
+    add_rhs_weak_facets<DEG>(mask, ci, mu, g, V, P0, acc);
+  }
+}
+
+__device__ __forceinline__ void jvp_factors(const flow_ns_params& prm,
+                                            const double* __restrict__ prm_dev,
+                                            double& ci, double& hr, double& mu) {
+  ci = prm_dev ? load_scalar(prm_dev) : -prm.dt / prm.rho * prm.theta_i;
+  hr = prm_dev ? load_scalar(prm_dev + 1) : 0.5 * prm.rho;
+  mu = prm_dev ? load_scalar(prm_dev + 2) : prm.mu;
 }
 
 template <int DEG>
@@ -383,63 +480,13 @@
     const double* __restrict__ prm_dev,
     double* __restrict__ scratch, const double* __restrict__ stop) {
   constexpr int NL = Elem<DEG>::NL;
-  constexpr int NQ = Elem<DEG>::NQ;
   if (stopped(stop)) return;
   const int c = cb + xcd_tile(blockIdx.x, gridDim.x) * blockDim.x + threadIdx.x;
   if (c >= ce) return;
-  const Geom g = load_geom(xy, nc, c);
-  double U[2][NL], V[2][NL];
-  load_local<NL>(ui, nu, cdu, nc, c, 2, U);
-  load_local<NL>(v, nv, cdu, nc, c, 2, V);
-  const int mask = bfmask[c];
-  const double ci = prm_dev ? load_scalar(prm_dev)
-                            : -prm.dt / prm.rho * prm.theta_i;
-  const double hr = prm_dev ? load_scalar(prm_dev + 1) : 0.5 * prm.rho;
-  const double mu = prm_dev ? load_scalar(prm_dev + 2) : prm.mu;
+  double ci, hr, mu;
+  jvp_factors(prm, prm_dev, ci, hr, mu);
   double acc[2][NL];
-#pragma unroll
-  for (int a = 0; a < 2; ++a)
-#pragma unroll
-    for (int i = 0; i < NL; ++i) acc[a][i] = 0.0;
-
-#pragma unroll
-  for (int q = 0; q < NQ; ++q) {
-    const double L[3] = {qpoint<DEG>(q, 0), qpoint<DEG>(q, 1), qpoint<DEG>(q, 2)};
-    const double w = 0.5 * qweight<DEG>(q) * g.adet;
-    double uq[2], vq[2], gu[2][2], gv[2][2];
-#pragma unroll
-    for (int a = 0; a < 2; ++a) {
-      uq[a] = eval_at<DEG>(U[a], L);
-      vq[a] = eval_at<DEG>(V[a], L);
-      double gur[3], gvr[3];
-      ref_gradient<DEG>(U[a], L, gur);
-      ref_gradient<DEG>(V[a], L, gvr);
-#pragma unroll
-      for (int d = 0; d < 2; ++d) {
-        gu[a][d] = gur[0] * g.gl[0][d] + gur[1] * g.gl[1][d] + gur[2] * g.gl[2][d];
-        gv[a][d] = gvr[0] * g.gl[0][d] + gvr[1] * g.gl[1][d] + gvr[2] * g.gl[2][d];
-      }
-    }
-#pragma unroll
-    for (int a = 0; a < 2; ++a) {
-      const double dconv = gv[a][0] * uq[0] + gv[a][1] * uq[1] +
-                           gu[a][0] * vq[0] + gu[a][1] * vq[1];
-      const double s0 = w * (vq[a] - ci * hr * dconv);
-      double S1[2];
-#pragma unroll
-      for (int d = 0; d < 2; ++d)
-        S1[d] = w * ci * (hr * (vq[d] * uq[a] + uq[d] * vq[a]) -
-                          mu * (gv[a][d] + gv[d][a]));
-      double T[3];
-#pragma unroll
-      for (int k = 0; k < 3; ++k) T[k] = g.gl[k][0] * S1[0] + g.gl[k][1] * S1[1];
-      test_accumulate<DEG>(L, s0, T, acc[a]);
-    }
-  }
-  if (mask && ci != 0.0) {
-    const double P0[3] = {0.0, 0.0, 0.0};
-    add_rhs_weak_facets<DEG>(mask, ci, mu, g, V, P0, acc);
-  }
+  momentum_jvp_cell<DEG>(nc, c, xy, cdu, nu, nv, bfmask, ui, v, ci, hr, mu, acc);
 #pragma unroll
   for (int a = 0; a < 2; ++a)
 #pragma unroll
@@ -999,19 +1046,17 @@
 }
 
 template <int DEG>
-__global__ __launch_bounds__(kBlock) void magnitude_kernel(
-    int nc, int cb, int ce, const double* __restrict__ xy, const int* __restrict__ cdu, int nu,
-    const double* __restrict__ u, int mode, double* __restrict__ scratch) {
+__device__ __forceinline__ void magnitude_cell(
+    int nc, int c, const double* __restrict__ xy, const int* __restrict__ cdu,
+    int nu, const double* __restrict__ u, int mode,
+    double acc[1][Elem<DEG>::NL]) {
   constexpr int NL = Elem<DEG>::NL;
   constexpr int NQ = 7;
-  const int c = cb + xcd_tile(blockIdx.x, gridDim.x) * blockDim.x + threadIdx.x;
-  if (c >= ce) return;
   const Geom g = load_geom(xy, nc, c);
   double U[2][NL];
   load_local<NL>(u, nu, cdu, nc, c, 2, U);
-  double acc[NL];
-#pragma unroll
-  for (int i = 0; i < NL; ++i) acc[i] = 0.0;
+#pragma unroll
+  for (int i = 0; i < NL; ++i) acc[0][i] = 0.0;
 #pragma unroll
   for (int q = 0; q < NQ; ++q) {
     const double L[3] = {kQ7L[q][0], kQ7L[q][1], kQ7L[q][2]};
@@ -1026,10 +1071,217 @@
     }
     const double m = mode == 0 ? sqrt(ux * ux + uy * uy) : fabs(ux) + fabs(uy);
 #pragma unroll
-    for (int i = 0; i < NL; ++i) acc[i] += w * m * phi[i];
-  }
-#pragma unroll
-  for (int i = 0; i < NL; ++i) scratch[static_cast<size_t>(i) * nc + c] = acc[i];
+    for (int i = 0; i < NL; ++i) acc[0][i] += w * m * phi[i];
+  }
+}
+
+template <int DEG>
+__global__ __launch_bounds__(kBlock) void magnitude_kernel(
+    int nc, int cb, int ce, const double* __restrict__ xy, const int* __restrict__ cdu, int nu,
+    const double* __restrict__ u, int mode, double* __restrict__ scratch) {
+  constexpr int NL = Elem<DEG>::NL;
+  const int c = cb + xcd_tile(blockIdx.x, gridDim.x) * blockDim.x + threadIdx.x;
+  if (c >= ce) return;
+  double acc[1][NL];
+  magnitude_cell<DEG>(nc, c, xy, cdu, nu, u, mode, acc);
+#pragma unroll
+  for (int i = 0; i < NL; ++i) scratch[static_cast<size_t>(i) * nc + c] = acc[0][i];
+}
+
+constexpr int kTile = FLOW_TILE_CELLS;
+static_assert(kTile == kBlock, "one lane per cell of a tile");
+constexpr int kTilePlane = 6 * kTile;
+static_assert(FLOW_TILE_ROW == 8, "one 16-byte row per interior dof");
+
+template <int NP>
+__device__ __forceinline__ void tile_row_sum(
+    const double* s_c, int d, uint4 row, const bool id[NP],
+    double* __restrict__ out, size_t os, const double* __restrict__ v,
+    size_t vs) {
+  const unsigned w[4] = {row.x, row.y, row.z, row.w};
+  double s[NP];
+#pragma unroll
+  for (int p = 0; p < NP; ++p) s[p] = 0.0;
+#pragma unroll
+  for (int e = 0; e < 2 * 4; ++e) {
+    const unsigned slot = (w[e >> 1] >> (16 * (e & 1))) & 0xffffu;
+    if (slot != 0xffffu) {
+#pragma unroll
+      for (int p = 0; p < NP; ++p) s[p] += s_c[p * kTilePlane + slot];
+    }
+  }
+#pragma unroll
+  for (int p = 0; p < NP; ++p) {
+    if (id[p]) s[p] = v[p * vs + d];
+    out[p * os + d] = s[p];
+  }
+}
+
+template <int NP>
+__device__ __forceinline__ void tile_id_flags(
+    const unsigned char* __restrict__ idrow, int n, int d, bool id[NP]) {
+#pragma unroll
+  for (int p = 0; p < NP; ++p)
+    id[p] = idrow && d >= 0 && idrow[static_cast<size_t>(p) * n + d];
+}
+
+template <int NP, class Cell>
+__global__ __launch_bounds__(kBlock) void tile_kernel(
+    flow_tile_plan P, Cell cell, double* __restrict__ out, size_t os,
+    double* __restrict__ bscr, const double* __restrict__ stop,
+    const unsigned char* __restrict__ idrow, const double* __restrict__ v,
+    size_t vs) {
+  __shared__ double s_c[NP * kTilePlane];
+  if (stopped(stop)) return;
+  const int t = xcd_tile(blockIdx.x, gridDim.x);
+  const int c0 = P.tile_ptr[t];
+  const int lc = threadIdx.x;
+  if (lc < P.tile_ptr[t + 1] - c0) {
+    double acc[NP][6];
+    cell(P.tile_cells[c0 + lc], acc);
+#pragma unroll
+    for (int p = 0; p < NP; ++p)
+#pragma unroll
+      for (int i = 0; i < 6; ++i) s_c[p * kTilePlane + i * kTile + lc] = acc[p][i];
+  }
+  const int i0 = P.int_ptr[t], i1 = P.int_ptr[t + 1];
+  const int b0 = P.bt_ptr[t], b1 = P.bt_ptr[t + 1];
+  const uint4* rows = reinterpret_cast<const uint4*>(P.int_rows);
+  int d[2];
+  uint4 row[2];
+  bool id[2][NP];
+#pragma unroll
+  for (int u = 0; u < 2; ++u) {
+    const int j = i0 + lc + u * kBlock;
+    d[u] = j < i1 ? P.int_dof[j] : -1;
+    row[u] = j < i1 ? rows[j] : make_uint4(0, 0, 0, 0);
+    tile_id_flags<NP>(idrow, P.n, d[u], id[u]);
+  }
+  const int bslot = b0 + lc < b1 ? P.bt_slot[b0 + lc] : 0;
+  __syncthreads();
+  const size_t nb = static_cast<size_t>(P.nbsrc);
+  for (int j = b0 + lc; j < b1; j += kBlock) {
+    const int slot = j == b0 + lc ? bslot : P.bt_slot[j];
+#pragma unroll
+    for (int p = 0; p < NP; ++p) bscr[p * nb + j] = s_c[p * kTilePlane + slot];
+  }
+#pragma unroll
+  for (int u = 0; u < 2; ++u)
+    if (d[u] >= 0) tile_row_sum<NP>(s_c, d[u], row[u], id[u], out, os, v, vs);
+  for (int j = i0 + lc + 2 * kBlock; j < i1; j += kBlock) {
+    const int dj = P.int_dof[j];
+    bool idj[NP];
+    tile_id_flags<NP>(idrow, P.n, dj, idj);
+    tile_row_sum<NP>(s_c, dj, rows[j], idj, out, os, v, vs);
+  }
+}
+
+template <int NP>
+__global__ __launch_bounds__(kBlock) void tile_fixup_kernel(
+    flow_tile_plan P, const double* __restrict__ bscr, double* __restrict__ out,
+    size_t os, const double* __restrict__ stop,
+    const unsigned char* __restrict__ idrow, const double* __restrict__ v,
+    size_t vs) {
+  if (stopped(stop)) return;
+  for (int k = blockIdx.x * blockDim.x + threadIdx.x; k < P.nbnd;
+       k += gridDim.x * blockDim.x) {
+    const int d = P.bnd_dof[k];
+    bool id[NP];
+    tile_id_flags<NP>(idrow, P.n, d, id);
+    double s[NP];
+    gather_sum<NP>(P.bnd_ptr[k], P.bnd_ptr[k + 1], P.bnd_src, bscr,
+                   static_cast<size_t>(P.nbsrc), s);
+#pragma unroll
+    for (int p = 0; p < NP; ++p) {
+      if (id[p]) s[p] = v[p * vs + d];
+      out[p * os + d] = s[p];
+    }
+  }
+}
+
+struct JvpTileCell {
+  int nc, nu, nv;
+  const double *xy, *ui, *v, *prm_dev;
+  const int *cdu, *bfmask;
+  flow_ns_params prm;
+  __device__ void operator()(int c, double acc[2][6]) const {
+    double ci, hr, mu;
+    jvp_factors(prm, prm_dev, ci, hr, mu);
+    momentum_jvp_cell<2>(nc, c, xy, cdu, nu, nv, bfmask, ui, v, ci, hr, mu, acc);
+  }
+};
+
+struct ResidualTileCell {
+  int nc, nu;
+  const double *xy, *ui, *u0, *p0;
+  const int *cdu, *cdp, *bfmask;
+  flow_coef f0, f1;
+  flow_ns_params prm;
+  __device__ void operator()(int c, double acc[2][6]) const {
+    momentum_residual_cell<2>(nc, c, xy, cdu, nu, cdp, bfmask, ui, u0, p0, f0,
+                              f1, prm, acc);
+  }
+};
+
+struct CorrectionTileCell {
+  int nc, nu, rotational;
+  const double *xy, *u, *p1, *p0;
+  const int *cdu, *cdp;
+  double dt_rho, mu;
+  __device__ void operator()(int c, double acc[2][6]) const {
+    correction_rhs_cell<2>(nc, c, xy, cdu, nu, cdp, u, p1, p0, dt_rho, mu,
+                           rotational, acc);
+  }
+};
+
+struct MagnitudeTileCell {
+  int nc, nu, mode;
+  const double *xy, *u;
+  const int* cdu;
+  __device__ void operator()(int c, double acc[1][6]) const {
+    magnitude_cell<2>(nc, c, xy, cdu, nu, u, mode, acc);
+  }
+};
+
+struct TileEntry {
+  const flow_space* V;
+  const int *cell_dofs, *vptr, *vsrc;
+  flow_tile_plan plan;
+};
+static std::mutex g_tiles_mu;
+static std::vector<TileEntry> g_tiles;
+
+bool tile_plan(const flow_mesh* mesh, const flow_space* V, flow_tile_plan* out) {
+  if (!mesh || !V || V->deg != 2 || V->r1 > 0) return false;
+  if (mesh->c1 > 0 && !(mesh->c0 == 0 && mesh->c1 == mesh->nc)) return false;
+  std::lock_guard<std::mutex> lock(g_tiles_mu);
+  for (const TileEntry& e : g_tiles) {
+    if (e.V != V) continue;
+    if (e.cell_dofs != V->cell_dofs || e.vptr != V->vptr || e.vsrc != V->vsrc ||
+        e.plan.n != V->n || e.plan.nc != mesh->nc)
+      return false;
+    *out = e.plan;
+    return true;
+  }
+  return false;
+}
+
+template <int NP, class Cell>
+static int tile_apply(const flow_tile_plan& T, const Cell& cell, double* out,
+                      size_t os, double* bscr, hipStream_t st,
+                      const double* stop = nullptr,
+                      const unsigned char* idrow = nullptr,
+                      const double* v = nullptr, size_t vs = 0) {
+  hipLaunchKernelGGL((tile_kernel<NP, Cell>), dim3(T.ntiles), dim3(kBlock), 0,
+                     st, T, cell, out, os, bscr, stop, idrow, v, vs);
+  FLOW_CHECK_LAUNCH();
+  if (T.nbnd > 0) {
+    hipLaunchKernelGGL(tile_fixup_kernel<NP>,
+                       dim3(grid_for(T.nbnd, kBlock, 1 << 20)), dim3(kBlock), 0,
+                       st, T, bscr, out, os, stop, idrow, v, vs);
+    FLOW_CHECK_LAUNCH();
+  }
+  return FLOW_OK;
 }
 
 static int check_mesh_space(const flow_mesh* mesh, const flow_space* V) {
@@ -1110,6 +1362,13 @@
   FLOW_REQUIRE(P->deg == 1 && W->vptr && W->vsrc, "spaces");
   FLOW_REQUIRE(u && p1 && p0 && scratch && b, "pointers");
   hipStream_t st = as_stream(stream);
+  flow_tile_plan T;
+  if (tile_plan(mesh, W, &T))
+    return tile_apply<2>(T,
+                         CorrectionTileCell{mesh->nc, W->n, rotational, mesh->xy,
+                                            u, p1, p0, W->cell_dofs,
+                                            P->cell_dofs, dt_rho, mu},
+                         b, W->n, scratch, st);
   const CellRange cr(mesh);
   FLOW_DISPATCH_DEG(W->deg, correction_rhs_kernel, cell_grid(cr.count()), st,
                     mesh->nc, cr.cb, cr.ce, mesh->xy, W->cell_dofs, W->n,
@@ -1158,7 +1417,15 @@
   hipStream_t st = as_stream(stream);
   const int nl = W->deg == 1 ? 3 : 6;
   const CellRange cr(mesh);
-  if (F) {
+  flow_tile_plan T;
+  if (F && tile_plan(mesh, W, &T)) {
+    if ((rc = tile_apply<2>(T,
+                            ResidualTileCell{mesh->nc, W->n, mesh->xy, ui, u0, p0,
+                                             W->cell_dofs, P->cell_dofs, bfmask,
+                                             *f0, *f1, *prm},
+                            F, W->n, scratch, st)))
+      return rc;
+  } else if (F) {
     FLOW_REQUIRE(W->vptr && W->vsrc, "vector map");
     FLOW_DISPATCH_DEG(W->deg, momentum_residual_kernel, cell_grid(cr.count()),
                       st, mesh->nc, cr.cb, cr.ce, mesh->xy, W->cell_dofs, W->n,
@@ -1232,21 +1499,31 @@
     const char* e = getenv("FLOW_AMD_JVP_PAIR");
     return e && e[0] == '1';
   }();
-  if (W->deg == 2 && pair) {
-    hipLaunchKernelGGL(momentum_jvp_pair_kernel<2>, cell_grid(2 * cr.count()),
-                       dim3(kBlock), 0, st, mesh->nc, cr.cb, cr.ce, mesh->xy,
-                       W->cell_dofs, W->n, vs, J->bfmask, J->ui, v, J->prm,
-                       prm_dev, J->scratch, stop);
-    FLOW_CHECK_LAUNCH();
+  const unsigned char* idrow = J->nbc > 0 ? J->bc_mask : nullptr;
+  flow_tile_plan T;
+  if (!pair && tile_plan(mesh, W, &T)) {
+    if ((rc = tile_apply<2>(T,
+                            JvpTileCell{mesh->nc, W->n, vs, mesh->xy, J->ui, v,
+                                        prm_dev, W->cell_dofs, J->bfmask, J->prm},
+                            out, os, J->scratch, st, stop, idrow, v, vs)))
+      return rc;
   } else {
-    FLOW_DISPATCH_DEG(W->deg, momentum_jvp_kernel, cell_grid(cr.count()), st,
-                      mesh->nc, cr.cb, cr.ce, mesh->xy, W->cell_dofs, W->n, vs,
-                      J->bfmask, J->ui, v, J->prm, prm_dev, J->scratch, stop);
-  }
-  if ((rc = gather(W->n, 2, W->vptr, W->vsrc, J->scratch,
-                   static_cast<size_t>(nl) * mesh->nc, out, st, os, W->r0,
-                   W->r1, stop, J->nbc > 0 ? J->bc_mask : nullptr, v, vs)))
-    return rc;
+    if (W->deg == 2 && pair) {
+      hipLaunchKernelGGL(momentum_jvp_pair_kernel<2>, cell_grid(2 * cr.count()),
+                         dim3(kBlock), 0, st, mesh->nc, cr.cb, cr.ce, mesh->xy,
+                         W->cell_dofs, W->n, vs, J->bfmask, J->ui, v, J->prm,
+                         prm_dev, J->scratch, stop);
+      FLOW_CHECK_LAUNCH();
+    } else {
+      FLOW_DISPATCH_DEG(W->deg, momentum_jvp_kernel, cell_grid(cr.count()), st,
+                        mesh->nc, cr.cb, cr.ce, mesh->xy, W->cell_dofs, W->n, vs,
+                        J->bfmask, J->ui, v, J->prm, prm_dev, J->scratch, stop);
+    }
+    if ((rc = gather(W->n, 2, W->vptr, W->vsrc, J->scratch,
+                     static_cast<size_t>(nl) * mesh->nc, out, st, os, W->r0,
+                     W->r1, stop, idrow, v, vs)))
+      return rc;
+  }
   if (J->nbc > 0 && !J->bc_mask) {
     const int r0 = W->r1 > 0 ? W->r0 : 0, r1 = W->r1 > 0 ? W->r1 : W->n;
     hipLaunchKernelGGL(bc_copy_kernel, dim3(grid_for(J->nbc)), dim3(kBlock), 0,
@@ -1274,6 +1551,12 @@
   FLOW_REQUIRE(mode == 0 || mode == 1, "mode");
   FLOW_REQUIRE(u && scratch && b && W->vptr && W->vsrc, "pointers");
   hipStream_t st = as_stream(stream);
+  flow_tile_plan T;
+  if (tile_plan(mesh, W, &T))
+    return tile_apply<1>(T,
+                         MagnitudeTileCell{mesh->nc, W->n, mode, mesh->xy, u,
+                                           W->cell_dofs},
+                         b, W->n, scratch, st);
   const CellRange cr(mesh);
   FLOW_DISPATCH_DEG(W->deg, magnitude_kernel, cell_grid(cr.count()), st, mesh->nc,
                     cr.cb, cr.ce, mesh->xy, W->cell_dofs, W->n, u, mode, scratch);
@@ -1436,3 +1719,34 @@
   FLOW_CHECK_LAUNCH();
   return gather(Q->n, 1, Q->vptr, Q->vsrc, scratch, 0, b, st, 0, Q->r0, Q->r1);
 }
+
+extern "C" int flow_space_set_tiles(const flow_space* V, const flow_tile_plan* plan) {
+  FLOW_REQUIRE(V != nullptr, "space");
+  if (plan) {
+    FLOW_REQUIRE(V->deg == 2 && V->n == plan->n && V->cell_dofs && V->vptr &&
+                     V->vsrc,
+                 "tile plans are for P2 spaces with contribution maps");
+    FLOW_REQUIRE(plan->nc > 0 && plan->ntiles > 0 && plan->nbnd >= 0 &&
+                     plan->nbsrc >= 0 && plan->nbsrc <= 6 * plan->nc,
+                 "tile plan sizes");
+    FLOW_REQUIRE(plan->tile_ptr && plan->tile_cells && plan->int_ptr &&
+                     (reinterpret_cast<size_t>(plan->int_rows) & 15) == 0 &&
+                     plan->bt_ptr && (plan->nbsrc == 0 || plan->bt_slot) &&
+                     (plan->nbnd == 0 ||
+                      (plan->bnd_dof && plan->bnd_ptr && plan->bnd_src)),
+                 "tile plan arrays");
+  }
+  std::lock_guard<std::mutex> lock(g_tiles_mu);
+  for (size_t i = 0; i < g_tiles.size(); ++i)
+    if (g_tiles[i].V == V) {
+      g_tiles.erase(g_tiles.begin() + i);
+      break;
+    }
+  if (plan) g_tiles.push_back(TileEntry{V, V->cell_dofs, V->vptr, V->vsrc, *plan});
+  return FLOW_OK;
+}
+
+extern "C" int flow_space_tiled(const flow_mesh* mesh, const flow_space* V) {
+  flow_tile_plan T;
+  return tile_plan(mesh, V, &T) ? 1 : 0;
+}
diff --git a/flow_amd/csrc/common.h b/flow_amd/csrc/common.h
--- a/flow_amd/csrc/common.h
+++ b/flow_amd/csrc/common.h
@@ -69,6 +69,7 @@
                        const double* stop = nullptr,
                        const double* prm_dev = nullptr);
 int momentum_jvp_params(const flow_momentum_jvp* J, double* dst, hipStream_t st);
+bool tile_plan(const flow_mesh* mesh, const flow_space* V, flow_tile_plan* out);
 
 constexpr long long kReplayAutoRows = 1500000;
 struct KeyHash {
diff --git a/flow_amd/csrc/la_kernels.hip b/flow_amd/csrc/la_kernels.hip
--- a/flow_amd/csrc/la_kernels.hip
+++ b/flow_amd/csrc/la_kernels.hip
@@ -263,6 +263,9 @@
     flow_momentum_jvp J = *static_cast<const flow_momentum_jvp*>(A->matfree);
     if (skip_prm) J.prm = flow_ns_params{0.0, 0.0, 0.0, 0.0, 0.0};
     k.obj(&J).obj(J.mesh).obj(J.W);
+    flow_tile_plan T;
+    const bool tiled = tile_plan(J.mesh, J.W, &T);
+    k.obj(tiled ? &T : nullptr);
   }
 }
 
diff --git a/flow_amd/fem/ops.py b/flow_amd/fem/ops.py
--- a/flow_amd/fem/ops.py
+++ b/flow_amd/fem/ops.py
@@ -1,9 +1,12 @@
 import ctypes
+import os
+import weakref
 
 import numpy
 import torch
 
 from . import reference
+from . import tiles
 from .function import (
     Function, Expression, Constant, as_cell_coefficient, cell_lattice_points,
     )
@@ -33,7 +36,44 @@
             _hip.i32(layout.dev('vsrc'), layout.nloc * nc, 'vsrc'),
             )
         layout._dev['struct'] = s
+        if layout.degree == 2 and tiles_wanted():
+            set_tiles(layout, True)
     return layout._dev['struct']
+
+
+def tiles_wanted():
+    return os.environ.get('FLOW_AMD_TILES', '1') != '0' and device.on_gpu()
+
+
+def _detach_tiles(lib, addr):
+    lib.flow_space_set_tiles(ctypes.cast(addr, ctypes.POINTER(_hip.SpaceS)),
+                             None)
+
+
+def set_tiles(layout, on, plan=None):
+    assert layout.degree == 2
+    s = space_struct(layout)
+    lib = _hip.lib()
+    if not on:
+        _hip.check(lib.flow_space_set_tiles(ctypes.byref(s), None))
+        return
+    held = layout._dev.get('tiles')
+    if held is None or plan is not None:
+        first = held is None
+        if plan is None:
+            plan = tiles.layout_plan(layout)
+        names = [f for f, _ in _hip.TilePlanS._fields_[5:]]
+        arrays = dict((k, device.to_device(plan[k])) for k in names)
+        ps = _hip.TilePlanS(
+            plan['nc'], plan['n'], plan['ntiles'], plan['nbnd'], plan['nbsrc'],
+            *[ctypes.c_void_p(arrays[k].data_ptr() if arrays[k].numel() else None)
+              for k in names])
+        _hip.check(lib.flow_space_set_tiles(ctypes.byref(s), None))
+        layout._dev['tiles'] = held = (ps, arrays)
+        if first:
+            weakref.finalize(layout, _detach_tiles, lib,
+                             ctypes.addressof(s)).atexit = False
+    _hip.check(lib.flow_space_set_tiles(ctypes.byref(s), ctypes.byref(held[0])))
 
 
 _G_CACHE = {}
diff --git a/flow_amd/fem/tiles.py b/flow_amd/fem/tiles.py
--- /dev/null
+++ b/flow_amd/fem/tiles.py
@@ -0,0 +1,124 @@
+import numpy
+
+TILE_CELLS = 256
+TILE_ROW = 8
+NLOC = 6
+
+
+def partition(centroids, cap=TILE_CELLS):
+    centroids = numpy.asarray(centroids, dtype=numpy.float64)
+    tiles = []
+    stack = [numpy.arange(len(centroids), dtype=numpy.int64)]
+    while stack:
+        idx = stack.pop()
+        n = len(idx)
+        k = -(-n // cap)
+        if k <= 1:
+            if n:
+                tiles.append(numpy.sort(idx))
+            continue
+        pts = centroids[idx]
+        axis = int(numpy.argmax(pts.max(axis=0) - pts.min(axis=0)))
+        nl = n * (k // 2) // k
+        part = numpy.argpartition(pts[:, axis], nl)
+        stack.append(idx[part[nl:]])
+        stack.append(idx[part[:nl]])
+    return tiles
+
+
+def _segments(starts, lens):
+    lens = numpy.asarray(lens, dtype=numpy.int64)
+    total = int(lens.sum())
+    if total == 0:
+        return numpy.zeros(0, dtype=numpy.int64)
+    offs = numpy.zeros(len(lens), dtype=numpy.int64)
+    numpy.cumsum(lens[:-1], out=offs[1:])
+    return numpy.repeat(numpy.asarray(starts, dtype=numpy.int64) - offs,
+                        lens) + numpy.arange(total, dtype=numpy.int64)
+
+
+def _ptr(counts):
+    p = numpy.zeros(len(counts) + 1, dtype=numpy.int64)
+    numpy.cumsum(counts, out=p[1:])
+    return p
+
+
+def build_plan(vptr, vsrc, nc, tiles):
+    vptr = numpy.asarray(vptr, dtype=numpy.int64)
+    vsrc = numpy.asarray(vsrc, dtype=numpy.int64)
+    n = len(vptr) - 1
+    sizes = numpy.array([len(t) for t in tiles], dtype=numpy.int64)
+    assert sizes.max() <= TILE_CELLS
+    ntiles = len(tiles)
+    tile_ptr = _ptr(sizes)
+    tile_cells = numpy.concatenate(tiles).astype(numpy.int64)
+    assert len(tile_cells) == nc
+    cell_tile = numpy.full(nc, -1, dtype=numpy.int64)
+    cell_tile[tile_cells] = numpy.repeat(numpy.arange(ntiles), sizes)
+    cell_local = numpy.empty(nc, dtype=numpy.int64)
+    cell_local[tile_cells] = numpy.arange(nc) - numpy.repeat(tile_ptr[:-1],
+                                                             sizes)
+    assert (cell_tile >= 0).all(), 'every cell in a tile'
+
+    cell = vsrc % nc
+    etile = cell_tile[cell]
+    elds = (vsrc // nc) * TILE_CELLS + cell_local[cell]
+    counts = vptr[1:] - vptr[:-1]
+    if len(vsrc):
+        at = numpy.minimum(vptr[:-1], len(vsrc) - 1)
+        tmin = numpy.minimum.reduceat(etile, at)
+        tmax = numpy.maximum.reduceat(etile, at)
+    else:
+        tmin = tmax = numpy.zeros(n, dtype=numpy.int64)
+    interior = (counts > 0) & (counts <= TILE_ROW) & (tmin == tmax)
+
+    idofs = numpy.nonzero(interior)[0]
+    order = numpy.argsort(tmin[idofs], kind='stable')
+    int_dof = idofs[order]
+    int_ptr = _ptr(numpy.bincount(tmin[int_dof], minlength=ntiles))
+    ient = _segments(vptr[int_dof], counts[int_dof])
+    int_rows = numpy.full((len(int_dof), TILE_ROW), -1, dtype=numpy.int64)
+    lens = counts[int_dof]
+    col = numpy.arange(len(ient)) - numpy.repeat(_ptr(lens)[:-1], lens)
+    int_rows[numpy.repeat(numpy.arange(len(int_dof)), lens), col] = elds[ient]
+
+    bnd_dof = numpy.nonzero(~interior)[0]
+    bent = _segments(vptr[bnd_dof], counts[bnd_dof])
+    bnd_ptr = _ptr(counts[bnd_dof])
+    key = etile[bent] * (NLOC * TILE_CELLS) + elds[bent]
+    border = numpy.argsort(key, kind='stable')
+    bnd_src = numpy.empty(len(bent), dtype=numpy.int64)
+    bnd_src[border] = numpy.arange(len(bent))
+    bt_slot = elds[bent][border]
+    bt_ptr = _ptr(numpy.bincount(etile[bent], minlength=ntiles))
+
+    i32 = numpy.int32
+    return {
+        'nc': int(nc), 'n': int(n), 'ntiles': int(ntiles),
+        'nbnd': int(len(bnd_dof)), 'nbsrc': int(len(bent)),
+        'tile_ptr': tile_ptr.astype(i32), 'tile_cells': tile_cells.astype(i32),
+        'int_ptr': int_ptr.astype(i32), 'int_dof': int_dof.astype(i32),
+        'int_rows': int_rows.astype(numpy.int16).reshape(-1),
+        'bt_ptr': bt_ptr.astype(i32), 'bt_slot': bt_slot.astype(numpy.int16),
+        'bnd_dof': bnd_dof.astype(i32), 'bnd_ptr': bnd_ptr.astype(i32),
+        'bnd_src': bnd_src.astype(i32),
+        }
+
+
+def layout_plan(layout):
+    assert layout.degree == 2
+    plan = getattr(layout, '_tile_plan', None)
+    if plan is None:
+        mesh = layout.mesh
+        centroids = mesh.points[mesh.cell_vertices].mean(axis=1)
+        ext = centroids.max(axis=0) - centroids.min(axis=0)
+        centroids = centroids * numpy.where(ext == ext.max(), 2.0, 1.0)
+        plan = build_plan(layout.vmap('vptr'), layout.vmap('vsrc'),
+                          mesh.num_cells(), partition(centroids))
+        layout._tile_plan = plan
+    return plan
+
+
+def boundary_fraction(plan):
+    return (plan['nbnd'] / float(plan['n']),
+            plan['nbsrc'] / float(NLOC * plan['nc']))
diff --git a/include/flow_hip.h b/include/flow_hip.h
--- a/include/flow_hip.h
+++ b/include/flow_hip.h
@@ -446,6 +446,28 @@
 int flow_momentum_jvp_apply(const flow_momentum_jvp* J, const double* v,
                             double* out, void* stream);
 
+#define FLOW_TILE_CELLS 256
+#define FLOW_TILE_ROW 8
+typedef struct {
+  int nc;
+  int n;
+  int ntiles;
+  int nbnd;
+  int nbsrc;
+  const int* tile_ptr;
+  const int* tile_cells;
+  const int* int_ptr;
+  const int* int_dof;
+  const unsigned short* int_rows;
+  const int* bt_ptr;
+  const unsigned short* bt_slot;
+  const int* bnd_dof;
+  const int* bnd_ptr;
+  const int* bnd_src;
+} flow_tile_plan;
+int flow_space_set_tiles(const flow_space* V, const flow_tile_plan* plan);
+int flow_space_tiled(const flow_mesh* mesh, const flow_space* V);
+
 int flow_assemble_source(const flow_mesh* mesh, const flow_space* V, int dim,
                          const flow_coef* f, double* scratch, double* b,
                          void* stream);
```

Measured after the change: 126.8, median of 4. About the same (+0.3%).
